# Minimap2onGPU/mm2-gb

Measured on AMD Instinct MI355X. Metric: chaining anchor-pairs/s, higher is better.
Workload: dtype int32+f32

## Files before the change

### include/mm2gb_chain.h

```cpp
#ifndef MM2GB_CHAIN_H
#define MM2GB_CHAIN_H

#include <stddef.h>
#include <stdint.h>

#ifdef __cplusplus
extern "C" {
#endif

#define MM2GB_VERSION "0.1-mi355x"

typedef struct { uint64_t x, y; } mm2gb_anchor_t;

typedef struct {
	int max_iter, max_dist_x, max_dist_y, max_skip, bw, min_cnt, min_score, is_cdna, n_seg;
	float chn_pen_gap, chn_pen_skip;
} mm2gb_misc_t;

typedef struct {
	int     num_streams;
	int     min_n;
	int64_t long_seg_buffer_size;
	int64_t max_total_n;
	int     max_read;
	int     avg_read_n;
	int     has_max_total_n, has_max_read, has_avg_read_n;
	struct { int blockdim, cut_check_anchors, anchor_per_block; } range_kernel;
	struct { int micro_batch, mid_blockdim, short_griddim, long_griddim, mid_griddim,
	             long_seg_cutoff, mid_seg_cutoff; } score_kernel;
} mm2gb_config_t;

typedef struct {
	int64_t n_anchors, n_reads;
	int64_t n_pairs;
	int64_t n_chunks;
	int64_t n_long_chunks;
	int64_t n_mid_chunks;
	int64_t n_tracked_chunks;
	int64_t n_clamped_blocks;
	float   ms_h2d, ms_prep, ms_score, ms_d2h, ms_total;
	float   ms_post;
} mm2gb_stats_t;

typedef struct mm2gb_engine mm2gb_engine_t;

const char *mm2gb_last_error(void);
const char *mm2gb_version(void);

void mm2gb_config_defaults(mm2gb_config_t *cfg);
int  mm2gb_config_parse(const char *json_text, mm2gb_config_t *cfg);
int  mm2gb_config_load(const char *path, mm2gb_config_t *cfg);

int  mm2gb_device_count(void);
int  mm2gb_device_numa_node(int device);
int  mm2gb_pin_thread_to_device(int device);
int  mm2gb_numa_cpus_for_bdf(const char *bdf, const char *sysfs_root_dir, int32_t *node_out, int32_t *cpus, int32_t max_cpus);
mm2gb_engine_t *mm2gb_engine_create(const mm2gb_config_t *cfg, const mm2gb_misc_t *misc, int device);
void mm2gb_engine_destroy(mm2gb_engine_t *eng);
int  mm2gb_engine_set_misc(mm2gb_engine_t *eng, const mm2gb_misc_t *misc);
int  mm2gb_engine_set_chain_skip(mm2gb_engine_t *eng, int keep);
int  mm2gb_engine_last_score_form(const mm2gb_engine_t *eng);
int  mm2gb_engine_band_groups(const mm2gb_engine_t *eng, int64_t *out);
int  mm2gb_engine_skip_stats(mm2gb_engine_t *eng, int64_t *out6);
int  mm2gb_engine_device(const mm2gb_engine_t *eng);
void mm2gb_engine_gang_counts(const mm2gb_engine_t *eng, int64_t *chunks, int64_t *workgroups);
int  mm2gb_has_gang_build(void);
int  mm2gb_engine_reserve(mm2gb_engine_t *eng, int64_t n_anchors, int64_t n_reads);

int mm2gb_score_host(mm2gb_engine_t *eng, int64_t n_reads, const int64_t *offsets, const mm2gb_anchor_t *anchors,
                     int32_t *f, int32_t *p, mm2gb_stats_t *stats);
int mm2gb_score_device(mm2gb_engine_t *eng, int64_t n_reads, const int64_t *d_offsets, const mm2gb_anchor_t *d_anchors,
                       int64_t n_anchors, int32_t *d_f, int32_t *d_p);
int mm2gb_engine_sync(mm2gb_engine_t *eng);
int mm2gb_engine_stats(mm2gb_engine_t *eng, mm2gb_stats_t *stats);
void *mm2gb_engine_stream(mm2gb_engine_t *eng);
float mm2gb_engine_last_kernel_ms(mm2gb_engine_t *eng);

typedef struct {
	int64_t *u_off;   uint64_t *u;
	int64_t *a_off;   mm2gb_anchor_t *a;
} mm2gb_chains_t;
int  mm2gb_chain_host(mm2gb_engine_t *eng, int64_t n_reads, const int64_t *offsets, const mm2gb_anchor_t *anchors,
                      int n_threads, mm2gb_chains_t *out, mm2gb_stats_t *stats);
void mm2gb_chains_free(mm2gb_chains_t *out);

int  mm2gb_chain_gpu(mm2gb_engine_t *eng, int64_t n_reads, const int64_t *offsets, const mm2gb_anchor_t *anchors,
                     mm2gb_chains_t *out, mm2gb_stats_t *stats);
int  mm2gb_post_device(mm2gb_engine_t *eng, int64_t n_reads, const int64_t *d_offsets, const mm2gb_anchor_t *d_anchors, int64_t n_anchors,
                       const int32_t *d_f, const int32_t *d_p, int64_t *n_chains, int64_t *n_kept, float *ms);
int  mm2gb_post_device_enqueue(mm2gb_engine_t *eng, int64_t n_reads, const int64_t *d_offsets, const mm2gb_anchor_t *d_anchors, int64_t n_anchors,
                               const int32_t *d_f, const int32_t *d_p);
int  mm2gb_post_device_totals(mm2gb_engine_t *eng, int64_t *n_chains, int64_t *n_kept, float *ms);
int  mm2gb_post_device_digest(mm2gb_engine_t *eng, int64_t n_reads, uint64_t *digest);
int  mm2gb_debug_last_fill(mm2gb_engine_t *eng, int64_t n, int32_t *f, int32_t *p);

typedef struct {
	int max_dist, max_dist_inner, bw, max_chn_skip, cap_rmq_size, min_cnt, min_sc;
	float chn_pen_gap, chn_pen_skip;
} mm2gb_rmq_param_t;
int  mm2gb_rmq_chain_gpu(mm2gb_engine_t *eng, const mm2gb_rmq_param_t *prm, int64_t n_reads, const int64_t *offsets, const mm2gb_anchor_t *anchors,
                         mm2gb_chains_t *out, int32_t *n_tied, mm2gb_stats_t *stats);
typedef struct { int64_t n_device, n_host_cost, n_host_tie; double est_device_s, est_host_s, device_s, host_s, tie_s, total_s; int32_t device_kernel , n_team ; } mm2gb_rmq_deal_t;
int  mm2gb_engine_set_rmq_kernel(mm2gb_engine_t *eng, int kind);
int  mm2gb_engine_set_rmq_team_reads(mm2gb_engine_t *eng, int n);
int  mm2gb_rmq_chain(mm2gb_engine_t *eng, const mm2gb_rmq_param_t *prm, int64_t n_reads, const int64_t *offsets, const mm2gb_anchor_t *anchors,
                     int n_threads, mm2gb_chains_t *out, int32_t *where, mm2gb_rmq_deal_t *deal);
int  mm2gb_rmq_chain_host(const mm2gb_rmq_param_t *prm, int64_t n_reads, const int64_t *offsets, const mm2gb_anchor_t *anchors, int n_threads,
                          mm2gb_chains_t *out, int32_t *n_tied);
int  mm2gb_rmq_chain_host_tied(const mm2gb_rmq_param_t *prm, int64_t n_reads, const int64_t *offsets, const mm2gb_anchor_t *anchors, int n_threads, mm2gb_chains_t *out);
mm2gb_anchor_t *mm2gb_lchain_rmq(int max_dist, int max_dist_inner, int bw, int max_chn_skip, int cap_rmq_size, int min_cnt, int min_sc,
                                 float chn_pen_gap, float chn_pen_skip, int64_t n, mm2gb_anchor_t *a, int *n_u_, uint64_t **_u, void *km);
void mm2gb_lchain_rmq_counts(int64_t *calls, int64_t *tied_calls);

typedef struct {
	int32_t id, cnt, rid, score, qs, qe, rs, re, parent, subsc, as, mlen, blen, n_sub, score0;
	uint32_t flags;
	uint32_t hash;
	float div;
} mm2gb_reg_t;
int  mm2gb_sort_seeds_gpu(mm2gb_engine_t *eng, int64_t n_reads, const int64_t *offsets, mm2gb_anchor_t *anchors);
typedef struct { uint32_t n, q_pos, span_flt, seg_tandem; } mm2gb_seed_t;
int  mm2gb_collect_seeds_gpu(mm2gb_engine_t *eng, int64_t opt_flag, int64_t n_reads, const int64_t *seed_off, const mm2gb_seed_t *seeds,
                             const int64_t *hit_off, const uint64_t *hits, const int32_t *qlen, const int32_t *q_rank,
                             int32_t n_ref, const int32_t *ref_len, const int32_t *ref_rank, int64_t *anchor_off, mm2gb_anchor_t *anchors);
int  mm2gb_gen_regs_gpu(mm2gb_engine_t *eng, int64_t n_reads, const mm2gb_chains_t *chains, const int32_t *qlen, const uint32_t *hash,
                        int is_qstrand, mm2gb_reg_t *regs);

typedef struct mm2gb_index mm2gb_index_t;
typedef struct { int32_t mid_occ, max_max_occ, occ_dist; float q_occ_frac; } mm2gb_seed_opt_t;
typedef struct {
	int32_t n_seeds, rep_len, n_mini_pos, pad_;
	int64_t n_hits;
	mm2gb_seed_t *seeds;
	uint64_t *hits;
	uint64_t *mini_pos;
} mm2gb_matches_t;
#define MM2GB_I_HPC 0x1
int  mm2gb_sketch(const char *seq, int32_t len, int w, int k, uint32_t rid, uint64_t **out_xy, int64_t *n_out);
int  mm2gb_sketch_flag(const char *seq, int32_t len, int w, int k, uint32_t rid, int flag, uint64_t **out_xy, int64_t *n_out);
mm2gb_index_t *mm2gb_index_build(int k, int w, int32_t n_seq, const char *const *seqs, const int32_t *lens, int n_threads);
mm2gb_index_t *mm2gb_index_build_flag(int k, int w, int flag, int32_t n_seq, const char *const *seqs, const int32_t *lens, int n_threads);
int  mm2gb_index_flag(const mm2gb_index_t *ix);
void mm2gb_index_destroy(mm2gb_index_t *ix);
int64_t mm2gb_index_size(const mm2gb_index_t *ix, int64_t *n_occurrences);
int32_t mm2gb_index_mid_occ(const mm2gb_index_t *ix, float mid_occ_frac, int32_t min_mid_occ, int32_t max_mid_occ);
int  mm2gb_collect_seeds_host(int64_t opt_flag, int64_t n_reads, const int64_t *seed_off, const mm2gb_seed_t *seeds, const int64_t *hit_off,
                              const uint64_t *hits, const int32_t *qlen, const int32_t *q_rank, int32_t n_ref, const int32_t *ref_len,
                              const int32_t *ref_rank, int n_threads, int64_t *anchor_off, mm2gb_anchor_t *anchors);
int  mm2gb_collect_matches(const mm2gb_index_t *ix, const char *seq, int32_t len, const mm2gb_seed_opt_t *opt, mm2gb_matches_t *out);
void mm2gb_matches_free(mm2gb_matches_t *m);

int  mm2gb_sketch_gpu(mm2gb_engine_t *eng, int w, int k, int64_t n_seqs, const int64_t *seq_off, const char *seqs,
                      const uint32_t *rid, int64_t *mini_off, uint64_t **out_xy);
int  mm2gb_sketch_gpu_flag(mm2gb_engine_t *eng, int w, int k, int flag, int64_t n_seqs, const int64_t *seq_off, const char *seqs,
                           const uint32_t *rid, int64_t *mini_off, uint64_t **out_xy);
int  mm2gb_index_to_device(mm2gb_index_t *ix, int device);
typedef struct {
	int64_t n_seeds, n_hits;
	int64_t *seed_off;
	mm2gb_seed_t *seeds;
	int64_t *hit_off;
	uint64_t *hits;
	uint64_t *mini_pos;
	int32_t *rep_len;
} mm2gb_match_batch_t;
int  mm2gb_collect_matches_gpu(mm2gb_engine_t *eng, const mm2gb_index_t *ix, const mm2gb_seed_opt_t *opt, int64_t n_reads,
                               const int64_t *seq_off, const char *seqs, mm2gb_match_batch_t *out);
void mm2gb_match_batch_free(mm2gb_match_batch_t *m);

typedef struct {
	int64_t n_keys, n_occ, n_bucket;
	int32_t bucket_shift, k, w, built_on;
	int64_t uploads;
	const uint64_t *keys;
	const int64_t  *first;
	const uint64_t *where;
	const uint32_t *bucket;
} mm2gb_index_view_t;
mm2gb_index_t *mm2gb_index_build_gpu(mm2gb_engine_t *eng, int k, int w, int32_t n_seq, const char *const *seqs, const int32_t *lens);
mm2gb_index_t *mm2gb_index_build_gpu_flag(mm2gb_engine_t *eng, int k, int w, int flag, int32_t n_seq, const char *const *seqs, const int32_t *lens);
int32_t mm2gb_index_mid_occ_gpu(mm2gb_engine_t *eng, const mm2gb_index_t *ix, float mid_occ_frac, int32_t min_mid_occ, int32_t max_mid_occ);
int  mm2gb_index_view(const mm2gb_index_t *ix, mm2gb_index_view_t *out);
int  mm2gb_index_fetch_device(const mm2gb_index_t *ix, int device, uint64_t *keys, int64_t *first, uint64_t *where, uint32_t *bucket);
int  mm2gb_index_build_split(const mm2gb_index_t *ix, double *ms5);

typedef struct {
	int64_t flag;
	int32_t seed, mid_occ, min_mid_occ, max_mid_occ, max_max_occ, occ_dist;
	float   mid_occ_frac, q_occ_frac;
	int32_t min_cnt, min_chain_score, bw, bw_long, max_gap, max_gap_ref, max_chain_iter;
	int32_t rmq_inner_dist, rmq_size_cap, rmq_rescue_size;
	float   rmq_rescue_ratio, chain_gap_scale, chain_skip_scale;
	float   mask_level; int32_t mask_len; float pri_ratio; int32_t best_n;
	int32_t host_threads;
	int32_t seeds_on_device;
	int32_t rechain_on_device;
	int32_t max_chain_skip;
	int32_t seeding_on_device;
} mm2gb_map_opt_t;
typedef struct { int64_t n_reads, n_mapped, n_anchors, n_chains, n_rechained, n_rmq_tied; double s_seed, s_anchors, s_chain, s_rechain, s_regs, s_post; } mm2gb_map_stats_t;
void mm2gb_map_opt_init(mm2gb_map_opt_t *opt);
int  mm2gb_map_reads(mm2gb_engine_t *eng, const mm2gb_index_t *ix, int k, const char *const *ref_names, const int32_t *ref_lens, int32_t n_ref,
                     const mm2gb_map_opt_t *opt, int32_t n_reads, const char *const *names, const char *const *seqs, const int32_t *lens,
                     char **paf_out, int64_t *paf_len, mm2gb_map_stats_t *stats);

int  mm2gb_map_reads_multi(mm2gb_engine_t *const *engines, int n_engines, const mm2gb_index_t *ix, int k, const char *const *ref_names, const int32_t *ref_lens,
                           int32_t n_ref, const mm2gb_map_opt_t *opt, int32_t n_reads, const char *const *names, const char *const *seqs, const int32_t *lens,
                           char **paf_out, int64_t *paf_len, mm2gb_map_stats_t *stats);
int  mm2gb_map_reads_stream(mm2gb_engine_t *const *engines, int n_engines, const mm2gb_index_t *ix, int k, const char *const *ref_names, const int32_t *ref_lens,
                            int32_t n_ref, const mm2gb_map_opt_t *opt, int32_t n_reads, const char *const *names, const char *const *seqs, const int32_t *lens,
                            int64_t chunk_bases, char **paf_out, int64_t *paf_len, mm2gb_map_stats_t *stats);
int  mm2gb_engine_release_host_scratch(mm2gb_engine_t *eng);

typedef struct mm2gb_pool mm2gb_pool_t;
mm2gb_pool_t *mm2gb_pool_create(const mm2gb_config_t *cfg, const mm2gb_misc_t *misc, int n_devices, const int *devices);
// ... 100 lines not shown
```

### mm2-gb_amd/__init__.py

```python
import ctypes as C
import os

import numpy as np

_HERE = os.path.dirname(os.path.abspath(__file__))
LIB_PATH = os.environ.get("MM2GB_LIB_PATH") or os.path.join(_HERE, "libmm2gb_chain.so")
INT32_MAX = 2**31 - 1


class Misc(C.Structure):
    _fields_ = [("max_iter", C.c_int), ("max_dist_x", C.c_int), ("max_dist_y", C.c_int), ("max_skip", C.c_int),
                ("bw", C.c_int), ("min_cnt", C.c_int), ("min_score", C.c_int), ("is_cdna", C.c_int), ("n_seg", C.c_int),
                ("chn_pen_gap", C.c_float), ("chn_pen_skip", C.c_float)]


class _RangeCfg(C.Structure):
    _fields_ = [("blockdim", C.c_int), ("cut_check_anchors", C.c_int), ("anchor_per_block", C.c_int)]


class _ScoreCfg(C.Structure):
    _fields_ = [("micro_batch", C.c_int), ("mid_blockdim", C.c_int), ("short_griddim", C.c_int), ("long_griddim", C.c_int),
                ("mid_griddim", C.c_int), ("long_seg_cutoff", C.c_int), ("mid_seg_cutoff", C.c_int)]


class Config(C.Structure):
    _fields_ = [("num_streams", C.c_int), ("min_n", C.c_int), ("long_seg_buffer_size", C.c_int64), ("max_total_n", C.c_int64),
                ("max_read", C.c_int), ("avg_read_n", C.c_int),
                ("has_max_total_n", C.c_int), ("has_max_read", C.c_int), ("has_avg_read_n", C.c_int),
                ("range_kernel", _RangeCfg), ("score_kernel", _ScoreCfg)]


class Stats(C.Structure):
    _fields_ = [("n_anchors", C.c_int64), ("n_reads", C.c_int64), ("n_pairs", C.c_int64), ("n_chunks", C.c_int64),
                ("n_long_chunks", C.c_int64), ("n_mid_chunks", C.c_int64), ("n_tracked_chunks", C.c_int64), ("n_clamped_blocks", C.c_int64),
                ("ms_h2d", C.c_float), ("ms_prep", C.c_float), ("ms_score", C.c_float), ("ms_d2h", C.c_float), ("ms_total", C.c_float),
                ("ms_post", C.c_float)]

    def as_dict(self):
        return {k: getattr(self, k) for k, _ in self._fields_}


class Chains(C.Structure):
    _fields_ = [("u_off", C.POINTER(C.c_int64)), ("u", C.POINTER(C.c_uint64)), ("a_off", C.POINTER(C.c_int64)), ("a", C.c_void_p)]


class RmqParam(C.Structure):
    _fields_ = [("max_dist", C.c_int), ("max_dist_inner", C.c_int), ("bw", C.c_int), ("max_chn_skip", C.c_int), ("cap_rmq_size", C.c_int),
                ("min_cnt", C.c_int), ("min_sc", C.c_int), ("chn_pen_gap", C.c_float), ("chn_pen_skip", C.c_float)]


READ_DONE_FN = C.CFUNCTYPE(None, C.c_void_p, C.c_int64, C.c_int, C.POINTER(C.c_uint64), C.c_int64, C.c_void_p)


class BatcherStats(C.Structure):
    _fields_ = [("reads", C.c_int64), ("anchors", C.c_int64), ("reads_per_lane", C.c_int64 * 2), ("batches", C.c_int64 * 2),
                ("batches_per_engine", C.c_int64 * 16), ("n_engines", C.c_int)]


class Mm2gbError(RuntimeError):
    pass


_lib = None

CORE_SYMBOLS = ["mm2gb_last_error", "mm2gb_version", "mm2gb_config_defaults", "mm2gb_config_parse", "mm2gb_config_load",
                "mm2gb_device_count", "mm2gb_device_numa_node", "mm2gb_pin_thread_to_device", "mm2gb_numa_cpus_for_bdf", "mm2gb_engine_create", "mm2gb_engine_destroy", "mm2gb_engine_set_misc", "mm2gb_engine_device", "mm2gb_engine_gang_counts", "mm2gb_has_gang_build",
                "mm2gb_engine_reserve", "mm2gb_score_host", "mm2gb_score_device", "mm2gb_engine_sync", "mm2gb_engine_stats",
                "mm2gb_engine_stream", "mm2gb_engine_last_kernel_ms", "mm2gb_chain_host", "mm2gb_chain_gpu", "mm2gb_post_device", "mm2gb_post_device_enqueue", "mm2gb_post_device_totals", "mm2gb_post_device_digest", "mm2gb_chains_free", "mm2gb_backtrack_host",
                "mm2gb_free", "mm2gb_lchain_dp", "mm2gb_synth_count", "mm2gb_synth_fill",
                "mm2gb_pool_create", "mm2gb_pool_destroy", "mm2gb_pool_size", "mm2gb_pool_device", "mm2gb_pool_set_misc",
                "mm2gb_pool_score_host", "mm2gb_pool_chain_host",
                "mm2gb_batcher_create", "mm2gb_batcher_add", "mm2gb_batcher_feed", "mm2gb_batcher_flush", "mm2gb_batcher_stats", "mm2gb_batcher_destroy",
                "mm2gb_plan_batches", "mm2gb_rmq_chain_gpu", "mm2gb_lchain_rmq", "mm2gb_lchain_rmq_counts",
                "mm2gb_sort_seeds_gpu", "mm2gb_gen_regs_gpu", "mm2gb_collect_seeds_gpu",
                "mm2gb_sketch", "mm2gb_index_build", "mm2gb_index_destroy", "mm2gb_index_size", "mm2gb_index_mid_occ", "mm2gb_collect_matches", "mm2gb_matches_free", "mm2gb_map_opt_init", "mm2gb_map_reads", "mm2gb_engine_release_host_scratch", "mm2gb_rmq_chain_host", "mm2gb_rmq_chain_host_tied", "mm2gb_rmq_chain", "mm2gb_engine_set_rmq_kernel", "mm2gb_engine_set_rmq_team_reads", "mm2gb_engine_set_chain_skip", "mm2gb_engine_last_score_form", "mm2gb_engine_band_groups", "mm2gb_collect_seeds_host", "mm2gb_map_reads_multi", "mm2gb_map_reads_stream",
                "mm2gb_sketch_gpu", "mm2gb_index_to_device", "mm2gb_collect_matches_gpu", "mm2gb_match_batch_free",
                "mm2gb_index_build_gpu", "mm2gb_index_mid_occ_gpu", "mm2gb_index_view", "mm2gb_index_fetch_device", "mm2gb_index_build_split",
                "mm2gb_sketch_flag", "mm2gb_sketch_gpu_flag", "mm2gb_index_build_flag", "mm2gb_index_build_gpu_flag", "mm2gb_index_flag",
                "mm2gb_align_opt_init", "mm2gb_align_regs_host", "mm2gb_align_regs_gpu", "mm2gb_align_out_free"]
BOUNDARY_SYMBOLS = ["init_stream_gpu", "chain_stream_gpu", "finish_stream_gpu", "free_stream_gpu"]


def lib():
    global _lib
    if _lib is None:
        if not os.path.exists(LIB_PATH):
            raise Mm2gbError(f"{LIB_PATH} is missing: build it with `make -C {_HERE}` (hipcc, --offload-arch=gfx950); "
                             "there is no CPU fallback")
        L = C.CDLL(LIB_PATH)
        L.mm2gb_last_error.restype = C.c_char_p
        L.mm2gb_version.restype = C.c_char_p
        L.mm2gb_config_defaults.argtypes = [C.POINTER(Config)]
        L.mm2gb_config_defaults.restype = None
        L.mm2gb_config_parse.argtypes = [C.c_char_p, C.POINTER(Config)]
        L.mm2gb_config_load.argtypes = [C.c_char_p, C.POINTER(Config)]
        L.mm2gb_engine_create.restype = C.c_void_p
        L.mm2gb_engine_create.argtypes = [C.POINTER(Config), C.POINTER(Misc), C.c_int]
        L.mm2gb_engine_destroy.argtypes = [C.c_void_p]
        L.mm2gb_engine_destroy.restype = None
        L.mm2gb_engine_set_misc.argtypes = [C.c_void_p, C.POINTER(Misc)]
        L.mm2gb_engine_device.argtypes = [C.c_void_p]
        L.mm2gb_engine_reserve.argtypes = [C.c_void_p, C.c_int64, C.c_int64]
        L.mm2gb_engine_set_chain_skip.argtypes = [C.c_void_p, C.c_int]
        L.mm2gb_engine_last_score_form.argtypes = [C.c_void_p]
        L.mm2gb_engine_band_groups.argtypes = [C.c_void_p, C.POINTER(C.c_int64)]
        L.mm2gb_score_host.argtypes = [C.c_void_p, C.c_int64, C.c_void_p, C.c_void_p, C.c_void_p, C.c_void_p, C.POINTER(Stats)]
        L.mm2gb_score_device.argtypes = [C.c_void_p, C.c_int64, C.c_void_p, C.c_void_p, C.c_int64, C.c_void_p, C.c_void_p]
        L.mm2gb_engine_sync.argtypes = [C.c_void_p]
        L.mm2gb_engine_stats.argtypes = [C.c_void_p, C.POINTER(Stats)]
        L.mm2gb_engine_stream.argtypes = [C.c_void_p]
        L.mm2gb_engine_stream.restype = C.c_void_p
        L.mm2gb_engine_last_kernel_ms.argtypes = [C.c_void_p]
        L.mm2gb_engine_last_kernel_ms.restype = C.c_float
        L.mm2gb_chain_host.argtypes = [C.c_void_p, C.c_int64, C.c_void_p, C.c_void_p, C.c_int, C.POINTER(Chains), C.POINTER(Stats)]
        L.mm2gb_chain_gpu.argtypes = [C.c_void_p, C.c_int64, C.c_void_p, C.c_void_p, C.POINTER(Chains), C.POINTER(Stats)]
        L.mm2gb_post_device_enqueue.argtypes = [C.c_void_p, C.c_int64, C.c_void_p, C.c_void_p, C.c_int64, C.c_void_p, C.c_void_p]
        L.mm2gb_post_device_totals.argtypes = [C.c_void_p, C.POINTER(C.c_int64), C.POINTER(C.c_int64), C.POINTER(C.c_float)]
        L.mm2gb_post_device_digest.argtypes = [C.c_void_p, C.c_int64, C.c_void_p]
        L.mm2gb_post_device.argtypes = [C.c_void_p, C.c_int64, C.c_void_p, C.c_void_p, C.c_int64, C.c_void_p, C.c_void_p,
                                        C.POINTER(C.c_int64), C.POINTER(C.c_int64), C.POINTER(C.c_float)]
        L.mm2gb_chains_free.argtypes = [C.POINTER(Chains)]
        L.mm2gb_chains_free.restype = None
        L.mm2gb_backtrack_host.argtypes = [C.POINTER(Misc), C.c_int64, C.c_void_p, C.c_void_p, C.c_void_p,
                                           C.POINTER(C.c_void_p), C.POINTER(C.c_void_p)]
        L.mm2gb_free.argtypes = [C.c_void_p]
        L.mm2gb_free.restype = None
        L.mm2gb_lchain_dp.restype = C.c_void_p
        L.mm2gb_lchain_dp.argtypes = [C.c_int] * 7 + [C.c_float, C.c_float, C.c_int, C.c_int, C.c_int64, C.c_void_p,
                                                      C.POINTER(C.c_int), C.POINTER(C.c_void_p), C.c_void_p]
        L.mm2gb_synth_count.restype = C.c_int64
        L.mm2gb_synth_count.argtypes = [C.c_uint64, C.c_int64, C.c_int64, C.c_int, C.c_int, C.c_void_p]
        L.mm2gb_synth_fill.argtypes = [C.c_uint64, C.c_int64, C.c_int64, C.c_int, C.c_int, C.c_void_p, C.c_void_p, C.c_int]
        L.mm2gb_pool_create.restype = C.c_void_p
        L.mm2gb_pool_create.argtypes = [C.POINTER(Config), C.POINTER(Misc), C.c_int, C.c_void_p]
        L.mm2gb_pool_destroy.argtypes = [C.c_void_p]
        L.mm2gb_pool_destroy.restype = None
        L.mm2gb_pool_size.argtypes = [C.c_void_p]
        L.mm2gb_pool_device.argtypes = [C.c_void_p, C.c_int]
        L.mm2gb_pool_set_misc.argtypes = [C.c_void_p, C.POINTER(Misc)]
        L.mm2gb_pool_score_host.argtypes = [C.c_void_p, C.c_int64, C.c_void_p, C.c_void_p, C.c_void_p, C.c_void_p, C.POINTER(Stats), C.c_void_p]
        L.mm2gb_pool_chain_host.argtypes = [C.c_void_p, C.c_int64, C.c_void_p, C.c_void_p, C.c_int, C.POINTER(Chains), C.POINTER(Stats)]
        L.mm2gb_rmq_chain_gpu.argtypes = [C.c_void_p, C.POINTER(RmqParam), C.c_int64, C.c_void_p, C.c_void_p, C.POINTER(Chains), C.c_void_p, C.POINTER(Stats)]
        L.mm2gb_lchain_rmq.restype = C.c_void_p
        L.mm2gb_lchain_rmq.argtypes = [C.c_int] * 7 + [C.c_float, C.c_float, C.c_int64, C.c_void_p, C.POINTER(C.c_int), C.POINTER(C.c_void_p), C.c_void_p]
        L.mm2gb_lchain_rmq_counts.argtypes = [C.POINTER(C.c_int64), C.POINTER(C.c_int64)]
        L.mm2gb_lchain_rmq_counts.restype = None
        L.mm2gb_sort_seeds_gpu.argtypes = [C.c_void_p, C.c_int64, C.c_void_p, C.c_void_p]
        L.mm2gb_sketch.argtypes = [C.c_char_p, C.c_int32, C.c_int, C.c_int, C.c_uint32, C.POINTER(C.c_void_p), C.POINTER(C.c_int64)]
        L.mm2gb_sketch_flag.argtypes = [C.c_char_p, C.c_int32, C.c_int, C.c_int, C.c_uint32, C.c_int, C.POINTER(C.c_void_p), C.POINTER(C.c_int64)]
        L.mm2gb_index_build_flag.restype = C.c_void_p
        L.mm2gb_index_build_flag.argtypes = [C.c_int, C.c_int, C.c_int, C.c_int32, C.POINTER(C.c_char_p), C.c_void_p, C.c_int]
        L.mm2gb_index_build_gpu_flag.restype = C.c_void_p
        L.mm2gb_index_build_gpu_flag.argtypes = [C.c_void_p, C.c_int, C.c_int, C.c_int, C.c_int32, C.POINTER(C.c_char_p), C.c_void_p]
        L.mm2gb_index_flag.argtypes = [C.c_void_p]
        L.mm2gb_sketch_gpu_flag.argtypes = [C.c_void_p, C.c_int, C.c_int, C.c_int, C.c_int64, C.c_void_p, C.c_char_p, C.c_void_p, C.c_void_p, C.POINTER(C.c_void_p)]
        L.mm2gb_index_build.restype = C.c_void_p
        L.mm2gb_index_build.argtypes = [C.c_int, C.c_int, C.c_int32, C.POINTER(C.c_char_p), C.c_void_p, C.c_int]
        L.mm2gb_index_destroy.restype = None
        L.mm2gb_index_destroy.argtypes = [C.c_void_p]
        L.mm2gb_index_size.restype = C.c_int64
        L.mm2gb_index_size.argtypes = [C.c_void_p, C.POINTER(C.c_int64)]
        L.mm2gb_index_mid_occ.restype = C.c_int32
        L.mm2gb_index_mid_occ.argtypes = [C.c_void_p, C.c_float, C.c_int32, C.c_int32]
        L.mm2gb_index_build_gpu.restype = C.c_void_p
        L.mm2gb_index_build_gpu.argtypes = [C.c_void_p, C.c_int, C.c_int, C.c_int32, C.POINTER(C.c_char_p), C.c_void_p]
        L.mm2gb_index_mid_occ_gpu.restype = C.c_int32
        L.mm2gb_index_mid_occ_gpu.argtypes = [C.c_void_p, C.c_void_p, C.c_float, C.c_int32, C.c_int32]
        L.mm2gb_index_view.argtypes = [C.c_void_p, C.c_void_p]
        L.mm2gb_index_fetch_device.argtypes = [C.c_void_p, C.c_int, C.c_void_p, C.c_void_p, C.c_void_p, C.c_void_p]
        L.mm2gb_index_build_split.argtypes = [C.c_void_p, C.c_void_p]
        L.mm2gb_collect_matches.argtypes = [C.c_void_p, C.c_char_p, C.c_int32, C.c_void_p, C.c_void_p]
        L.mm2gb_matches_free.restype = None
        L.mm2gb_matches_free.argtypes = [C.c_void_p]
        L.mm2gb_sketch_gpu.argtypes = [C.c_void_p, C.c_int, C.c_int, C.c_int64, C.c_void_p, C.c_char_p, C.c_void_p, C.c_void_p, C.POINTER(C.c_void_p)]
        L.mm2gb_index_to_device.argtypes = [C.c_void_p, C.c_int]
        L.mm2gb_collect_matches_gpu.argtypes = [C.c_void_p, C.c_void_p, C.c_void_p, C.c_int64, C.c_void_p, C.c_char_p, C.c_void_p]
        L.mm2gb_match_batch_free.restype = None
        L.mm2gb_match_batch_free.argtypes = [C.c_void_p]
        L.mm2gb_collect_seeds_gpu.argtypes = [C.c_void_p, C.c_int64, C.c_int64, C.c_void_p, C.c_void_p, C.c_void_p, C.c_void_p, C.c_void_p, C.c_void_p,
                                              C.c_int32, C.c_void_p, C.c_void_p, C.c_void_p, C.c_void_p]
        L.mm2gb_gen_regs_gpu.argtypes = [C.c_void_p, C.c_int64, C.POINTER(Chains), C.c_void_p, C.c_void_p, C.c_int, C.c_void_p]
        L.mm2gb_batcher_create.restype = C.c_void_p
        L.mm2gb_batcher_create.argtypes = [C.POINTER(Config), C.POINTER(Misc), C.c_int, C.c_void_p, C.c_int, READ_DONE_FN, C.c_void_p]
        L.mm2gb_batcher_add.argtypes = [C.c_void_p, C.c_int64, C.c_void_p, C.c_int64]
        L.mm2gb_batcher_flush.argtypes = [C.c_void_p]
        L.mm2gb_batcher_stats.argtypes = [C.c_void_p, C.POINTER(BatcherStats)]
        L.mm2gb_batcher_destroy.argtypes = [C.c_void_p]
        L.mm2gb_batcher_destroy.restype = None
        L.mm2gb_plan_batches.restype = C.c_int64
        L.mm2gb_plan_batches.argtypes = [C.c_int64, C.c_void_p, C.c_int64, C.c_int, C.c_int, C.c_void_p, C.c_void_p]
        _lib = L
    return _lib


def _check(rc):
    if rc != 0:
        raise Mm2gbError(lib().mm2gb_last_error().decode())


def default_misc(**kw):
    d = dict(max_iter=5000, max_dist_x=5000, max_dist_y=5000, max_skip=INT32_MAX, bw=500, min_cnt=3, min_score=40,
             is_cdna=0, n_seg=1, chn_pen_gap=np.float32(0.8 * 0.01 * 15), chn_pen_skip=np.float32(0.0))
    d.update(kw)
    return Misc(**d)


def default_config():
    c = Config()
    lib().mm2gb_config_defaults(C.byref(c))
    return c


def parse_config(text):
    c = Config()
    _check(lib().mm2gb_config_parse(text.encode(), C.byref(c)))
    return c


def load_config(path):
    c = Config()
    _check(lib().mm2gb_config_load(os.fsencode(path), C.byref(c)))
    return c


def device_count():
    return lib().mm2gb_device_count()


def device_numa_node(device):
    return lib().mm2gb_device_numa_node(int(device))


def pin_thread_to_device(device):
    return lib().mm2gb_pin_thread_to_device(int(device))


def numa_cpus_for_bdf(bdf, sysfs_root=""):
    L = lib()
    L.mm2gb_numa_cpus_for_bdf.restype = C.c_int
    L.mm2gb_numa_cpus_for_bdf.argtypes = [C.c_char_p, C.c_char_p, C.POINTER(C.c_int32), C.POINTER(C.c_int32), C.c_int32]
    node = C.c_int32(-1)
    buf = (C.c_int32 * 4096)()
    n = L.mm2gb_numa_cpus_for_bdf(bdf.encode(), sysfs_root.encode(), C.byref(node), buf, 4096)
    return node.value, list(buf[:min(n, 4096)])


class Engine:

    def __init__(self, misc=None, config=None, device=0, chain_skip=None):
        L = lib()
        self.misc = misc if misc is not None else default_misc()
        self.config = config if config is not None else default_config()
        self.device = int(device)
        self._h = L.mm2gb_engine_create(C.byref(self.config), C.byref(self.misc), device)
        if not self._h:
            raise Mm2gbError(L.mm2gb_last_error().decode())
        if chain_skip is not None:
            self.set_chain_skip(chain_skip)

    def close(self):
        if getattr(self, "_h", None):
            lib().mm2gb_engine_destroy(self._h)
            self._h = None

    __del__ = close

    def __enter__(self):
        return self

    def __exit__(self, *exc):
        self.close()

    def set_misc(self, misc):
        _check(lib().mm2gb_engine_set_misc(self._h, C.byref(misc)))
        self.misc = misc

    def set_chain_skip(self, keep):
        _check(lib().mm2gb_engine_set_chain_skip(self._h, 1 if keep else 0))

    def last_score_form(self):
        return int(lib().mm2gb_engine_last_score_form(self._h))

    def band_groups(self):
        out = (C.c_int64 * 2)()
        _check(lib().mm2gb_engine_band_groups(self._h, out))
        return int(out[0]), int(out[1])

    def skip_stats(self):
        L = lib()
        L.mm2gb_engine_skip_stats.argtypes = [C.c_void_p, C.c_void_p]
        out = np.zeros(6, dtype=np.int64)
        _check(L.mm2gb_engine_skip_stats(self._h, out.ctypes.data))
        keys = ("rounds", "rescan_rounds", "targets", "slowest_chunk_ticks", "slowest_chunk_anchors", "span_ticks")
        return {k: int(v) for k, v in zip(keys, out)}

    def gang_counts(self):
        c, h = C.c_int64(), C.c_int64()
        lib().mm2gb_engine_gang_counts.argtypes = [C.c_void_p, C.POINTER(C.c_int64), C.POINTER(C.c_int64)]
        lib().mm2gb_engine_gang_counts.restype = None
        lib().mm2gb_engine_gang_counts(self._h, C.byref(c), C.byref(h))
        return c.value, h.value

    def score(self, anchors, offsets):
        a = np.ascontiguousarray(anchors, dtype=np.uint64)
        off = np.ascontiguousarray(offsets, dtype=np.int64)
        n = int(off[-1])
        assert a.shape == (n, 2)
        f = np.empty(n, dtype=np.int32)
        p = np.empty(n, dtype=np.int32)
        st = Stats()
        _check(lib().mm2gb_score_host(self._h, len(off) - 1, off.ctypes.data, a.ctypes.data, f.ctypes.data, p.ctypes.data, C.byref(st)))
        return f, p, st.as_dict()

    def score_device(self, n_reads, d_offsets, d_anchors, n_anchors, d_f, d_p):
        _check(lib().mm2gb_score_device(self._h, n_reads, d_offsets, d_anchors, n_anchors, d_f, d_p))

    def sync(self):
        _check(lib().mm2gb_engine_sync(self._h))

    def stats(self):
        st = Stats()
        _check(lib().mm2gb_engine_stats(self._h, C.byref(st)))
        return st.as_dict()

    def stream(self):
        return lib().mm2gb_engine_stream(self._h)

    def chain(self, anchors, offsets, threads=1):
        a = np.ascontiguousarray(anchors, dtype=np.uint64)
        off = np.ascontiguousarray(offsets, dtype=np.int64)
        R = len(off) - 1
        out = Chains()
        st = Stats()
        _check(lib().mm2gb_chain_host(self._h, R, off.ctypes.data, a.ctypes.data, threads, C.byref(out), C.byref(st)))
        return _take_chains(out, R), st.as_dict()


def _engine_chain_gpu(self, anchors, offsets):
    a = np.ascontiguousarray(anchors, dtype=np.uint64)
    off = np.ascontiguousarray(offsets, dtype=np.int64)
    R = len(off) - 1
    out = Chains()
    st = Stats()
    _check(lib().mm2gb_chain_gpu(self._h, R, off.ctypes.data, a.ctypes.data, C.byref(out), C.byref(st)))
    return _take_chains(out, R), st.as_dict()


Engine.chain_gpu = _engine_chain_gpu


def default_rmq_param(**kw):
    d = dict(max_dist=5000, max_dist_inner=1000, bw=20000, max_chn_skip=INT32_MAX, cap_rmq_size=100000, min_cnt=3, min_sc=40,
             chn_pen_gap=np.float32(0.8 * 0.01 * 15), chn_pen_skip=np.float32(0.0))
    d.update(kw)
    return RmqParam(**d)


def _engine_rmq_chain(self, anchors, offsets, prm):
    a = np.ascontiguousarray(anchors, dtype=np.uint64)
    off = np.ascontiguousarray(offsets, dtype=np.int64)
    R = len(off) - 1
    out = Chains()
    st = Stats()
    tied = np.zeros(max(R, 1), dtype=np.int32)
    _check(lib().mm2gb_rmq_chain_gpu(self._h, C.byref(prm), R, off.ctypes.data, a.ctypes.data, C.byref(out), tied.ctypes.data, C.byref(st)))
    return _take_chains(out, R), tied[:R], st.as_dict()


Engine.rmq_chain = _engine_rmq_chain


class RmqDeal(C.Structure):
    _fields_ = [("n_device", C.c_int64), ("n_host_cost", C.c_int64), ("n_host_tie", C.c_int64), ("est_device_s", C.c_double), ("est_host_s", C.c_double),
                ("device_s", C.c_double), ("host_s", C.c_double), ("tie_s", C.c_double), ("total_s", C.c_double), ("device_kernel", C.c_int32), ("n_team", C.c_int32)]

    def as_dict(self):
        return {k: getattr(self, k) for k, _ in self._fields_}


def _engine_rmq_chain_exact(self, anchors, offsets, prm, threads=4):
    L = lib()
    L.mm2gb_rmq_chain.argtypes = [C.c_void_p, C.c_void_p, C.c_int64, C.c_void_p, C.c_void_p, C.c_int, C.c_void_p, C.c_void_p, C.c_void_p]
    a = np.ascontiguousarray(anchors, dtype=np.uint64)
    off = np.ascontiguousarray(offsets, dtype=np.int64)
    R = len(off) - 1
    out = Chains()
    where = np.zeros(max(R, 1), dtype=np.int32)
    deal = RmqDeal()
    _check(L.mm2gb_rmq_chain(self._h, C.byref(prm), R, off.ctypes.data, a.ctypes.data, int(threads), C.byref(out), where.ctypes.data, C.byref(deal)))
    return _take_chains(out, R), where[:R], deal.as_dict()


Engine.rmq_chain_exact = _engine_rmq_chain_exact


def rmq_chain_host(anchors, offsets, prm, threads=4):
    L = lib()
    L.mm2gb_rmq_chain_host.argtypes = [C.c_void_p, C.c_int64, C.c_void_p, C.c_void_p, C.c_int, C.c_void_p, C.c_void_p]
    a = np.ascontiguousarray(anchors, dtype=np.uint64)
    off = np.ascontiguousarray(offsets, dtype=np.int64)
    R = len(off) - 1
    out = Chains()
    tied = np.zeros(max(R, 1), dtype=np.int32)
    _check(L.mm2gb_rmq_chain_host(C.byref(prm), R, off.ctypes.data, a.ctypes.data, int(threads), C.byref(out), tied.ctypes.data))
    return _take_chains(out, R), tied[:R]

REG_DTYPE = np.dtype([(k, "<i4") for k in "id cnt rid score qs qe rs re parent subsc as_ mlen blen n_sub score0".split()] +
                     [("flags", "<u4"), ("hash", "<u4"), ("div", "<f4")])


def _engine_sort_seeds(self, anchors, offsets):
    a = np.ascontiguousarray(anchors, dtype=np.uint64).copy()
    off = np.ascontiguousarray(offsets, dtype=np.int64)
    _check(lib().mm2gb_sort_seeds_gpu(self._h, len(off) - 1, off.ctypes.data, a.ctypes.data))
    return a


def _engine_collect_seeds(self, flag, reads, ref_len=None, ref_rank=None):
    R = len(reads)
    seed_off = np.zeros(R + 1, np.int64)
    seed_off[1:] = np.cumsum([len(r["seeds"]) for r in reads])
    seeds = np.ascontiguousarray(np.concatenate([np.asarray(r["seeds"], np.uint32).reshape(-1, 4) for r in reads]) if R else np.zeros((0, 4), np.uint32), dtype=np.uint32)
    hit_off = np.zeros(len(seeds) + 1, np.int64)
    np.cumsum(seeds[:, 0], out=hit_off[1:])
    hits = np.ascontiguousarray(np.concatenate([np.asarray(r["hits"], np.uint64) for r in reads]) if R else np.zeros(0, np.uint64), dtype=np.uint64)
    qlen = np.ascontiguousarray([r["qlen"] for r in reads], dtype=np.int32)
    have_rank = any("q_rank" in r for r in reads)
    q_rank = np.ascontiguousarray([r.get("q_rank", 0) for r in reads], dtype=np.int32) if have_rank else None
    rl = np.ascontiguousarray(ref_len, dtype=np.int32) if ref_len is not None else None
    rr = np.ascontiguousarray(ref_rank, dtype=np.int32) if ref_rank is not None else None
    n_ref = len(rl) if rl is not None else (len(rr) if rr is not None else 0)
    a_off = np.zeros(R + 1, np.int64)
    out = np.zeros((max(len(hits), 1), 2), np.uint64)
    _check(lib().mm2gb_collect_seeds_gpu(self._h, int(flag), R, seed_off.ctypes.data, seeds.ctypes.data, hit_off.ctypes.data, hits.ctypes.data, qlen.ctypes.data,
                                         q_rank.ctypes.data if q_rank is not None else None, n_ref, rl.ctypes.data if rl is not None else None,
                                         rr.ctypes.data if rr is not None else None, a_off.ctypes.data, out.ctypes.data))
    return [out[a_off[r]:a_off[r + 1]].copy() for r in range(R)]


# ... 650 lines not shown
```

### mm2-gb_amd/csrc/chain_dev.h

```cpp
#pragma once
#include <hip/hip_runtime.h>
#include <stdint.h>

namespace mm2gb {

struct DevParams {
	int   max_dist_x, max_dist_y, bw, max_iter, n_seg, is_cdna;
	int   dq_lim;
	int   lut_last;
	int   lut_base;
	int   lut_clamp;
	int   free_sweep;
	int   band_slab;
	int   band_lag;
	float gap, skip;
};

enum : unsigned { FLAG_ANY_SEGID = 1u,
                  FLAG_NO_LUT = 2u };

constexpr int LUT_LDS_TOTAL = 31 * 2560;
constexpr int LUT_ENTRIES   = 5120;
constexpr int LUT_LDS_BASE  = LUT_LDS_TOTAL - LUT_ENTRIES * 4;
constexpr int LUT_BIAS      = (1 << 30) + (1 << 16);

constexpr int PLAN_BLOCK = 1024;
#ifndef MM2GB_PLAN_THREADS
#define MM2GB_PLAN_THREADS 256
#endif
constexpr int PLAN_THREADS = MM2GB_PLAN_THREADS;
constexpr int COST_PER_ANCHOR = 16;
constexpr int PLAN_COST_BINS = 1024;

struct GangSlot {
	int next_strip;
	int done;
	int keep[6];
	int chunk;
	int first_wg, n_wg;
	int tiles_per_wave;
	int pad_[20];
};
static_assert(sizeof(GangSlot) == 128, "one slot per 128-byte line");
constexpr int GANG_MAX_CHUNKS = 64;
constexpr int GANG_STRIP_PAIRS = 16;

struct DevBatch {
	const uint4   *raw;
	const int64_t *offsets;
	int64_t        n;
	int64_t        n_reads;
	int32_t  *st;
	int32_t  *f;
	int32_t  *p;
	int32_t  *diag;
	int32_t  *band_res;
	int32_t  *blk_firstcut;
	int64_t  *blk_pairs;
	int32_t  *blk_clamped;
	int32_t  *blk_read;
	int32_t  *blk_wmax;
	int64_t   n_blocks;
	int32_t  *chunk_start, *chunk_end;
	int64_t  *chunk_cost;
	uint8_t  *chunk_track;
	int64_t  *chunk_pp;
	int32_t  *chunk_kk, *chunk_blk;
	int64_t  *tile_sums, *tile_base;
	int32_t  *bins;
	int32_t  *order;
	int32_t  *long_list;
	int32_t  *mid_list;
	int32_t  *counters;
	int64_t  *totals;
	unsigned *flags;
	const int32_t *lut;
	int64_t  *dbg;
	GangSlot *gang_slots;
};
enum { CNT_NCHUNK = 0, CNT_CURSOR = 1, CNT_NLONG = 2, CNT_LCURSOR = 3, CNT_NTRACK = 4, CNT_NCLAMP = 5, CNT_NMID = 6, CNT_MCURSOR = 7,
       CNT_NGANG = 12,
       CNT_GANG_STRIPS = 13,
       CNT_GANG_WGS = 14,
       CNT_BAND_WAVE = 16,
       CNT_BAND_TEAM = 17,
       CNT_WORDS = 18 };

struct LaunchCfg {
	int score_grid;
	int host_mode;
	int ring_slots;
	int big_team;
	int whole_wg_pct;
	int team4_all;
	int team4_share_pct;
	int gang_max;
	int gang_pct;
	int gang_pairs;
	int64_t long_min_cost;
	int     long_min_window;
	int     wide_window;
};

void launch_window(const DevBatch &b, const DevParams &P, hipStream_t s);
void launch_plan(const DevBatch &b, const LaunchCfg &cfg, hipStream_t s);
void launch_score(const DevBatch &b, const DevParams &P, const LaunchCfg &cfg, hipStream_t s);
constexpr int SKIP_STAT_WORDS = 6;
void launch_skip_fill(const DevBatch &b, const DevParams &P, int max_skip, int32_t *mark, unsigned long long *stats, int n_cu, hipStream_t s);
void launch_build_lut(int *d_lut, const DevParams &P, hipStream_t s);
size_t score_lds_bytes(const DevParams &P, int host_mode, int ring_slots);
int  score_set_lds_limit(size_t bytes);
enum { SCORE_MODE_LUT = 0, SCORE_MODE_FAST = 1, SCORE_MODE_GENERAL = 2 };

}
```

### mm2-gb_amd/csrc/chain_kernels.hip

```cpp
#include <hip/hip_runtime.h>
#include <stdint.h>
#include <limits.h>
#include <algorithm>
#include "chain_dev.h"
#include "wave_scan.h"

namespace mm2gb {

#define WAVE 64

__device__ __forceinline__ int lane_id() { return threadIdx.x & (WAVE - 1); }
__device__ __forceinline__ int bcast(int v, int src_lane) { return __builtin_amdgcn_readlane(v, src_lane); }
__device__ __forceinline__ int first_lane(int v) { return __builtin_amdgcn_readfirstlane(v); }
__device__ __forceinline__ int wave_max_i32_dpp(int v)
{
	v = max(v, __builtin_amdgcn_update_dpp(INT_MIN, v, 0x111, 0xf, 0xf, false));
	v = max(v, __builtin_amdgcn_update_dpp(INT_MIN, v, 0x112, 0xf, 0xf, false));
	v = max(v, __builtin_amdgcn_update_dpp(INT_MIN, v, 0x114, 0xf, 0xf, false));
	v = max(v, __builtin_amdgcn_update_dpp(INT_MIN, v, 0x118, 0xf, 0xf, false));
	v = max(v, __builtin_amdgcn_update_dpp(INT_MIN, v, 0x142, 0xa, 0xf, false));
	v = max(v, __builtin_amdgcn_update_dpp(INT_MIN, v, 0x143, 0xc, 0xf, false));
	return __builtin_amdgcn_readlane(v, WAVE - 1);
}
__device__ __forceinline__ int prev_lane(int v) { return __builtin_amdgcn_update_dpp(v, v, 0x138, 0xf, 0xf, false); }
__device__ __forceinline__ int a_x(const DevBatch &b, int i) { return ((const int*)b.raw)[(size_t)i * 4]; }
__device__ __forceinline__ int a_y(const DevBatch &b, int i) { return ((const int*)b.raw)[(size_t)i * 4 + 2]; }
__device__ __forceinline__ int a_span(const DevBatch &b, int i) { return (int)(((const unsigned*)b.raw)[(size_t)i * 4 + 3] & 0xffu); }
__device__ __forceinline__ int tag_of(unsigned y_hi) { return (int)(((y_hi >> 8) & 0xff00u) | (y_hi & 0xffu)); }
__device__ __forceinline__ int a_tag(const DevBatch &b, int i) { return tag_of(((const unsigned*)b.raw)[(size_t)i * 4 + 3]); }


__device__ __forceinline__ bool in_reach(int2 v, int hi_i, unsigned x_i, unsigned dist)
{
	return v.y == hi_i && x_i <= (unsigned)v.x + dist;
}

constexpr int WIN_SAMPLE = 32;
#ifndef MM2GB_WIN_LOOKBACK
#define MM2GB_WIN_LOOKBACK 1024
#endif
constexpr int WIN_LOOKBACK = MM2GB_WIN_LOOKBACK;
constexpr int WIN_SAMPLES = WIN_LOOKBACK / WIN_SAMPLE;
constexpr int WIN_PER = PLAN_BLOCK / PLAN_THREADS;
static_assert(WIN_LOOKBACK % WIN_SAMPLE == 0 && WIN_SAMPLES <= WAVE, "the samples are one wave's lanes");
static_assert(WIN_LOOKBACK % PLAN_THREADS == 0 && 32 % WIN_PER == 0, "staging rounds; a thread's anchors share one word of read starts");

__global__ __launch_bounds__(256) void k_block_reads(DevBatch b)
{
	const int64_t blk = (int64_t)blockIdx.x * blockDim.x + threadIdx.x;
	if (blk >= b.n_blocks) return;
	const int64_t base = blk * PLAN_BLOCK;
	int64_t lo = 0, hi = b.n_reads;
	while (hi - lo > 1) {
		const int64_t mid = (lo + hi) >> 1;
		if (b.offsets[mid] <= base) lo = mid; else hi = mid;
	}
	b.blk_read[blk] = (int32_t)lo;
}

__global__ __launch_bounds__(PLAN_THREADS) void k_window(DevBatch b, DevParams P)
{
	constexpr int NW = PLAN_THREADS / WAVE;
	__shared__ int s_cut[NW];
	__shared__ unsigned long long s_pairs[NW];
	__shared__ int s_clamp[NW];
	__shared__ int s_wmax[2 * NW];
	__shared__ int2 win[WIN_LOOKBACK + PLAN_BLOCK];
	__shared__ unsigned s_starts[PLAN_BLOCK / 32];
	__shared__ unsigned s_disorder[PLAN_BLOCK / 32];
	const unsigned nb = gridDim.x, per = nb / 8, rem = nb % 8, xcd = blockIdx.x % 8, kth = blockIdx.x / 8;
	const unsigned blk = nb < 64 ? blockIdx.x : xcd * per + (xcd < rem ? xcd : rem) + kth;
	const int64_t base = (int64_t)blk * PLAN_BLOCK;
	const int base32 = (int)base, lds0 = base32 - WIN_LOOKBACK;
	const unsigned dist = (unsigned)P.max_dist_x;
	if (threadIdx.x < PLAN_BLOCK / 32) s_starts[threadIdx.x] = s_disorder[threadIdx.x] = 0;
	__syncthreads();

	const int64_t rd_first = b.blk_read[blk];
	uint4 own[WIN_PER];
#pragma unroll
	for (int m = 0; m < WIN_PER; ++m) {
		const int64_t g = base + threadIdx.x + m * PLAN_THREADS;
		own[m] = g < b.n ? b.raw[g] : make_uint4(0, 0, 0, 0);
	}
	const uint2 x0 = *(const uint2*)&b.raw[base];
	uint2 own_prev[WIN_PER];
#pragma unroll
	for (int m = 0; m < WIN_PER; ++m) {
		const int64_t g = base + threadIdx.x + m * PLAN_THREADS;
		own_prev[m] = make_uint2(0, 0);
		if (lane_id() == 0 && g > 0 && g <= b.n) own_prev[m] = *(const uint2*)&b.raw[g - 1];
	}
	const int64_t smp_pos = base - (int64_t)(lane_id() + 1) * WIN_SAMPLE;
	uint2 smp = make_uint2(0, 0);
	if (lane_id() < WIN_SAMPLES && smp_pos >= 0) smp = *(const uint2*)&b.raw[smp_pos];
	const int rs_first = (int)b.offsets[rd_first];
	for (int64_t r0 = rd_first + 1; r0 <= b.n_reads; r0 += PLAN_THREADS) {
		const int64_t r = r0 + threadIdx.x;
		if (r <= b.n_reads) {
			const int64_t v = b.offsets[r] - base;
			if (v >= 0 && v < PLAN_BLOCK) atomicOr(&s_starts[v >> 5], 1u << (v & 31));
		}
		if (b.offsets[min(r0 + PLAN_THREADS - 1, b.n_reads)] >= base + PLAN_BLOCK) break;
	}
	bool any_seg = false, big_y = false;
#pragma unroll
	for (int m = 0; m < WIN_PER; ++m) {
		const int k = threadIdx.x + m * PLAN_THREADS;
		const uint4 v = own[m];
		if (base + k < b.n) {
			const unsigned span = v.w & 0xffu;
			const unsigned seg = (v.w >> 16) & 0xffu;
			any_seg |= seg != 0;
			big_y |= v.z >= (1u << 22) || span == 0;
		}
		win[WIN_LOOKBACK + k] = make_int2((int)v.x, (int)v.y);
		const unsigned nx = (unsigned)prev_lane((int)v.x), nh = (unsigned)prev_lane((int)v.y);
		const unsigned px = lane_id() == 0 ? own_prev[m].x : nx, ph = lane_id() == 0 ? own_prev[m].y : nh;
		if (k > 0 && base + k < b.n && (ph > v.y || (ph == v.y && px > v.x))) atomicOr(&s_disorder[k >> 5], 1u << (k & 31));
	}
	if (__ballot(any_seg) != 0 && lane_id() == 0) atomicOr(b.flags, FLAG_ANY_SEGID);
	if (__ballot(big_y) != 0 && lane_id() == 0) atomicOr(b.flags, FLAG_NO_LUT);

	const int lo = (int)max((int64_t)rs_first, base - (int64_t)P.max_iter - 1);
	const bool smp_in = lane_id() < WIN_SAMPLES && smp_pos >= lo && in_reach(make_int2((int)smp.x, (int)smp.y), (int)x0.y, x0.x, dist);
	const unsigned long long smp_mask = ~__ballot(smp_in);
	const int n_in = smp_mask == 0 ? WAVE : __builtin_ctzll(smp_mask);
	const int floor_ = n_in < WIN_SAMPLES ? max(lo, base32 - (n_in + 1) * WIN_SAMPLE) : lo;
	const int ls = max(floor_, lds0);
#pragma unroll
	for (int m = 0; m < WIN_LOOKBACK / PLAN_THREADS; ++m) {
		const int j = base32 - WIN_LOOKBACK + (int)threadIdx.x + m * PLAN_THREADS;
		if (j >= ls) win[j - lds0] = *(const int2*)&b.raw[j];
	}
	__syncthreads();

	const int q0 = (int)threadIdx.x * WIN_PER;
	const int w0 = q0 >> 5;
	int start_before = -1;
	for (int u = 0; u < w0; ++u) {
		const unsigned word = s_starts[u];
		if (word != 0) start_before = u * 32 + 31 - __clz(word);
	}
	const unsigned my_word = s_starts[w0];
	const bool sorted = __ballot(lane_id() < PLAN_BLOCK / 32 && (s_disorder[lane_id()] & ~s_starts[lane_id()]) != 0) == 0;
	auto read_in_order = [&](int q, int rq) {
		const int lo = max(rq, 0);
		int hi = PLAN_BLOCK;
		for (int u = q >> 5; u < PLAN_BLOCK / 32; ++u) {
			const unsigned m = s_starts[u] & (u > q >> 5 ? 0xffffffffu : (q & 31) == 31 ? 0u : 0xffffffffu << ((q & 31) + 1));
			if (m != 0) { hi = u * 32 + __ffs(m) - 1; break; }
		}
		for (int u = lo >> 5; u <= (hi - 1) >> 5; ++u) {
			const unsigned from = u == lo >> 5 ? 0xffffffffu << (lo & 31) : 0xffffffffu;
			const unsigned to = u == (hi - 1) >> 5 ? 0xffffffffu >> (31 - ((hi - 1) & 31)) : 0xffffffffu;
			if (s_disorder[u] & ~s_starts[u] & from & to) return false;
		}
// ... 1075 lines not shown
			for (; jb < i0; jb += WAVE) {
				const int jn = jb + WAVE < i0 ? jb + WAVE + lane : jb + lane;
				const int nf = b.f[jn], nq = MODE == MODE_LUT ? a_span(b, jn) : 0;
				const int k_from = tile_lo > jb ? tile_lo - jb : 0;
				sweep_any<MODE>(b, T, jb, k_from, sf, sq, jb >= st_hi && jb + WAVE <= eq_lo, stage, P, lut, best, arg);
				sf = nf; sq = nq;
			}
		}
		in_tile<MODE, TRACK>(b, T, i0, n_here, P, lut, stage, best, arg, keep, [&](int jj) { return b.f[jj]; });
		if (T.live) {
			const int i = i0 + lane;
			b.f[i] = arg < 0 ? T.q : best;
			b.p[i] = arg < 0 ? 0 : i - arg;
		}
	}
}

struct TilePair {
	TileXY A, B;
	int n_a, n_b;
	int lo_a, hi_a, lo_b, hi_b;
	int x_first, x_last_a, x_last;
	int best_a, arg_a, best_b, arg_b;
};

__device__ __forceinline__ TileXY load_xy(const DevBatch &b, int i0, int ce, int &best)
{
	const int i = i0 + lane_id();
	const bool live = i < ce;
	const int il = live ? i : ce - 1;
	TileXY t;
	t.x = a_x(b, il); t.y = a_y(b, il);
	t.st = live ? b.st[il] : INT_MAX;
	best = a_span(b, il) + 1;
	return t;
}

__device__ __forceinline__ TilePair load_pair(const DevBatch &b, int i0, int ce)
{
	TilePair t;
	t.n_a = min(WAVE, ce - i0);
	t.n_b = max(0, min(WAVE, ce - i0 - WAVE));
	t.A = load_xy(b, i0, ce, t.best_a);
	t.B = load_xy(b, t.n_b ? i0 + WAVE : i0, ce, t.best_b);
	t.lo_a = first_lane(t.A.st); t.hi_a = bcast(t.A.st, t.n_a - 1);
	t.lo_b = t.n_b ? first_lane(t.B.st) : INT_MAX; t.hi_b = t.n_b ? bcast(t.B.st, t.n_b - 1) : INT_MAX;
	t.x_first = first_lane(t.A.x); t.x_last_a = bcast(t.A.x, t.n_a - 1);
	t.x_last = t.n_b ? bcast(t.B.x, t.n_b - 1) : t.x_last_a;
	t.arg_a = -1; t.arg_b = -1;
	return t;
}

__device__ __forceinline__ void sweep_pair_block(const DevBatch &b, TilePair &t, int jb, int eq_lo, int sf, int sq, int4 *stage, const DevParams &P)
{
	const bool nc_a = jb >= t.hi_a && jb + WAVE <= eq_lo;
	const bool use_b = t.n_b > 0 && jb + WAVE > t.lo_b;
	const bool nc_b = use_b && jb >= t.hi_b && jb + WAVE <= eq_lo;
	const int xs = a_x(b, jb + lane_id()), ys = a_y(b, jb + lane_id());
	const unsigned free_span = (unsigned)(P.dq_lim - P.bw);
	const bool free_block = P.free_sweep && (unsigned)(t.x_last - first_lane(xs)) <= free_span;
	const bool free_a = P.free_sweep && (unsigned)(t.x_last_a - first_lane(xs)) <= free_span;
	const bool single = t.n_b == 0;
	const bool far_block = free_block && nc_a && (nc_b || single) && t.x_first > bcast(xs, WAVE - 1) && __ballot(sq + P.bw > t.x_first - bcast(xs, WAVE - 1)) == 0;
	const int d0 = (first_lane(xs) - first_lane(ys)) * 4;
	stage_block_lut(xs, ys, sf, sq, stage, far_block, d0);
	if (nc_a && nc_b) sweep_staged_lut2(t.A, t.B, jb, free_block, far_block, d0, stage, P, t.best_a, t.arg_a, t.best_b, t.arg_b);
	else {
		sweep_staged_lut(t.A, jb, t.lo_a > jb ? t.lo_a - jb : 0, nc_a, nc_a && free_a, stage, P, t.best_a, t.arg_a, far_block, d0);
		if (use_b) sweep_staged_lut(t.B, jb, t.lo_b > jb ? t.lo_b - jb : 0, nc_b, nc_b && free_block, stage, P, t.best_b, t.arg_b);
	}
	__builtin_amdgcn_wave_barrier();
}

__device__ __forceinline__ void sweep_a_into_b(const DevBatch &b, TilePair &t, int cs, int i0, int f_a, int q_a, int4 *stage, const DevParams &P)
{
	if (i0 + WAVE <= t.lo_b) return;
	stage_block_lut(b, i0, f_a, q_a, stage);
	const int eq_lo = equal_x_run_start(b, cs, i0 + WAVE, first_lane(t.B.x));
	const bool no_check = i0 >= t.hi_b && i0 + WAVE <= eq_lo;
	const bool span_ab = P.free_sweep && (unsigned)(t.x_last - t.x_first) <= (unsigned)(P.dq_lim - P.bw);
	sweep_staged_lut(t.B, i0, t.lo_b > i0 ? t.lo_b - i0 : 0, no_check, no_check && span_ab, stage, P, t.best_b, t.arg_b);
	__builtin_amdgcn_wave_barrier();
}

__device__ __forceinline__ int wave_min_i32(int v) { return -wave_max_i32_dpp(-v); }

__device__ __forceinline__ void sweep_block_lut_band(int t_st, int tx4, int ty4, int idx, const int4 *stage, const DevParams &P, int &bestv)
{
	constexpr int G = 4;
	const unsigned base = (unsigned)P.lut_base, lim4 = (unsigned)P.dq_lim << 2;
	int pos = 0x7fffffff;
	asm volatile("" : "+v"(pos));
	for (int kg = 0; kg < WAVE; kg += G) {
		int4 s4[G];
		int dqm[G], drm[G], pen[G];
#pragma unroll
		for (int u = 0; u < G; ++u) s4[u] = stage[kg + u];
#pragma unroll
		for (int u = 0; u < G; ++u) {
			dqm[u] = ty4 - s4[u].w; drm[u] = tx4 - s4[u].z;
			pen[u] = *(lds_i32_ptr)(uintptr_t)lut_address(drm[u], dqm[u] & pos, base);
		}
#pragma unroll
		for (int u = 0; u < G; ++u) {
			const int dg = drm[u] < dqm[u] ? drm[u] : dqm[u];
			int v = ((s4[u].y < dg ? s4[u].y : dg) << 5) + s4[u].x;
			asm("" : "+v"(v));
			v += pen[u];
			const int j = __builtin_amdgcn_readlane(idx, kg + u);
			unsigned long long saved;
			asm volatile("s_mov_b64 %[sv], exec\n\tv_cmpx_gt_u32_e32 vcc, %[lim], %[dq]\n\tv_cmpx_ge_i32_e32 vcc, %[j], %[st]\n\tv_max_i32_e32 %[b], %[v], %[b]\n\ts_mov_b64 exec, %[sv]"
			             : [b] "+v"(bestv), [sv] "=&s"(saved) : [lim] "s"(lim4), [dq] "v"(dqm[u]), [st] "v"(t_st), [j] "s"(j), [v] "v"(v) : "vcc");
		}
	}
}

__device__ __forceinline__ int band_group(const DevBatch &b, const DevParams &P, int4 *stage, const int tgt, const int jl)
{
	const int lane = lane_id();
	const int l0 = __builtin_ctzll(__ballot(tgt >= 0));
	const int t = tgt >= 0 ? tgt : bcast(tgt, l0);
	const int x = a_x(b, t), y = a_y(b, t), st = b.st[t];
	int best = a_span(b, t) + 1, arg = -1;
	const int lo = wave_min_i32(st), hi_st = wave_max_i32_dpp(st);
	if (lo < jl) {
		const int d = x - y;
		const int dmin = wave_min_i32(d), dmax = wave_max_i32_dpp(d);
		const int gx_min = wave_min_i32(x), gx_max = wave_max_i32_dpp(x);
		const int band_lo = dmin - P.bw;
		const unsigned width = (unsigned)(dmax - dmin) + 2u * (unsigned)P.bw;
		const int tx4 = (int)(((unsigned)x - 1u) << 2), ty4 = (int)(((unsigned)y - 1u) << 2);
		const unsigned free_span = (unsigned)(P.dq_lim - P.bw);
		auto sweep = [&](const int idx) __attribute__((always_inline)) {
			const int xs = a_x(b, idx), ys = a_y(b, idx), sq = a_span(b, idx), sf = b.f[idx];
			const int sx_min = wave_min_i32(xs), sx_max = wave_max_i32_dpp(xs);
			const bool no_check = first_lane(idx) >= hi_st && gx_min > sx_max;
			const bool free_block = no_check && P.free_sweep && (unsigned)(gx_max - sx_min) <= free_span;
			const bool far_block = free_block && __ballot(sq + P.bw > gx_min - xs) == 0;
			const int d0 = (first_lane(xs) - first_lane(ys)) * 4;
			stage_block_lut(xs, ys, sf, sq, stage, far_block, d0);
			int bestv = best << 7;
			if (far_block) sweep_block_lut_free<true>(tx4, ty4, stage, (unsigned)P.lut_base, d0, bestv);
			else if (free_block) sweep_block_lut_free<false>(tx4, ty4, stage, (unsigned)P.lut_base, 0, bestv);
			else if (no_check) sweep_block_lut<false, false>(st, tx4, ty4, 0, 0, stage, P, bestv);
			else sweep_block_lut_band(st, tx4, ty4, idx, stage, P, bestv);
			const int won = bestv & 127;
			const int wj = __shfl(idx, (won - 1) & (WAVE - 1));
			arg = (unsigned)(won - 1) < (unsigned)WAVE ? wj : arg;
			best = bestv >> 7;
			__builtin_amdgcn_wave_barrier();
		};
		int sidx = 0, n_st = 0;
		int jb = lo;
		int dn = jb + lane < jl ? __hip_atomic_load(b.diag + jb + lane, __ATOMIC_RELAXED, __HIP_MEMORY_SCOPE_AGENT) : 0;
		for (; jb < jl; jb += WAVE) {
			const int j = jb + lane;
			const int dj = dn;
			dn = j + WAVE < jl ? __hip_atomic_load(b.diag + j + WAVE, __ATOMIC_RELAXED, __HIP_MEMORY_SCOPE_AGENT) : 0;
			const bool hit = j < jl && (unsigned)(dj - band_lo) <= width;
			const unsigned long long m = __ballot(hit);
			if (m == 0) continue;
			const int c = __popcll(m);
			const int rank = __builtin_amdgcn_mbcnt_hi((unsigned)(m >> 32), __builtin_amdgcn_mbcnt_lo((unsigned)m, 0u));
			const int dst = (hit ? n_st + rank : n_st + c) & (WAVE - 1);
			const int recv = __builtin_amdgcn_ds_permute(dst << 2, j);
			if (n_st + c < WAVE) {
				sidx = lane >= n_st && lane < n_st + c ? recv : sidx;
				n_st += c;
			} else {
				sweep(lane >= n_st ? recv : sidx);
				n_st += c - WAVE;
				sidx = recv;
			}
		}
		if (n_st > 0) sweep(lane < n_st ? sidx : bcast(sidx, n_st - 1));
	}
	if (tgt >= 0) { b.band_res[2 * tgt] = best; b.band_res[2 * tgt + 1] = arg; }
	return lo < jl;
}

__device__ __forceinline__ int band_slab_part(const DevBatch &b, const DevParams &P, int4 *stage, const int s0, const int n, const int jl,
                                              const int g_from, const int g_to)
{
	constexpr int R = 8;
	const int lane = lane_id();
	unsigned key[R];
	int lo = INT_MAX, hi = INT_MIN, st_lo = INT_MAX;
#pragma unroll
	for (int r = 0; r < R; ++r) {
		const int e = r * WAVE + lane;
		const int d = e < n ? a_x(b, s0 + e) - a_y(b, s0 + e) : 0;
		if (e < n) { lo = min(lo, d); hi = max(hi, d); st_lo = min(st_lo, b.st[s0 + e]); }
	}
	if (wave_min_i32(st_lo) >= jl) return 0;
	const int dmin = wave_min_i32(lo), dmax = wave_max_i32_dpp(hi);
	const unsigned range = (unsigned)(dmax - dmin);
	if (range <= 2u * (unsigned)P.bw) {
#pragma unroll
		for (int r = 0; r < R; ++r) key[r] = r * WAVE + lane < n ? (unsigned)(r * WAVE + lane) : ~0u;
	} else {
		const int sh = (range >> 22) ? 32 - __clz((int)(range >> 22)) : 0;
#pragma unroll
		for (int r = 0; r < R; ++r) {
			const int e = r * WAVE + lane;
			key[r] = e < n ? (((unsigned)(a_x(b, s0 + e) - a_y(b, s0 + e) - dmin) >> sh) << 9) | (unsigned)e : ~0u;
		}
#pragma unroll
		for (int k = 2; k <= R * WAVE; k <<= 1) {
#pragma unroll
			for (int j = k >> 1; j > 0; j >>= 1) {
				if (j >= WAVE) {
					const int jr = j / WAVE;
#pragma unroll
					for (int r = 0; r < R; ++r) {
						if (r & jr) continue;
						const bool up = ((r * WAVE) & k) == 0;
						const unsigned a = key[r], c = key[r | jr];
						key[r] = up ? min(a, c) : max(a, c);
						key[r | jr] = up ? max(a, c) : min(a, c);
					}
				} else {
#pragma unroll
					for (int r = 0; r < R; ++r) {
						const unsigned o = (unsigned)__shfl_xor((int)key[r], j);
						const bool up = ((r * WAVE + lane) & k) == 0, lower = (lane & j) == 0;
						key[r] = up == lower ? min(key[r], o) : max(key[r], o);
					}
				}
			}
		}
	}
	int swept = 0;
	for (int g = g_from; g < g_to; ++g) {
		unsigned kg = key[0];
#pragma unroll
		for (int r = 1; r < R; ++r) kg = g == r ? key[r] : kg;
		const int tgt = kg == ~0u ? -1 : s0 + (int)(kg & 511u);
		if (__ballot(tgt >= 0) == 0) break;
		swept += band_group(b, P, stage, tgt, jl);
	}
	return swept;
}
__device__ __forceinline__ bool band_fits_team(const DevParams &P, const int anchors_per_part, const int n_waves)
{
	return P.band_slab > 0 && P.band_slab / anchors_per_part <= n_waves;
}
__device__ __forceinline__ bool band_chunk(const DevBatch &b, const DevParams &P, const int ci, const int cs, const int ce)
{
	const long long len = ce - cs;
	return P.band_slab > 0 && b.band_res && 2 * (b.chunk_cost[ci] - 16 * len) > (long long)P.band_lag * len;
}

__device__ __forceinline__ void band_merge(const DevBatch &b, const int i0, const int n_here, int &best, int &arg)
{
	const int i = i0 + min(lane_id(), n_here - 1);
	const int bb = __hip_atomic_load(b.band_res + 2 * i, __ATOMIC_RELAXED, __HIP_MEMORY_SCOPE_AGENT);
	const int ba = __hip_atomic_load(b.band_res + 2 * i + 1, __ATOMIC_RELAXED, __HIP_MEMORY_SCOPE_AGENT);
	const bool take = ba >= 0 && (arg < 0 || bb > best);
	best = take ? bb : best;
	arg = take ? ba : arg;
}

__device__ __forceinline__ void band_store_diag(const DevBatch &b, const TilePair &t, const int i0)
{
	if (lane_id() < t.n_a) b.diag[i0 + lane_id()] = t.A.x - t.A.y;
	if (lane_id() < t.n_b) b.diag[i0 + WAVE + lane_id()] = t.B.x - t.B.y;
}

template <bool TRACK>
__device__ __forceinline__ void run_chunk_pairs(const DevBatch &b, const DevParams &P, const int *lut, int4 *stage, const int cs, const int ce, const bool band_on)
{
	const int lane = lane_id();
	Keep keep; keep.idx = -1; keep.x = keep.hi = keep.y = keep.tag = keep.f = 0;
	auto f_old = [&](int jj) { return b.f[jj]; };
	const bool band = band_on;
	int band_groups = 0;
	for (int i0 = cs; i0 < ce; i0 += 2 * WAVE) {
		TilePair t = load_pair(b, i0, ce);
		int jb = cs + ((t.lo_a - cs) & ~(WAVE - 1));
		const int s0 = band ? i0 - (i0 - cs) % P.band_slab : cs, jl = s0 - P.band_lag;
		const bool in_band = band && jl > cs;
		if (band) band_store_diag(b, t, i0);
		if (in_band && i0 == s0) {
			band_groups += band_slab_part(b, P, stage, s0, min(P.band_slab, ce - s0), jl, 0, P.band_slab / WAVE);
			asm volatile("s_waitcnt vmcnt(0)" ::: "memory");
		}
		if (in_band && jb < jl) jb = jl;
		if (jb < i0) {
			const int eq_lo = equal_x_run_start(b, cs, i0, first_lane(t.A.x));
			int sf = b.f[jb + lane], sq = a_span(b, jb + lane);
			for (; jb < i0; jb += WAVE) {
				const int jn = jb + WAVE < i0 ? jb + WAVE + lane : jb + lane;
				const int nf = b.f[jn], nq = a_span(b, jn);
				sweep_pair_block(b, t, jb, eq_lo, sf, sq, stage, P);
				sf = nf; sq = nq;
			}
		}
		const Target TA = load_target(b, i0, ce, TRACK);
		if (in_band && t.lo_a < jl) band_merge(b, i0, t.n_a, t.best_a, t.arg_a);
		in_tile<MODE_LUT, TRACK>(b, TA, i0, t.n_a, P, lut, stage, t.best_a, t.arg_a, keep, f_old);
		const int f_a = t.arg_a < 0 ? TA.q : t.best_a;
		if (TA.live) {
			const int i = i0 + lane;
			b.f[i] = f_a;
			b.p[i] = t.arg_a < 0 ? 0 : i - t.arg_a;
		}
		if (t.n_b == 0) break;
		sweep_a_into_b(b, t, cs, i0, f_a, TA.q, stage, P);
		const Target TB = load_target(b, i0 + WAVE, ce, TRACK);
		if (in_band && t.lo_b < jl) band_merge(b, i0 + WAVE, t.n_b, t.best_b, t.arg_b);
		in_tile<MODE_LUT, TRACK>(b, TB, i0 + WAVE, t.n_b, P, lut, stage, t.best_b, t.arg_b, keep, f_old);
		if (TB.live) {
			const int i = i0 + WAVE + lane;
			b.f[i] = t.arg_b < 0 ? TB.q : t.best_b;
			b.p[i] = t.arg_b < 0 ? 0 : i - t.arg_b;
		}
	}
	if (band_groups > 0 && lane == 0) atomicAdd(&b.counters[CNT_BAND_WAVE], band_groups);
}

struct CoopShared { int done; int keep[6]; int chunk; int bar_count; int bar_gen; int part; int band; };
#define MM2GB_AGENT __HIP_MEMORY_SCOPE_AGENT
__device__ __forceinline__ int  gload(const int *p) { return __hip_atomic_load(p, __ATOMIC_RELAXED, MM2GB_AGENT); }
__device__ __forceinline__ void gstore(int *p, int v) { __hip_atomic_store(p, v, __ATOMIC_RELAXED, MM2GB_AGENT); }
__device__ __forceinline__ void drain_stores() { asm volatile("s_waitcnt vmcnt(0)" ::: "memory"); }
constexpr int SMALL_TEAM = 4, N_SMALL_TEAMS = SCORE_THREADS / WAVE / SMALL_TEAM;
constexpr int N_TEAM_RECORDS = N_SMALL_TEAMS + 3;
constexpr int TAB_INTS = 12;

__device__ __forceinline__ void team_barrier(CoopShared *sh, int team_size)
{
	__builtin_amdgcn_fence(__ATOMIC_RELEASE, "workgroup");
	if (lane_id() == 0) {
		const int gen = __hip_atomic_load(&sh->bar_gen, __ATOMIC_RELAXED, __HIP_MEMORY_SCOPE_WORKGROUP);
		if (__hip_atomic_fetch_add(&sh->bar_count, 1, __ATOMIC_ACQ_REL, __HIP_MEMORY_SCOPE_WORKGROUP) == team_size - 1) {
			__hip_atomic_store(&sh->bar_count, 0, __ATOMIC_RELAXED, __HIP_MEMORY_SCOPE_WORKGROUP);
			__hip_atomic_fetch_add(&sh->bar_gen, 1, __ATOMIC_RELEASE, __HIP_MEMORY_SCOPE_WORKGROUP);
		} else {
			while (__hip_atomic_load(&sh->bar_gen, __ATOMIC_ACQUIRE, __HIP_MEMORY_SCOPE_WORKGROUP) == gen) __builtin_amdgcn_s_sleep(2);
		}
	}
	__builtin_amdgcn_fence(__ATOMIC_ACQUIRE, "workgroup");
}

template <class TT, class SF, class WQ>
__device__ __forceinline__ void sweep_block_by_quarters(const DevBatch &b, const TT &T, const int jb, const int k_from, const int sq, int4 *stage, const DevParams &P,
                                                        int &best, int &arg, SF &&sf_of, WQ &&wait_q)
{
	const int xs = a_x(b, jb + lane_id()), ys = a_y(b, jb + lane_id());
	const int tx4 = (int)(((unsigned)T.x - 1u) << 2), ty4 = (int)(((unsigned)T.y - 1u) << 2);
	for (int q = 0; q < 4; ++q) {
		wait_q(q);
		const int lo = max(k_from, 16 * q), hi = 16 * q + 16;
		if (lo >= hi) continue;
		stage_block_lut(xs, ys, sf_of(), sq, stage);
		int bestv = best << 7;
		sweep_block_lut_edge(T.st, tx4, ty4, jb, lo, stage, P, bestv, hi);
		const int won = bestv & 127;
		arg = (unsigned)(won - 1) < (unsigned)WAVE ? jb + won - 1 : arg;
		best = bestv >> 7;
		__builtin_amdgcn_wave_barrier();
	}
}

template <int MODE, bool TRACK>
__device__ __forceinline__ void coop_chunk(const DevBatch &b, const DevParams &P, const int *lut, int4 *stage, int *ring, const int n_slots, CoopShared *sh,
                           const int cs, const int ce, const int wave, const int n_waves, const bool band_on)
{
	const int lane = lane_id();
	const int n_tiles = (ce - cs + WAVE - 1) / WAVE;
	auto wait_done = [&](int need) {
		while (first_lane(__hip_atomic_load(&sh->done, __ATOMIC_ACQUIRE, __HIP_MEMORY_SCOPE_WORKGROUP)) < need) __builtin_amdgcn_s_sleep(MM2GB_POLL_SLEEP);
	};
	const bool band = MODE == MODE_LUT && band_on && band_fits_team(P, WAVE, n_waves);
	const int tps = band ? P.band_slab / WAVE : 1, s_first = band ? P.band_lag / P.band_slab + 1 : 0;
	int band_groups = 0;
	for (int t = wave; t < n_tiles; t += n_waves) {
		const int i0 = cs + t * WAVE;
		const Target T = load_target(b, i0, ce, TRACK);
		const int n_here = min(WAVE, ce - i0);
		int best = T.q + 1, arg = -1;
		const int tile_lo = first_lane(T.st);
		const int st_hi = bcast(T.st, n_here - 1);
		int jb = cs + ((tile_lo - cs) & ~(WAVE - 1));
		const int sl = t / tps, s0 = cs + sl * P.band_slab, jl = s0 - P.band_lag;
		const bool in_band = band && jl > cs;
		int *band_cnt = sl & 1 ? &sh->band : &sh->part;
		if (band && T.live) b.diag[i0 + lane] = T.x - T.y;
		if (in_band) {
			const int part = t - sl * tps;
			wait_done((jl - cs) / WAVE);
			band_groups += band_slab_part(b, P, stage, s0, min(P.band_slab, ce - s0), jl, part, part + 1);
			if (lane == 0) __hip_atomic_fetch_add(band_cnt, 1, __ATOMIC_RELEASE, __HIP_MEMORY_SCOPE_WORKGROUP);
			if (jb < jl) jb = jl;
		}
		const int eq_lo = MODE == MODE_LUT && jb < i0 ? equal_x_run_start(b, cs, i0, first_lane(T.x)) : i0;
		int slot = (int)((unsigned)((jb - cs) / WAVE) % (unsigned)n_slots);
		for (; jb < i0; jb += WAVE) {
			const int sq = MODE == MODE_LUT ? a_span(b, jb + lane) : 0;
			const int k = (jb - cs) / WAVE, k_from = tile_lo > jb ? tile_lo - jb : 0;
			wait_done(k + 1);
			const int sf = ring[slot * WAVE + lane];
			slot = slot + 1 == n_slots ? 0 : slot + 1;
			sweep_any<MODE>(b, T, jb, k_from, sf, sq, jb >= st_hi && jb + WAVE <= eq_lo, stage, P, lut, best, arg);
		}
		const int my_slot = (int)((unsigned)t % (unsigned)n_slots);
		wait_done(t);
		if (in_band && tile_lo < jl) {
			const int s_min = s_first + ((sl - s_first) & 1);
			const int need = tps * ((sl - s_min) / 2) + min(tps, n_tiles - sl * tps);
			while (first_lane(__hip_atomic_load(band_cnt, __ATOMIC_ACQUIRE, __HIP_MEMORY_SCOPE_WORKGROUP)) < need) __builtin_amdgcn_s_sleep(MM2GB_POLL_SLEEP);
			band_merge(b, i0, n_here, best, arg);
		}
		Keep keep;
		if (TRACK) { keep.idx = first_lane(sh->keep[0]); keep.x = first_lane(sh->keep[1]); keep.hi = first_lane(sh->keep[2]); keep.y = first_lane(sh->keep[3]); keep.tag = first_lane(sh->keep[4]); keep.f = first_lane(sh->keep[5]); }
		else { keep.idx = -1; keep.x = keep.hi = keep.y = keep.tag = keep.f = 0; }
		in_tile<MODE, TRACK>(b, T, i0, n_here, P, lut, stage, best, arg, keep,
		                     [&](int jj) { const unsigned d = (unsigned)(jj - cs); return ring[(d / WAVE) % (unsigned)n_slots * WAVE + d % WAVE]; });
		const int i = i0 + lane;
		const int fi = arg < 0 ? T.q : best;
		if (T.live) {
			ring[my_slot * WAVE + lane] = fi;
			b.f[i] = fi;
			b.p[i] = arg < 0 ? 0 : i - arg;
		}
		if (TRACK && lane == 0) { sh->keep[0] = keep.idx; sh->keep[1] = keep.x; sh->keep[2] = keep.hi; sh->keep[3] = keep.y; sh->keep[4] = keep.tag; sh->keep[5] = keep.f; }
		if (lane == 0) __hip_atomic_store(&sh->done, t + 1, __ATOMIC_RELEASE, __HIP_MEMORY_SCOPE_WORKGROUP);
	}
	if (band_groups > 0 && lane == 0) atomicAdd(&b.counters[CNT_BAND_TEAM], band_groups);
}

template <bool TRACK>
__device__ __forceinline__ void coop_chunk_pairs(const DevBatch &b, const DevParams &P, const int *lut, int4 *stage, int *ring, const int n_slots, CoopShared *sh,
                                 const int cs, const int ce, const int wave, const int n_waves, const bool band_on)
{
	const int lane = lane_id();
	const int n_tiles = (ce - cs + WAVE - 1) / WAVE;
	auto wait_done = [&](int need) {
		while (first_lane(__hip_atomic_load(&sh->done, __ATOMIC_ACQUIRE, __HIP_MEMORY_SCOPE_WORKGROUP)) < need) __builtin_amdgcn_s_sleep(MM2GB_POLL_SLEEP);
	};
	int cur = 0;
	const lds_i32_ptr ring_l = (lds_i32_ptr)(uintptr_t)(unsigned)(uintptr_t)ring;
	auto f_old = [&](int jj) {
		const unsigned d = (unsigned)(jj - cs);
		const int k = (int)(d / WAVE);
		return k >= cur - n_slots ? ring_l[(unsigned)k % (unsigned)n_slots * WAVE + d % WAVE] : b.f[jj];
	};
	const bool band = band_on && band_fits_team(P, 2 * WAVE, n_waves);
	const int pps = band ? P.band_slab / (2 * WAVE) : 1, n_pairs = (n_tiles + 1) / 2, s_first = band ? P.band_lag / P.band_slab + 1 : 0;
	int band_groups = 0;
	for (int pr = wave; 2 * pr < n_tiles; pr += n_waves) {
		const int ta = 2 * pr, i0 = cs + ta * WAVE;
		TilePair t = load_pair(b, i0, ce);
		int jb = cs + ((t.lo_a - cs) & ~(WAVE - 1));
		const int sl = pr / pps, s0 = cs + sl * P.band_slab, jl = s0 - P.band_lag;
		const bool in_band = band && jl > cs;
		int *band_cnt = sl & 1 ? &sh->band : &sh->part;
		if (band) band_store_diag(b, t, i0);
		if (in_band) {
			const int part = pr - sl * pps;
			wait_done((jl - cs) / WAVE);
			band_groups += band_slab_part(b, P, stage, s0, min(P.band_slab, ce - s0), jl, 2 * part, 2 * part + 2);
			if (lane == 0) __hip_atomic_fetch_add(band_cnt, 1, __ATOMIC_RELEASE, __HIP_MEMORY_SCOPE_WORKGROUP);
			if (jb < jl) jb = jl;
		}
		const int eq_lo = jb < i0 ? equal_x_run_start(b, cs, i0, first_lane(t.A.x)) : i0;
		int slot = (int)((unsigned)((jb - cs) / WAVE) % (unsigned)n_slots);
		const int first_in_ring = ta - n_slots;
		int nf = 0;
		if (jb < i0 && (jb - cs) / WAVE < first_in_ring) { wait_done((jb - cs) / WAVE + 1); nf = b.f[jb + lane]; }
		for (; jb < i0; jb += WAVE) {
			const int sq = a_span(b, jb + lane);
			const int k = (jb - cs) / WAVE;
			wait_done(k + 1);
			int sf;
			if (k < first_in_ring) {
				sf = nf;
				if (k + 1 < first_in_ring) { wait_done(k + 2); nf = b.f[jb + WAVE + lane]; }
			} else sf = ring[slot * WAVE + lane];
			slot = slot + 1 == n_slots ? 0 : slot + 1;
			sweep_pair_block(b, t, jb, eq_lo, sf, sq, stage, P);
		}
		const int slot_a = (int)((unsigned)ta % (unsigned)n_slots), slot_b = slot_a + 1 == n_slots ? 0 : slot_a + 1;
		wait_done(ta);
		Keep keep;
		if (TRACK) { keep.idx = first_lane(sh->keep[0]); keep.x = first_lane(sh->keep[1]); keep.hi = first_lane(sh->keep[2]); keep.y = first_lane(sh->keep[3]); keep.tag = first_lane(sh->keep[4]); keep.f = first_lane(sh->keep[5]); }
		else { keep.idx = -1; keep.x = keep.hi = keep.y = keep.tag = keep.f = 0; }
		const Target TA = load_target(b, i0, ce, TRACK);
		if (in_band && t.lo_a < jl) {
			const int s_min = s_first + ((sl - s_first) & 1);
			const int need = pps * ((sl - s_min) / 2) + min(pps, n_pairs - sl * pps);
			while (first_lane(__hip_atomic_load(band_cnt, __ATOMIC_ACQUIRE, __HIP_MEMORY_SCOPE_WORKGROUP)) < need) __builtin_amdgcn_s_sleep(MM2GB_POLL_SLEEP);
			band_merge(b, i0, t.n_a, t.best_a, t.arg_a);
		}
		cur = ta;
		in_tile<MODE_LUT, TRACK>(b, TA, i0, t.n_a, P, lut, stage, t.best_a, t.arg_a, keep, f_old);
		__builtin_amdgcn_s_setprio(MM2GB_INTILE_PRIO);
		const int f_a = t.arg_a < 0 ? TA.q : t.best_a;
		if (TA.live) {
			const int i = i0 + lane;
			ring[slot_a * WAVE + lane] = f_a;
			b.f[i] = f_a;
			b.p[i] = t.arg_a < 0 ? 0 : i - t.arg_a;
		}
		if (t.n_b > 0) {
			if (lane == 0) __hip_atomic_store(&sh->done, ta + 1, __ATOMIC_RELEASE, __HIP_MEMORY_SCOPE_WORKGROUP);
			sweep_a_into_b(b, t, cs, i0, f_a, TA.q, stage, P);
			const Target TB = load_target(b, i0 + WAVE, ce, TRACK);
			if (in_band && t.lo_b < jl) {
				const int s_min = s_first + ((sl - s_first) & 1);
				const int need = pps * ((sl - s_min) / 2) + min(pps, n_pairs - sl * pps);
				while (first_lane(__hip_atomic_load(band_cnt, __ATOMIC_ACQUIRE, __HIP_MEMORY_SCOPE_WORKGROUP)) < need) __builtin_amdgcn_s_sleep(MM2GB_POLL_SLEEP);
				band_merge(b, i0 + WAVE, t.n_b, t.best_b, t.arg_b);
			}
			cur = ta + 1;
			in_tile<MODE_LUT, TRACK>(b, TB, i0 + WAVE, t.n_b, P, lut, stage, t.best_b, t.arg_b, keep, f_old);
			__builtin_amdgcn_s_setprio(MM2GB_INTILE_PRIO);
			if (TB.live) {
				const int i = i0 + WAVE + lane;
				const int f_b = t.arg_b < 0 ? TB.q : t.best_b;
				ring[slot_b * WAVE + lane] = f_b;
				b.f[i] = f_b;
				b.p[i] = t.arg_b < 0 ? 0 : i - t.arg_b;
			}
		}
		if (TRACK && lane == 0) { sh->keep[0] = keep.idx; sh->keep[1] = keep.x; sh->keep[2] = keep.hi; sh->keep[3] = keep.y; sh->keep[4] = keep.tag; sh->keep[5] = keep.f; }
		if (lane == 0) __hip_atomic_store(&sh->done, ta + (t.n_b > 0 ? 2 : 1), __ATOMIC_RELEASE, __HIP_MEMORY_SCOPE_WORKGROUP);
		__builtin_amdgcn_s_setprio(0);
	}
	if (band_groups > 0 && lane == 0) atomicAdd(&b.counters[CNT_BAND_TEAM], band_groups);
}


template <bool TRACK>
__device__ __forceinline__ void gang_chunk_pairs(const DevBatch &b, const DevParams &P, const int *lut, int4 *stage, int *ring, const int n_slots, CoopShared *sh,
                                 GangSlot *gs, int *tab, int &seq, const int cs, const int ce, const int wave)
{
	const int lane = lane_id();
	const int n_tiles = (ce - cs + WAVE - 1) / WAVE;
	const int tpu = first_lane(gload(&gs->tiles_per_wave)) == 2 ? 2 : 1;
	const int STRIP_TILES = tpu * GANG_STRIP_PAIRS;
	int known = 0, known_global = 0;
	auto look_global = [&]() { known_global = max(known_global, first_lane(gload(&gs->done))); known = max(known, known_global); };
	auto wait_done = [&](int need) {
		if (known >= need) return;
		for (;;) {
			known = max(known, first_lane(__hip_atomic_load(&sh->done, __ATOMIC_ACQUIRE, __HIP_MEMORY_SCOPE_WORKGROUP)));
			if (known >= need) return;
			look_global();
			if (known >= need) { if (lane == 0) __hip_atomic_fetch_max(&sh->done, known, __ATOMIC_RELEASE, __HIP_MEMORY_SCOPE_WORKGROUP); return; }
			__builtin_amdgcn_s_sleep(MM2GB_GANG_POLL_SLEEP);
		}
	};
	auto wait_done_global = [&](int need) { while (known_global < need) { look_global(); if (known_global < need) __builtin_amdgcn_s_sleep(MM2GB_GANG_POLL_SLEEP); } };
	int s0 = -1, s1 = -1, s2 = -1;
	int cur = 0;
	const lds_i32_ptr ring_l = (lds_i32_ptr)(uintptr_t)(unsigned)(uintptr_t)ring;
	auto in_ring = [&](int k) { const int sk = k / STRIP_TILES; return (sk == s0 || sk == s1 || sk == s2) && k >= cur - n_slots; };
	auto f_old = [&](int jj) {
		const unsigned d = (unsigned)(jj - cs);
		const int k = (int)(d / WAVE);
		return in_ring(k) ? ring_l[(unsigned)k % (unsigned)n_slots * WAVE + d % WAVE] : gload(&b.f[jj]);
	};
	for (;; ++seq) {
		int s = 0;
		if (wave == 0) {
			if (lane == 0) {
				s = __hip_atomic_fetch_add(&gs->next_strip, 1, __ATOMIC_RELAXED, MM2GB_AGENT);
				tab[seq & 7] = s;
				__hip_atomic_store(&tab[8], seq + 1, __ATOMIC_RELEASE, __HIP_MEMORY_SCOPE_WORKGROUP);
			}
			s = first_lane(s);
		} else {
			while (first_lane(__hip_atomic_load(&tab[8], __ATOMIC_ACQUIRE, __HIP_MEMORY_SCOPE_WORKGROUP)) <= seq) __builtin_amdgcn_s_sleep(2);
			s = first_lane(tab[seq & 7]);
		}
		if (s * STRIP_TILES >= n_tiles) { ++seq; break; }
		s2 = s1; s1 = s0; s0 = s;
		const int pr = s * GANG_STRIP_PAIRS + wave;
		if (tpu * pr >= n_tiles) continue;
		const int ta = tpu * pr, i0 = cs + ta * WAVE;
		cur = ta;
		TilePair t = load_pair(b, i0, tpu == 2 ? ce : min(ce, i0 + WAVE));
		int jb = cs + ((t.lo_a - cs) & ~(WAVE - 1));
		const int eq_lo = jb < i0 ? equal_x_run_start(b, cs, i0, first_lane(t.A.x)) : i0;
		bool have = false;
		int nf = 0;
		for (; jb < i0; jb += WAVE) {
			const int sq = a_span(b, jb + lane);
			const int k = (jb - cs) / WAVE;
			if (tpu == 1 && wave > 0 && jb + WAVE == i0 && !P.lut_clamp && known <= k) {
				const int rs = (int)((unsigned)k % (unsigned)n_slots);
				sweep_block_by_quarters(b, t.A, jb, t.lo_a > jb ? t.lo_a - jb : 0, sq, stage, P, t.best_a, t.arg_a, [&]() { return ring[rs * WAVE + lane]; },
				                        [&](int q) {
					while (known <= k) {
						known = max(known, first_lane(__hip_atomic_load(&sh->done, __ATOMIC_ACQUIRE, __HIP_MEMORY_SCOPE_WORKGROUP)));
						if (known > k || first_lane(__hip_atomic_load(&sh->part, __ATOMIC_ACQUIRE, __HIP_MEMORY_SCOPE_WORKGROUP)) >= 4 * k + q + 1) break;
						__builtin_amdgcn_s_sleep(MM2GB_QUARTER_POLL_SLEEP);
					}
				});
				have = false;
				continue;
			}
			wait_done(k + 1);
			int sf;
			if (in_ring(k)) sf = ring[(unsigned)k % (unsigned)n_slots * WAVE + lane];
			else sf = have ? nf : gload(&b.f[jb + lane]);
			have = jb + WAVE < i0 && known >= k + 2 && !in_ring(k + 1);
			if (have) nf = gload(&b.f[jb + WAVE + lane]);
			sweep_pair_block(b, t, jb, eq_lo, sf, sq, stage, P);
		}
// ... 45 lines not shown
			gstore(&gs->keep[0], keep.idx + 1); gstore(&gs->keep[1], keep.x); gstore(&gs->keep[2], keep.hi); gstore(&gs->keep[3], keep.y); gstore(&gs->keep[4], keep.tag); gstore(&gs->keep[5], keep.f);
		}
		drain_stores();
		wait_done_global(ta);
		if (lane == 0) gstore(&gs->done, now_done);
		known = max(known, now_done); known_global = max(known_global, now_done);
	}
}


template <int MODE, bool GANG>
__device__ __forceinline__ int team_phase(const DevBatch &b, const DevParams &P, const int *lut, int4 *stage, int *ring, const int ring_slots, CoopShared *teams,
                          const int32_t *list, const int n_list, const int cursor, const int wave, const int team_size,
                          int first = -1, const long long min_cost = 0)
{
	const int n_teams = SCORE_THREADS / WAVE / team_size;
	const int team = wave / team_size, team_wave = wave - team * team_size;
	const int slots = ring_slots / n_teams;
	int *my_ring = ring + team * slots * WAVE;
	CoopShared *sh = &teams[team];
	while (true) {
		const bool given = first >= 0 && team == 0;
		if (team_wave == 0 && lane_id() == 0) { sh->chunk = given ? first : atomicAdd(&b.counters[cursor], 1); sh->done = 0; sh->part = 0; sh->band = 0; sh->keep[0] = -1; }
		first = -1;
		team_barrier(sh, team_size);
		const int c = first_lane(sh->chunk);
		if (c >= n_list) return -1;
		const int ci = first_lane(list[c]);
		if (min_cost > 0 && b.chunk_cost[ci] < min_cost) return c;
		if (GANG && (b.chunk_track[ci] & 8)) { team_barrier(sh, team_size); continue; }
		const int cs = first_lane(b.chunk_start[ci]), ce = first_lane(b.chunk_end[ci]);
		const bool band_on = MODE == MODE_LUT && band_chunk(b, P, ci, cs, ce);
		if (MODE == MODE_LUT && team_size < SCORE_THREADS / WAVE) {
			if (b.chunk_track[ci] & 1) coop_chunk_pairs<true>(b, P, lut, stage, my_ring, slots, sh, cs, ce, team_wave, team_size, band_on);
			else coop_chunk_pairs<false>(b, P, lut, stage, my_ring, slots, sh, cs, ce, team_wave, team_size, band_on);
		} else {
			if (b.chunk_track[ci] & 1) coop_chunk<MODE, true>(b, P, lut, stage, my_ring, slots, sh, cs, ce, team_wave, team_size, band_on);
			else coop_chunk<MODE, false>(b, P, lut, stage, my_ring, slots, sh, cs, ce, team_wave, team_size, band_on);
		}
		team_barrier(sh, team_size);
	}
}


template <int MODE, bool GANG>
__global__ __launch_bounds__(SCORE_THREADS, 8) void k_score(DevBatch b, DevParams P, int host_mode, int ring_slots, int big_team, int whole_wg_pct)
{
	extern __shared__ __attribute__((aligned(16))) int smem[];
	const unsigned fl = b.flags[0];
	const int mode = (fl & FLAG_ANY_SEGID) ? MODE_GENERAL : (host_mode == MODE_LUT && (fl & FLAG_NO_LUT)) ? MODE_FAST : host_mode;
	if (mode != MODE) return;
	int *lut = smem + (MODE == MODE_LUT ? P.lut_base / 4 : 0);
	if (MODE == MODE_LUT && ((unsigned)(uintptr_t)(__attribute__((address_space(3))) int*)smem != 0u ||
	                         (size_t)ring_slots * WAVE * 4 + SCORE_THREADS * sizeof(int4) + N_TEAM_RECORDS * sizeof(CoopShared) + TAB_INTS * 4 > (size_t)LUT_LDS_BASE ||
	                         P.lut_base < LUT_LDS_BASE || P.lut_base + 4 * (P.lut_last + 1) != LUT_LDS_TOTAL)) __builtin_trap();
	int *ring = smem;
	int4 *stage = (int4*)(ring + ring_slots * WAVE) + (threadIdx.x / WAVE) * WAVE;
	CoopShared *teams = (CoopShared*)((int4*)(ring + ring_slots * WAVE) + SCORE_THREADS);
	if (MODE == MODE_LUT) for (int k = threadIdx.x; k <= P.lut_last; k += SCORE_THREADS) lut[k] = b.lut[k];
	if (threadIdx.x < N_TEAM_RECORDS) { teams[threadIdx.x].bar_count = 0; teams[threadIdx.x].bar_gen = 0; }
	int *gang_tab = (int*)(teams + N_TEAM_RECORDS);
	if (threadIdx.x == 0) gang_tab[8] = 0;
	__syncthreads();

	const int n_long = first_lane(b.counters[CNT_NLONG]), n_mid = first_lane(b.counters[CNT_NMID]);
	const int wave = first_lane(threadIdx.x / WAVE);
	if (b.dbg && threadIdx.x == 0) b.dbg[blockIdx.x * 4 + 0] = (long long)__builtin_amdgcn_s_memrealtime();
	int gang_seq = 0;
	const int n_gang = (GANG && MODE == MODE_LUT && b.gang_slots && ring_slots > 0) ? first_lane(b.counters[CNT_NGANG]) : 0;
	if constexpr (GANG && MODE == MODE_LUT) {
	auto gang_run = [&](int e, bool late) __attribute__((always_inline)) {
		CoopShared *sh = teams + N_SMALL_TEAMS + 2;
		GangSlot *gs = b.gang_slots + e;
		const int ci = first_lane(gs->chunk);
		const int cs = first_lane(b.chunk_start[ci]), ce = first_lane(b.chunk_end[ci]);
		if (threadIdx.x == 0) {
			int go = 1;
			if (late) {
				const int next = gload(&gs->next_strip), done = gload(&gs->done), n_tiles = (ce - cs + WAVE - 1) / WAVE;
				const int st_tiles = (gload(&gs->tiles_per_wave) == 2 ? 2 : 1) * GANG_STRIP_PAIRS;
				go = next * st_tiles < n_tiles && next * st_tiles - done < 4 * st_tiles;
			}
			sh->chunk = go; sh->done = 0; sh->part = 0; sh->band = 0; sh->keep[0] = -1;
		}
		team_barrier(sh, SCORE_THREADS / WAVE);
		const int go = first_lane(sh->chunk);
		if (go) {
			if (b.chunk_track[ci] & 1) gang_chunk_pairs<true>(b, P, lut, stage, ring, ring_slots, sh, gs, gang_tab, gang_seq, cs, ce, wave);
			else gang_chunk_pairs<false>(b, P, lut, stage, ring, ring_slots, sh, gs, gang_tab, gang_seq, cs, ce, wave);
		}
		team_barrier(sh, SCORE_THREADS / WAVE);
	};
	if (n_gang > 0) {
		for (int e = 0; e < n_gang; ++e) {
			const int fw = first_lane(b.gang_slots[e].first_wg), nw = first_lane(b.gang_slots[e].n_wg);
			if ((int)blockIdx.x >= fw && (int)blockIdx.x < fw + nw) { gang_run(e, false); break; }
		}
	}
	}
	if (ring_slots > 0) {
		int first = -1;
		for (int phase = 0; phase < 3; ++phase) {
			const bool whole = phase == 0, small = phase == 2;
			if (whole && !(big_team < SCORE_THREADS / WAVE && whole_wg_pct > 0)) continue;
			const long long share = whole ? max(1ll, (long long)(b.totals[2] / gridDim.x * whole_wg_pct / 100)) : 0;
			CoopShared *records = small ? teams : whole ? teams + N_SMALL_TEAMS + 2 : teams + N_SMALL_TEAMS;
			const int got = team_phase<MODE, GANG>(b, P, lut, stage, ring, ring_slots, records, small ? b.mid_list : b.long_list, small ? n_mid : n_long,
			                                 small ? CNT_MCURSOR : CNT_LCURSOR, wave, small ? SMALL_TEAM : whole ? SCORE_THREADS / WAVE : big_team,
			                                 whole || small ? -1 : first, share);
			if (whole) first = got;
			if (phase == 1 && b.dbg && lane_id() == 0) atomicMax((unsigned long long*)&b.dbg[blockIdx.x * 4 + 1], (unsigned long long)__builtin_amdgcn_s_memrealtime());
		}
	}
	if (b.dbg && lane_id() == 0) atomicMax((unsigned long long*)&b.dbg[blockIdx.x * 4 + 2], (unsigned long long)__builtin_amdgcn_s_memrealtime());
	const int n_chunks = b.counters[CNT_NCHUNK] - n_long - n_mid;
	while (true) {
		int c = 0;
		if (lane_id() == 0) c = atomicAdd(&b.counters[CNT_CURSOR], 1);
		c = first_lane(c);
		if (c >= n_chunks) break;
		const int ci = first_lane(b.order[c]);
		const int cs = first_lane(b.chunk_start[ci]), ce = first_lane(b.chunk_end[ci]);
		if (MODE == MODE_LUT) {
			const bool band_on = band_chunk(b, P, ci, cs, ce);
			if (b.chunk_track[ci] & 1) run_chunk_pairs<true>(b, P, lut, stage, cs, ce, band_on);
			else run_chunk_pairs<false>(b, P, lut, stage, cs, ce, band_on);
		} else {
			if (b.chunk_track[ci] & 1) run_chunk<MODE, true>(b, P, lut, stage, cs, ce);
			else run_chunk<MODE, false>(b, P, lut, stage, cs, ce);
		}
	}
	if (b.dbg && lane_id() == 0) atomicMax((unsigned long long*)&b.dbg[blockIdx.x * 4 + 3], (unsigned long long)__builtin_amdgcn_s_memrealtime());
}

void launch_window(const DevBatch &b, const DevParams &P, hipStream_t s)
{
	if (b.n <= 0) return;
	hipLaunchKernelGGL(k_block_reads, dim3((unsigned)((b.n_blocks + 255) / 256)), dim3(256), 0, s, b);
	hipLaunchKernelGGL(k_window, dim3((unsigned)b.n_blocks), dim3(PLAN_THREADS), 0, s, b, P);
}

void launch_plan(const DevBatch &b, const LaunchCfg &cfg, hipStream_t s)
{
	const int n_tiles = (int)((b.n_blocks + PLANNER_THREADS - 1) / PLANNER_THREADS);
	const int chunk_grid = (int)std::min<int64_t>(1024, (b.n_blocks + 255) / 256);
	(void)hipMemsetAsync(b.bins, 0, N_LISTS * COST_BINS * sizeof(int), s);
	hipLaunchKernelGGL(plan_tile_sums, dim3(n_tiles), dim3(PLANNER_THREADS), 0, s, b);
	hipLaunchKernelGGL(plan_tile_scan, dim3(1), dim3(PLANNER_THREADS), 0, s, b, n_tiles);
	hipLaunchKernelGGL(plan_emit, dim3(n_tiles), dim3(PLANNER_THREADS), 0, s, b);
	hipLaunchKernelGGL(plan_finish, dim3(chunk_grid), dim3(256), 0, s, b, cfg);
	hipLaunchKernelGGL(plan_bins, dim3(1), dim3(64), 0, s, b);
	hipLaunchKernelGGL(plan_scatter, dim3(chunk_grid), dim3(256), 0, s, b);
	if (b.gang_slots) hipLaunchKernelGGL(plan_gangs, dim3(1), dim3(256), 0, s, b, cfg);
}

void launch_build_lut(int *d_lut, const DevParams &P, hipStream_t s)
{
	hipLaunchKernelGGL(k_build_lut, dim3((LUT_ENTRIES + 255) / 256), dim3(256), 0, s, d_lut, P);
}

size_t score_lds_bytes(const DevParams &P, int host_mode, int ring_slots)
{
	const size_t front = (size_t)ring_slots * WAVE * 4 + (size_t)SCORE_THREADS * sizeof(int4) + N_TEAM_RECORDS * sizeof(CoopShared) + TAB_INTS * 4;
	if (host_mode != MODE_LUT) return front;
	return front <= (size_t)LUT_LDS_BASE ? (size_t)LUT_LDS_TOTAL : (size_t)1 << 30;
}

int score_set_lds_limit(size_t bytes)
{
	hipError_t e = hipFuncSetAttribute((const void*)k_score<MODE_LUT, false>, hipFuncAttributeMaxDynamicSharedMemorySize, (int)bytes);
	if (e == hipSuccess) e = hipFuncSetAttribute((const void*)k_score<MODE_LUT, true>, hipFuncAttributeMaxDynamicSharedMemorySize, (int)bytes);
	if (e == hipSuccess) e = hipFuncSetAttribute((const void*)k_score<MODE_FAST, false>, hipFuncAttributeMaxDynamicSharedMemorySize, (int)bytes);
	if (e == hipSuccess) e = hipFuncSetAttribute((const void*)k_score<MODE_GENERAL, false>, hipFuncAttributeMaxDynamicSharedMemorySize, (int)bytes);
	return e == hipSuccess ? 0 : -1;
}

void launch_score(const DevBatch &b, const DevParams &P, const LaunchCfg &cfg, hipStream_t s)
{
	if (b.n <= 0) return;
	const size_t lds = score_lds_bytes(P, cfg.host_mode, cfg.ring_slots);
	const size_t lds_general = score_lds_bytes(P, MODE_GENERAL, cfg.ring_slots);
	if (cfg.host_mode == MODE_LUT) {
		if (b.gang_slots) hipLaunchKernelGGL((k_score<MODE_LUT, true>), dim3(cfg.score_grid), dim3(SCORE_THREADS), lds, s, b, P, cfg.host_mode, cfg.ring_slots, cfg.big_team, cfg.whole_wg_pct);
		else hipLaunchKernelGGL((k_score<MODE_LUT, false>), dim3(cfg.score_grid), dim3(SCORE_THREADS), lds, s, b, P, cfg.host_mode, cfg.ring_slots, cfg.big_team, cfg.whole_wg_pct);
	}
	if (cfg.host_mode == MODE_FAST || cfg.host_mode == MODE_LUT) hipLaunchKernelGGL((k_score<MODE_FAST, false>), dim3(cfg.score_grid), dim3(SCORE_THREADS), lds, s, b, P, cfg.host_mode, cfg.ring_slots, cfg.big_team, cfg.whole_wg_pct);
	hipLaunchKernelGGL((k_score<MODE_GENERAL, false>), dim3(cfg.score_grid), dim3(SCORE_THREADS), lds_general, s, b, P, cfg.host_mode, cfg.ring_slots, cfg.big_team, cfg.whole_wg_pct);
}


constexpr int SKIP_THREADS = 256;
constexpr int SKIP_WAVES_PER_CU = 32;

__device__ __forceinline__ int load_past_cache(const int32_t *p) { return __hip_atomic_load(p, __ATOMIC_RELAXED, __HIP_MEMORY_SCOPE_AGENT); }
__device__ __forceinline__ int shift_in(int v, int first)
{
	int r = prev_lane(v);
	asm volatile("v_writelane_b32 %0, %1, 0" : "+v"(r) : "s"(first_lane(first)));
	return r;
}

struct SkipCand { int x, y, t, f, p, mk; };
__device__ __forceinline__ SkipCand skip_round_load(const DevBatch &b, const int32_t *mark, int top, int st_i, int l)
{
	SkipCand c = { 0, 0, 0, 0, -1, -1 };
	const int j = top - l;
	if (j >= st_i) {
		const uint4 e = b.raw[j];
		c.x = (int)e.x; c.y = (int)e.z; c.t = tag_of(e.w);
		c.f = load_past_cache(b.f + j);
		const int pr = load_past_cache(b.p + j);
		c.p = pr ? j - pr : -1;
		c.mk = load_past_cache(mark + j);
	}
	return c;
}

__global__ __launch_bounds__(SKIP_THREADS) void k_skip_fill(DevBatch b, DevParams P, int max_skip, int32_t *mark, unsigned long long *stats)
{
	const int l = lane_id();
	const int n_chunks = b.counters[CNT_NCHUNK], n_long = b.counters[CNT_NLONG], n_mid = b.counters[CNT_NMID];
	const unsigned long long reach = (unsigned long long)P.max_dist_x;
	for (;;) {
		int item = 0;
		if (l == 0) item = atomicAdd(&b.counters[CNT_CURSOR], 1);
		item = bcast(item, 0);
		if (item >= n_chunks) break;
		const int c = item < n_long ? b.long_list[item] : item < n_long + n_mid ? b.mid_list[item - n_long] : b.order[item - n_long - n_mid];
		const int cs = b.chunk_start[c], ce = b.chunk_end[c];
		const unsigned long long t_start = stats ? __builtin_amdgcn_s_memrealtime() : 0;
		unsigned long long n_rounds = 0, n_rescan = 0;
		int64_t r = b.blk_read[cs / PLAN_BLOCK];
		while (r + 1 < b.n_reads && b.offsets[r + 1] <= cs) ++r;
		int64_t next_read = r + 1 <= b.n_reads ? b.offsets[r + 1] : INT64_MAX;
		int rx = 0, ry = 0, rt = 0, rf = 0, rp = -1;
		int max_ii = -1, mi_x = 0, mi_y = 0, mi_tag = 0, mi_f = 0;
		unsigned long long mi_x64 = 0;
		uint4 nxt = b.raw[cs];
		int nxt_st = b.st[cs];
		for (int i = cs; i < ce; ++i) {
			const uint4 ai = nxt;
			const int st_i = min(max(nxt_st, cs), i);
			if (i + 1 < ce) { nxt = b.raw[i + 1]; nxt_st = b.st[i + 1]; }
			if (i >= next_read) {
				while (r + 1 < b.n_reads && b.offsets[r + 1] <= i) ++r;
				next_read = r + 1 <= b.n_reads ? b.offsets[r + 1] : INT64_MAX;
				max_ii = -1;
			}
			const int xi = (int)ai.x, yi = (int)ai.z, ti = tag_of(ai.w), segi = ti >> 8;
			const unsigned long long xi64 = (unsigned long long)ai.y << 32 | ai.x;
			int max_f = ti & 0xff, max_j = -1, n_skip = 0, end_j = st_i - 1;
			SkipCand nx = { 0, 0, 0, 0, -1, -1 };
			if (i - 1 - WAVE >= st_i) nx = skip_round_load(b, mark, i - 1 - WAVE, st_i, l);
			unsigned long long carry = 0;
			for (int top = i - 1; top >= st_i; top -= WAVE) {
				++n_rounds;
				const bool have = top - l >= st_i;
				SkipCand cu = { rx, ry, rt, rf, rp, -1 };
				if (top != i - 1) {
					cu = nx;
					if (top - WAVE >= st_i) nx = skip_round_load(b, mark, top - WAVE, st_i, l);
				}
				int sc = 0;
				const bool ok = have && pair_score<MODE_GENERAL>(xi, yi, segi, cu.x, cu.y, cu.t, P, nullptr, sc);
				const int val = sc + cu.f;
				const int pj = cu.p;
				const int below = wave_max_below(ok ? val : INT_MIN);
				const bool better = ok && val > max(max_f, below);
				const int to = top - pj;
				const unsigned long long offered = wave_or_u64(ok && pj >= 0 && to < WAVE ? 1ull << to : 0ull);
				const bool again = ok && !better && (cu.mk == i || (((offered | carry) >> l) & 1));
				const int count = wave_skip_counts(better ? -1 : again ? 1 : 0, better ? 0 : SKIP_NONE, n_skip);
				const unsigned long long ends = __ballot(again && count > max_skip);
				const int upto = ends ? __builtin_ctzll(ends) : WAVE;
				const unsigned long long got = __ballot(better) & (upto < WAVE ? (1ull << upto) - 1 : ~0ull);
				if (got) {
					const int last = 63 - __builtin_clzll(got);
					max_f = bcast(val, last); max_j = top - last;
				}
				if (ends) { end_j = top - upto; break; }
				n_skip = bcast(count, WAVE - 1);
				carry = wave_or_u64(ok && pj >= 0 && to >= WAVE && to < 2 * WAVE ? 1ull << (to - WAVE) : 0ull);
				if (ok && pj >= 0 && to >= 2 * WAVE) __hip_atomic_store(mark + pj, i, __ATOMIC_RELAXED, __HIP_MEMORY_SCOPE_AGENT);
			}
			if (max_ii < 0 || xi64 - mi_x64 > reach) {
				int best = INT_MIN, who = -1;
				for (int top = i - 1; top >= st_i; top -= WAVE) {
					++n_rescan;
					const int j = top - l;
					int fj = rf;
					if (top != i - 1) fj = j >= st_i ? load_past_cache(b.f + j) : INT_MIN;
					else if (j < st_i) fj = INT_MIN;
					const int m = wave_max_i32_dpp(fj);
					if (m > best) { best = m; who = top - (int)__builtin_ctzll(__ballot(fj == m)); }
				}
				max_ii = who;
				if (who >= 0) {
					const uint4 e = b.raw[who];
					mi_x = (int)e.x; mi_y = (int)e.z; mi_tag = tag_of(e.w); mi_f = best;
					mi_x64 = (unsigned long long)e.y << 32 | e.x;
				}
			}
			if (max_ii >= 0 && max_ii < end_j) {
				int tmp = 0;
				if (pair_score<MODE_GENERAL>(xi, yi, segi, mi_x, mi_y, mi_tag, P, nullptr, tmp) && max_f < tmp + mi_f) { max_f = tmp + mi_f; max_j = max_ii; }
			}
// ... 23 lines not shown
```

### mm2-gb_amd/csrc/engine.h

```cpp
#pragma once
#include <hip/hip_runtime.h>
#include <stdint.h>
#include <functional>
#include <string>
#include <vector>
#include "../../include/mm2gb_chain.h"
#include "chain_dev.h"
#include "post_dev.h"
#include "seed_dev.h"

namespace mm2gb {

void set_error(const std::string &msg);
int  index_on_device(const mm2gb_index_t *ix, int device, DevIndexView *out);
void retire_device_buffer(void *ptr, size_t bytes);
int  fail(const std::string &msg);

#define MM2GB_HIP(call)                                                                                        \
	do {                                                                                                       \
		hipError_t e_ = (call);                                                                                \
		if (e_ != hipSuccess)                                                                                  \
			return ::mm2gb::fail(std::string(#call) + ": " + hipGetErrorString(e_));                           \
	} while (0)

struct DevBuf {
	void  *ptr = nullptr;
	size_t bytes = 0;
	int ensure(size_t need);
	void release();
};

void flush_retired_buffers();

struct PinnedBuf {
	void  *ptr = nullptr;
	size_t bytes = 0;
	int ensure(size_t need);
	void release();
};

struct IoSet {
	DevBuf raw, offsets, f, p;
	hipEvent_t in_start = nullptr, in_done = nullptr, comp_done = nullptr, out_start = nullptr, out_done = nullptr;
	bool used = false;
};

struct BatchSlot { hipEvent_t prep0 = nullptr, prep1 = nullptr, score1 = nullptr; };
constexpr int MAX_SLOTS = 256;

struct Engine {
	int device = 0;
	mm2gb_config_t cfg;
	mm2gb_misc_t   misc;
	DevParams      params;
	LaunchCfg      launch;
	hipStream_t    stream = nullptr;
	hipStream_t    s_in = nullptr, s_out = nullptr;
	bool           lean_streams = false;
	bool           counted_on_device = false;
	int            n_cu = 256;

	struct WorkSet {
		hipStream_t stream = nullptr;
		int64_t cap_n = 0, cap_reads = 0, cap_blocks = 0;
		DevBuf st;
		DevBuf blk_firstcut, blk_pairs, blk_clamped, blk_wmax, blk_read;
		DevBuf chunk_start, chunk_end, chunk_cost, chunk_track, order, long_list, mid_list;
		DevBuf chunk_pp, chunk_kk, chunk_blk, tile_sums, tile_base, bins;
		DevBuf counters, totals, flags;
		DevBuf gang_slots;
		DevBuf skip_mark;
		DevBuf skip_stats;
		DevBuf band_diag, band_res;
		std::vector<DevBuf*> all() { return { &st, &blk_firstcut, &blk_pairs, &blk_clamped, &blk_wmax, &blk_read, &chunk_start, &chunk_end, &chunk_cost,
		                                      &chunk_track, &order, &long_list, &mid_list, &chunk_pp, &chunk_kk, &chunk_blk, &tile_sums, &tile_base, &bins, &counters, &totals, &flags, &gang_slots, &skip_mark, &skip_stats, &band_diag, &band_res }; }
	};
	WorkSet work[2];
	DevBuf lut, dbg;
	int64_t cap_post_n = 0, cap_post_reads = 0;
	DevBuf post_dbg_tasks, post_dbg_stasks, rmq_dbg_reads, rmq_skey_in, rmq_skey, rmq_sa, rmq_srange, rmq_sort_tmp, post_z, post_fp, post_picked, post_utmp, post_heads, post_nu, post_nkept, post_misc, post_bins, post_order, post_up4, post_up16, post_sort_s, post_sort_perm, post_sort_tmp, post_cls, post_cls_cnt, post_cls_nz, post_read_nz, post_uloc, post_wtask, post_stask, rmq_tied, rmq_sum, rmq_by_y, rmq_ord, rmq_meta, rmq_win, rmq_tree, reg_out;
	DevBuf sd_seeds, sd_seed_off, sd_hit_off, sd_hits, sd_qlen, sd_q_rank, sd_ref_len, sd_ref_rank, sd_seed_read, sd_tmp, sd_n_kept, sd_a_off, sd_out;
	DevBuf sk_seqs, sk_seq_off, sk_rid, sk_mini, sk_mini_read, sk_mini_off, sk_work, sd_src_first, sd_mini_pos, sd_rep_len;
	DevBuf kw_jobs, kw_q, kw_t, kw_res, kw_slab, kw_cig, kw_img, kw_cnt, kw_off, kw_pack;
	double kw_ms[2] = { 0, 0 };
	DevBuf al_refs, al_reads, al_jobs, al_slices, al_list, al_drop;
	struct PostOut {
		DevBuf u_off, a_off, u_out, a_out;
		int64_t *h_totals = nullptr;
		hipEvent_t done = nullptr;
	} post_out[2];
	DevBuf &post_uoff = post_out[0].u_off, &post_aoff = post_out[0].a_off, &post_uout = post_out[0].u_out, &post_aout = post_out[0].a_out;
	int64_t *&h_post_totals = post_out[0].h_totals;
	hipEvent_t post0 = nullptr, post1 = nullptr;
	hipEvent_t post_fork = nullptr, post_join = nullptr;
	IoSet io[2];
	uint64_t io_seq = 0;
	PinnedBuf h_slice_off;
	std::vector<hipEvent_t> slice_in;
	PinnedBuf h_res_f, h_res_p;
	char    *h_small = nullptr;
	int32_t *h_counters = nullptr;
	int64_t *h_totals = nullptr;
	BatchSlot slots[MAX_SLOTS];
	int n_slots = 0;

	mm2gb_stats_t last = {};
	bool misc_valid = false, coop_disabled = false, debug_phases = false, one_compute_stream = false;
	int64_t team4_min_n = 0;
	int64_t gang_max_n = 0;
	int64_t last_gang_chunks = 0, last_gang_wgs = 0;
	bool rmq_tiles_last = false;
	std::function<void(const int32_t*)> rmq_tied_ready;
	hipEvent_t rmq_fill_done = nullptr;
	int  rmq_team_reads = 0;
	bool rmq_abandon_tied = false;
	bool rmq_calibrate = false;
	int  rmq_kernel = 0;
	bool lds_contract_ok = false;
	int64_t dual_stream_max_n = 16 * 1000 * 1000;
	bool chain_skip = false;
	int64_t last_band_groups[2] = { 0, 0 };
	int  last_score_form = 0;
	bool skip_stats = false;
	int  last_skip_set = 0;

	int  init(const mm2gb_config_t *cfg, const mm2gb_misc_t *misc, int device);
	void shutdown();
	int  set_misc(const mm2gb_misc_t *m);
	int  configure_score();
	int  reserve(int64_t n_anchors, int64_t n_reads, int set = 0);
	int  begin_call();
	int  enqueue_host(int64_t n_reads, const int64_t *h_offsets, const mm2gb_anchor_t *h_anchors, int64_t n, int32_t *h_f, int32_t *h_p, bool want_stats = true);
	int  enqueue(int64_t n_reads, const int64_t *d_offsets, const mm2gb_anchor_t *d_anchors, int64_t n, int32_t *d_f, int32_t *d_p, bool want_stats = true, int set = 0);
	int  score_host(int64_t n_reads, const int64_t *offsets, const mm2gb_anchor_t *anchors, int32_t *f, int32_t *p,
	                const std::function<void(int64_t, int64_t)> *slice_done);
	int  reserve_post(int64_t n_anchors, int64_t n_reads);
	int  reserve_post_out(int set, int64_t n_anchors, int64_t n_reads);
	void print_post_debug(int64_t n_reads);
	int  enqueue_post(int64_t n_reads, const int64_t *d_offsets, const mm2gb_anchor_t *d_anchors, int64_t n, const int32_t *d_f, const int32_t *d_p,
	                  const mm2gb_rmq_param_t *rmq = nullptr, int out_set = 0);
	int  enqueue_host_chains(int64_t n_reads, const int64_t *h_offsets, const mm2gb_anchor_t *h_anchors, int64_t n, int out_set, bool want_stats = false);
	int  fetch_chains(int out_set, int64_t n_reads, mm2gb_chains_t *out);
	int  chain_gpu(int64_t n_reads, const int64_t *offsets, const mm2gb_anchor_t *anchors, mm2gb_chains_t *out,
	               const mm2gb_rmq_param_t *rmq = nullptr, int32_t *n_tied = nullptr);
	int  chain_gpu_sliced(int64_t n_reads, const int64_t *offsets, const mm2gb_anchor_t *anchors, mm2gb_chains_t *out, int64_t slice);
	int  collect_seeds(int64_t opt_flag, int64_t n_reads, const int64_t *seed_off, const mm2gb_seed_t *seeds, const int64_t *hit_off, const uint64_t *hits,
	                   const int32_t *qlen, const int32_t *q_rank, int32_t n_ref, const int32_t *ref_len, const int32_t *ref_rank, int64_t *anchor_off, mm2gb_anchor_t *anchors);
	int  sketch_device(int w, int k, int flag, int64_t n_seqs, const int64_t *seq_off, const char *seqs, const uint32_t *rid, int64_t *n_mini);
	int  collect_matches_device(const DevIndexView &ix, const mm2gb_seed_opt_t &opt, int64_t n_reads, const int64_t *seq_off, const char *seqs, int64_t *n_seeds, int64_t *n_hits);
	int  collect_seeds_resident(int64_t opt_flag, int64_t n_reads, int64_t n_seeds, int64_t n_hits, int64_t *anchor_off, mm2gb_anchor_t *anchors);
	int  sort_seeds(int64_t n_reads, const int64_t *offsets, mm2gb_anchor_t *anchors);
	int  gen_regs(int64_t n_reads, const mm2gb_chains_t *chains, const int32_t *qlen, const uint32_t *hash, int is_qstrand, mm2gb_reg_t *regs);
	int  record_outputs_done(hipEvent_t ev);
	int  sync();
	int  collect_stats();
};

}

struct mm2gb_engine { mm2gb::Engine e; void *host_scratch = nullptr; void (*host_scratch_free)(void*) = nullptr; };

namespace mm2gb {
int chain_batch_on_engine(mm2gb_engine_t *eng, int64_t n_reads, const int64_t *offsets, const mm2gb_anchor_t *anchors, int n_threads, mm2gb_chains_t *out, mm2gb_stats_t *stats);
}
```

### mm2-gb_amd/csrc/engine.hip

```cpp
#include <atomic>
#include <hip/hip_runtime.h>
#include <sys/mman.h>
#include <mutex>
#include <algorithm>
#include <chrono>
#include <cstdio>
#include <cstdlib>
#include <cstring>
#include <vector>
#include <string>
#include "engine.h"
#include "host_chain.h"

namespace mm2gb {

static thread_local std::string g_err;
void set_error(const std::string &msg) { g_err = msg; }
int fail(const std::string &msg) { g_err = msg; return -1; }
const char *last_error_cstr() { return g_err.c_str(); }

static size_t grown(size_t need, size_t have)
{
	return have == 0 ? need : std::max(need, have + have / 4);
}
// ... 317 lines not shown
	hipDeviceProp_t prop;
	MM2GB_HIP(hipGetDeviceProperties(&prop, device));
	n_cu = prop.multiProcessorCount > 0 ? prop.multiProcessorCount : 256;
	cfg = *c;
	launch.score_grid = cfg.score_kernel.short_griddim > 0 ? std::max(1, cfg.score_kernel.short_griddim / 4) : n_cu * 2;
	launch.long_min_window = 128;
	launch.long_min_cost = (int64_t)std::max(1, cfg.score_kernel.mid_seg_cutoff) * std::max(64, cfg.range_kernel.blockdim) * 1024;
	launch.wide_window = 1024;
	if (const char *v = getenv("MM2GB_LONG_MIN_WINDOW")) launch.long_min_window = std::max(1, atoi(v));
	if (const char *v = getenv("MM2GB_WIDE_WINDOW")) launch.wide_window = std::max(1, atoi(v));
	if (const char *v = getenv("MM2GB_LONG_MIN_COST")) launch.long_min_cost = std::max<int64_t>(1, atoll(v));
	launch.team4_all = 0; launch.team4_share_pct = 60; team4_min_n = 250000000;
	if (const char *v = getenv("MM2GB_TEAM4_ALL")) launch.team4_all = atoi(v) != 0;
	if (const char *v = getenv("MM2GB_TEAM4_SHARE_PCT")) launch.team4_share_pct = std::max(0, atoi(v));
	if (const char *v = getenv("MM2GB_TEAM4_MIN_ANCHORS")) team4_min_n = std::max<int64_t>(0, atoll(v));
	if (const char *v = getenv("MM2GB_DEBUG_PHASES")) debug_phases = *v && *v != '0';
	if (const char *v = getenv("MM2GB_CHAIN_SKIP")) chain_skip = strcmp(v, "keep") == 0;
	{ const char *v = getenv("MM2GB_SKIP_STATS"); skip_stats = v && *v && *v != '0'; }
	launch.gang_max = 8; launch.gang_pct = 150; gang_max_n = 150000000;
	if (const char *v = getenv("MM2GB_GANG_MAX")) launch.gang_max = std::max(0, std::min(64, atoi(v)));
	if (const char *v = getenv("MM2GB_GANG_PCT")) launch.gang_pct = std::max(1, atoi(v));
	launch.gang_pairs = 0;
	if (const char *v = getenv("MM2GB_GANG_PAIRS")) launch.gang_pairs = *v && *v != '0';
	if (const char *v = getenv("MM2GB_GANG_MAX_ANCHORS")) gang_max_n = std::max<int64_t>(0, atoll(v));
	if (debug_phases && dbg.ensure((size_t)launch.score_grid * 32)) return -1;
	const char *env = getenv("MM2GB_NO_COOP");
	coop_disabled = env && *env && *env != '0';
	{
		const int before = dev >= 0 && dev < MAX_COUNTED_DEVICES ? g_engines_on_device[dev].fetch_add(1) : 0;
		counted_on_device = dev >= 0 && dev < MAX_COUNTED_DEVICES;
		const char *v = getenv("MM2GB_LEAN_STREAMS");
		lean_streams = v && *v ? *v != '0' : before > 0;
	}
	MM2GB_HIP(hipStreamCreateWithFlags(&work[0].stream, hipStreamNonBlocking));
	if (lean_streams) work[1].stream = work[0].stream; else MM2GB_HIP(hipStreamCreateWithFlags(&work[1].stream, hipStreamNonBlocking));
	stream = work[0].stream;
	{ const char *v = getenv("MM2GB_ONE_COMPUTE_STREAM"); one_compute_stream = v && *v && *v != '0'; }
	if (const char *v = getenv("MM2GB_DUAL_STREAM_MAX")) dual_stream_max_n = std::max<int64_t>(0, atoll(v));
	if (lean_streams) s_in = work[0].stream; else MM2GB_HIP(hipStreamCreateWithFlags(&s_in, hipStreamNonBlocking));
	MM2GB_HIP(hipStreamCreateWithFlags(&s_out, hipStreamNonBlocking));
	for (IoSet &s : io)
		for (hipEvent_t *e : { &s.in_start, &s.in_done, &s.comp_done, &s.out_start, &s.out_done }) MM2GB_HIP(hipEventCreate(e));
	{
		const size_t need = (size_t)MAX_SLOTS * CNT_WORDS * sizeof(int32_t) + (size_t)MAX_SLOTS * 2 * sizeof(int64_t) + 2 * 64;
		h_small = (char*)pinned_alloc(need);
		if (!h_small) return fail("mm2gb: cannot allocate the engine's page-locked read-back block");
		h_counters = (int32_t*)h_small;
		h_totals = (int64_t*)(h_small + (size_t)MAX_SLOTS * CNT_WORDS * sizeof(int32_t));
		post_out[0].h_totals = (int64_t*)((char*)h_totals + (size_t)MAX_SLOTS * 2 * sizeof(int64_t));
		post_out[1].h_totals = post_out[0].h_totals + 8;
	}
	for (WorkSet &w : work) if (w.counters.ensure(CNT_WORDS * sizeof(int32_t)) || w.totals.ensure(4 * sizeof(int64_t)) || w.flags.ensure(4 * sizeof(unsigned))) return -1;
	{
		static std::mutex probe_lock;
		static int probed[64];
		std::lock_guard<std::mutex> g(probe_lock);
		const char *v = getenv("MM2GB_LDS_PROBE");
		int &state = probed[device & 63];
		if (v && atoi(v) == 0) lds_contract_ok = false;
		else { if (!state) state = probe_lds_contract(n_cu, stream) ? 1 : 2; lds_contract_ok = state == 1; }
	}
	if (set_misc(m)) return -1;
	return 0;
}

void Engine::shutdown()
{
	if (counted_on_device) { g_engines_on_device[device].fetch_sub(1); counted_on_device = false; }
	(void)hipSetDevice(device);
	for (hipStream_t s : { s_in, work[0].stream, work[1].stream, s_out }) if (s) (void)hipStreamSynchronize(s);
	flush_retired_buffers();
	for (WorkSet &w : work) { for (DevBuf *b : w.all()) b->release(); w.cap_n = w.cap_reads = w.cap_blocks = 0; }
	lut.release(); dbg.release();
	for (IoSet &s : io) {
		s.raw.release(); s.offsets.release(); s.f.release(); s.p.release();
		for (hipEvent_t *e : { &s.in_start, &s.in_done, &s.comp_done, &s.out_start, &s.out_done }) if (*e) { (void)hipEventDestroy(*e); *e = nullptr; }
		s.used = false;
	}
	for (BatchSlot &b : slots)
		for (hipEvent_t *e : { &b.prep0, &b.prep1, &b.score1 }) if (*e) { (void)hipEventDestroy(*e); *e = nullptr; }
	h_slice_off.release(); h_res_f.release(); h_res_p.release();
	for (hipEvent_t &e : slice_in) if (e) (void)hipEventDestroy(e);
	slice_in.clear();
	for (DevBuf *b : { &post_dbg_tasks, &post_dbg_stasks, &rmq_dbg_reads, &rmq_skey_in, &rmq_skey, &rmq_sa, &rmq_srange, &rmq_sort_tmp, &post_z, &post_fp, &post_picked, &post_utmp, &post_heads, &post_nu, &post_nkept, &post_misc, &post_bins, &post_order, &post_up4, &post_up16, &post_sort_s, &post_sort_perm, &post_sort_tmp, &post_cls, &post_cls_cnt, &post_cls_nz, &post_read_nz, &post_uloc, &post_wtask, &post_stask, &rmq_tied, &rmq_sum, &rmq_by_y, &rmq_ord, &rmq_meta, &rmq_win, &rmq_tree, &reg_out,
	                   &sd_seeds, &sd_seed_off, &sd_hit_off, &sd_hits, &sd_qlen, &sd_q_rank, &sd_ref_len, &sd_ref_rank, &sd_seed_read, &sd_tmp, &sd_n_kept, &sd_a_off, &sd_out,
	                   &sk_seqs, &sk_seq_off, &sk_rid, &sk_mini, &sk_mini_read, &sk_mini_off, &sk_work, &sd_src_first, &sd_mini_pos, &sd_rep_len,
	                   &kw_jobs, &kw_q, &kw_t, &kw_res, &kw_slab, &kw_cig, &kw_img, &kw_cnt, &kw_off, &kw_pack,
	                   &al_refs, &al_reads, &al_jobs, &al_slices, &al_list, &al_drop,
	                   &post_out[0].u_off, &post_out[0].a_off, &post_out[0].u_out, &post_out[0].a_out, &post_out[1].u_off, &post_out[1].a_off, &post_out[1].u_out, &post_out[1].a_out })
		b->release();
	cap_post_n = cap_post_reads = 0;
	for (PostOut &po : post_out) {
		po.h_totals = nullptr;
		if (po.done) { (void)hipEventDestroy(po.done); po.done = nullptr; }
	}
	for (hipEvent_t *e : { &post0, &post1, &post_fork, &post_join, &rmq_fill_done }) if (*e) { (void)hipEventDestroy(*e); *e = nullptr; }
	pinned_free(h_small);
	h_small = nullptr;
	if (lean_streams) { s_in = nullptr; work[1].stream = nullptr; }
	for (hipStream_t *s : { &s_in, &work[0].stream, &work[1].stream, &s_out }) if (*s) { (void)hipStreamDestroy(*s); *s = nullptr; }
	stream = nullptr;
	h_counters = nullptr; h_totals = nullptr;
}

int Engine::reserve(int64_t n, int64_t n_reads, int set)
{
	MM2GB_HIP(hipSetDevice(device));
	if (n >= ((int64_t)1 << 31) - 2 * PLAN_BLOCK) return fail("mm2gb: a micro-batch is limited to 2^31 anchors (got " + std::to_string(n) + ")");
	WorkSet &w = work[set];
	if (n > w.cap_n || n_reads > w.cap_reads) {
		MM2GB_HIP(hipStreamSynchronize(w.stream));
		const int64_t nn = std::max<int64_t>(std::max(n, w.cap_n), 1024);
		const int64_t nb = (nn + PLAN_BLOCK - 1) / PLAN_BLOCK + 1;
		const int64_t had_reads = w.cap_reads;
		w.cap_n = w.cap_blocks = w.cap_reads = 0;
		if (w.st.ensure(nn * 4)) return -1;
		if (w.blk_firstcut.ensure(nb * 4) || w.blk_pairs.ensure(nb * 8) || w.blk_clamped.ensure(nb * 4) || w.blk_wmax.ensure(nb * 8) || w.blk_read.ensure(nb * 4)) return -1;
		if (w.chunk_start.ensure(nb * 4) || w.chunk_end.ensure(nb * 4) || w.chunk_cost.ensure(nb * 8) || w.chunk_track.ensure(nb) ||
		    w.order.ensure(nb * 4) || w.long_list.ensure(nb * 4) || w.mid_list.ensure(nb * 4) || w.chunk_pp.ensure(nb * 8) || w.chunk_kk.ensure(nb * 4) || w.chunk_blk.ensure(nb * 4) ||
		    w.tile_sums.ensure((nb / 1024 + 2) * 24) || w.tile_base.ensure((nb / 1024 + 2) * 24) || w.bins.ensure(3 * PLAN_COST_BINS * 4)) return -1;
		w.cap_n = nn; w.cap_blocks = nb; w.cap_reads = std::max(had_reads, n_reads);
	}
	return 0;
}

int Engine::begin_call()
{
	if (n_slots > 0 && sync()) return -1;
	n_slots = 0;
	last = mm2gb_stats_t();
	last_gang_chunks = last_gang_wgs = 0;
	last_band_groups[0] = last_band_groups[1] = 0;
	return 0;
}

int Engine::enqueue(int64_t n_reads, const int64_t *d_offsets, const mm2gb_anchor_t *d_anchors, int64_t n, int32_t *d_f, int32_t *d_p, bool want_stats, int set)
{
	if (n < 0 || n_reads < 0) return fail("mm2gb: negative batch size");
	if (want_stats && n_slots >= MAX_SLOTS && sync()) return -1;
	if (reserve(n, n_reads, set)) return -1;
	WorkSet &w = work[set];
	hipStream_t stream = w.stream;
	DevBuf &st = w.st, &blk_firstcut = w.blk_firstcut, &blk_pairs = w.blk_pairs, &blk_clamped = w.blk_clamped, &blk_wmax = w.blk_wmax,
	       &blk_read = w.blk_read, &chunk_start = w.chunk_start, &chunk_end = w.chunk_end, &chunk_cost = w.chunk_cost, &chunk_track = w.chunk_track, &order = w.order,
	       &long_list = w.long_list, &mid_list = w.mid_list, &chunk_pp = w.chunk_pp, &chunk_kk = w.chunk_kk, &chunk_blk = w.chunk_blk, &tile_sums = w.tile_sums,
	       &tile_base = w.tile_base, &bins = w.bins, &counters = w.counters, &totals = w.totals, &flags = w.flags;
	const int slot = want_stats ? n_slots++ : 0;
	BatchSlot &bs = slots[slot];
	if (want_stats) for (hipEvent_t *e : { &bs.prep0, &bs.prep1, &bs.score1 }) if (!*e) MM2GB_HIP(hipEventCreate(e));
	DevBatch b;
	b.raw = (const uint4*)d_anchors; b.offsets = d_offsets; b.n = n; b.n_reads = n_reads;
	b.st = (int32_t*)st.ptr;
	b.f = d_f; b.p = d_p;
	b.diag = nullptr; b.band_res = nullptr;
	b.blk_firstcut = (int32_t*)blk_firstcut.ptr; b.blk_pairs = (int64_t*)blk_pairs.ptr; b.blk_clamped = (int32_t*)blk_clamped.ptr; b.blk_wmax = (int32_t*)blk_wmax.ptr; b.blk_read = (int32_t*)blk_read.ptr;
	b.n_blocks = (n + PLAN_BLOCK - 1) / PLAN_BLOCK;
	b.chunk_start = (int32_t*)chunk_start.ptr; b.chunk_end = (int32_t*)chunk_end.ptr; b.chunk_cost = (int64_t*)chunk_cost.ptr;
	b.chunk_track = (uint8_t*)chunk_track.ptr; b.order = (int32_t*)order.ptr; b.long_list = (int32_t*)long_list.ptr; b.mid_list = (int32_t*)mid_list.ptr;
	b.chunk_pp = (int64_t*)chunk_pp.ptr; b.chunk_kk = (int32_t*)chunk_kk.ptr; b.chunk_blk = (int32_t*)chunk_blk.ptr;
	b.tile_sums = (int64_t*)tile_sums.ptr; b.tile_base = (int64_t*)tile_base.ptr; b.bins = (int32_t*)bins.ptr;
	b.counters = (int32_t*)counters.ptr; b.totals = (int64_t*)totals.ptr; b.flags = (unsigned*)flags.ptr;
	b.lut = (const int32_t*)lut.ptr;
	b.dbg = debug_phases ? (int64_t*)dbg.ptr : nullptr;
	if (debug_phases) MM2GB_HIP(hipMemsetAsync(dbg.ptr, 0, (size_t)launch.score_grid * 32, stream));
	LaunchCfg cfg_now = launch;
	if (n < team4_min_n) cfg_now.team4_share_pct = 0;
	b.gang_slots = nullptr;
	if (launch.gang_max >= 2 && launch.host_mode == SCORE_MODE_LUT && launch.ring_slots > 0 && n > 0 && n <= gang_max_n) {
		if (w.gang_slots.ensure((size_t)GANG_MAX_CHUNKS * sizeof(GangSlot))) return -1;
		b.gang_slots = (GangSlot*)w.gang_slots.ptr;
	}

	MM2GB_HIP(hipMemsetAsync(counters.ptr, 0, CNT_WORDS * sizeof(int32_t), stream));
	MM2GB_HIP(hipMemsetAsync(totals.ptr, 0, 4 * sizeof(int64_t), stream));
	MM2GB_HIP(hipMemsetAsync(flags.ptr, 0, 4 * sizeof(unsigned), stream));
	if (want_stats) MM2GB_HIP(hipEventRecord(bs.prep0, stream));
	if (n > 0) {
		launch_window(b, params, stream);
		launch_plan(b, cfg_now, stream);
	}
	if (want_stats) MM2GB_HIP(hipEventRecord(bs.prep1, stream));
	const bool walk = chain_skip && misc.max_skip < misc.max_iter;
	last_score_form = walk ? 1 : 0;
	if (n > 0 && walk) {
		if (w.skip_mark.ensure((size_t)n * sizeof(int32_t))) return -1;
		if (skip_stats && w.skip_stats.ensure(SKIP_STAT_WORDS * sizeof(unsigned long long))) return -1;
		last_skip_set = set;
		launch_skip_fill(b, params, misc.max_skip, (int32_t*)w.skip_mark.ptr, skip_stats ? (unsigned long long*)w.skip_stats.ptr : nullptr, n_cu, stream);
	} else if (n > 0) {
		if (params.band_slab > 0 && launch.host_mode == SCORE_MODE_LUT) {
			if (w.band_diag.ensure((size_t)n * sizeof(int32_t)) || w.band_res.ensure((size_t)n * 2 * sizeof(int32_t))) return -1;
			b.diag = (int32_t*)w.band_diag.ptr; b.band_res = (int32_t*)w.band_res.ptr;
		}
		launch_score(b, params, cfg_now, stream);
	}
	if (want_stats) {
		MM2GB_HIP(hipEventRecord(bs.score1, stream));
		MM2GB_HIP(hipMemcpyAsync(h_counters + (size_t)slot * CNT_WORDS, counters.ptr, CNT_WORDS * sizeof(int32_t), hipMemcpyDeviceToHost, stream));
		MM2GB_HIP(hipMemcpyAsync(h_totals + (size_t)slot * 2, totals.ptr, 2 * sizeof(int64_t), hipMemcpyDeviceToHost, stream));
		last.n_anchors += n; last.n_reads += n_reads;
	}
	MM2GB_HIP(hipGetLastError());
	return 0;
}

int Engine::reserve_post(int64_t n, int64_t n_reads)
{
	MM2GB_HIP(hipSetDevice(device));
	for (PostOut &po : post_out) {
		if (!po.h_totals) return fail("mm2gb: engine not initialised");
		if (!po.done) MM2GB_HIP(hipEventCreateWithFlags(&po.done, hipEventDisableTiming));
	}
	for (hipEvent_t *e : { &post0, &post1 }) if (!*e) MM2GB_HIP(hipEventCreate(e));
	for (hipEvent_t *e : { &post_fork, &post_join }) if (!*e) MM2GB_HIP(hipEventCreateWithFlags(e, hipEventDisableTiming));
	if (n <= cap_post_n && n_reads <= cap_post_reads) return 0;
	MM2GB_HIP(hipStreamSynchronize(stream));
	const int64_t nn = std::max<int64_t>(std::max(n, cap_post_n), 1024), nr = std::max<int64_t>(std::max(n_reads, cap_post_reads), 16);
	cap_post_n = cap_post_reads = 0;
	const size_t chains = (size_t)(nn + nr);
	if (post_sort_s.ensure((size_t)nn + 16384) || post_sort_perm.ensure((size_t)nn * 4) || post_sort_tmp.ensure((size_t)nn * 8)) return -1;
	if (post_z.ensure((size_t)nn * 8) || post_fp.ensure((size_t)nn * 8) || post_picked.ensure((size_t)nn * 4) || post_utmp.ensure(chains * 8) ||
	    post_heads.ensure(chains * 16) || post_nu.ensure((size_t)nr * 4) || post_nkept.ensure((size_t)nr * 4) || post_misc.ensure(2048) || post_bins.ensure(2 * N_SIZE_CLASSES * 4) || post_order.ensure((size_t)nr * 4) ||
	    post_up4.ensure((size_t)nn * 4) || post_up16.ensure((size_t)nn * 4)) return -1;
	if (post_cls.ensure((size_t)nn) || post_cls_cnt.ensure((size_t)nr * N_TREE_CLASSES * 4) || post_cls_nz.ensure((size_t)nr * N_TREE_CLASSES * 4) || post_read_nz.ensure((size_t)nr * 4) ||
	    post_uloc.ensure(chains * 4) || post_wtask.ensure((size_t)nr * N_TREE_CLASSES * 4 * 2)) return -1;
	if (post_stask.ensure(((size_t)nn / 64 + (size_t)nr + 64) * (16 + 16 + 4))) return -1;
	cap_post_n = nn; cap_post_reads = nr;
	return 0;
}

int Engine::reserve_post_out(int set, int64_t n, int64_t n_reads)
{
	PostOut &po = post_out[set];
	const int64_t nn = std::max<int64_t>(n, 1024), nr = std::max<int64_t>(n_reads, 16);
	const size_t need_off = (size_t)(nr + 1) * 8, need_u = (size_t)(nn + nr) * 8, need_a = (size_t)nn * 16;
	if (po.u_off.bytes >= need_off && po.a_off.bytes >= need_off && po.u_out.bytes >= need_u && po.a_out.bytes >= need_a) return 0;
	MM2GB_HIP(hipStreamSynchronize(stream));
	MM2GB_HIP(hipStreamSynchronize(s_out));
	if (po.u_off.ensure(need_off) || po.a_off.ensure(need_off) || po.u_out.ensure(need_u) || po.a_out.ensure(need_a)) return -1;
	return 0;
}

int Engine::enqueue_post(int64_t n_reads, const int64_t *d_offsets, const mm2gb_anchor_t *d_anchors, int64_t n, const int32_t *d_f, const int32_t *d_p,
                         const mm2gb_rmq_param_t *rmq, int out_set)
{
	if (out_set < 0 || out_set > 1) return fail("mm2gb: post set out of range");
	if (reserve_post(n, n_reads) || reserve_post_out(out_set, n, n_reads)) return -1;
	PostOut &po = post_out[out_set];
	PostBatch b;
	b.raw = (const uint4*)d_anchors; b.offsets = d_offsets; b.n = n; b.n_reads = n_reads; b.f = d_f; b.p = d_p;
	b.z = (unsigned long long*)post_z.ptr; b.fp = (int2*)post_fp.ptr; b.picked = (int32_t*)post_picked.ptr;
	b.up4 = (int32_t*)post_up4.ptr; b.up16 = (int32_t*)post_up16.ptr;
	b.sort_s = (unsigned char*)post_sort_s.ptr; b.sort_perm = (int32_t*)post_sort_perm.ptr; b.sort_tmp = (unsigned long long*)post_sort_tmp.ptr;
	b.u_tmp = (unsigned long long*)post_utmp.ptr; b.heads = (ulonglong2*)post_heads.ptr;
	b.n_u = (int32_t*)post_nu.ptr; b.n_kept = (int32_t*)post_nkept.ptr; b.u_off = (int64_t*)po.u_off.ptr; b.a_off = (int64_t*)po.a_off.ptr;
	b.u_out = (unsigned long long*)po.u_out.ptr; b.a_out = (uint4*)po.a_out.ptr;
	b.totals = (int64_t*)post_misc.ptr; b.cursor = (int32_t*)((char*)post_misc.ptr + 16);
	b.order = (int32_t*)post_order.ptr; b.size_bins = (int32_t*)post_bins.ptr;
	b.cls = (unsigned char*)post_cls.ptr;
	b.cls_cnt = (int32_t*)post_cls_cnt.ptr; b.cls_nz = (int32_t*)post_cls_nz.ptr; b.read_nz = (int32_t*)post_read_nz.ptr;
	b.zc = (unsigned long long*)post_sort_tmp.ptr; b.kpos = (int32_t*)post_sort_perm.ptr; b.u_loc = (int32_t*)post_uloc.ptr;
	b.wtask = (int32_t*)post_wtask.ptr; b.wtask_order = b.wtask + (size_t)std::max<int64_t>(cap_post_reads, 16) * N_TREE_CLASSES;
	{
		const size_t cap = (size_t)cap_post_n / 64 + (size_t)cap_post_reads + 64;
		b.stask[0] = (int4*)post_stask.ptr; b.stask[1] = b.stask[0] + cap;
		b.stask_order = (int32_t*)(b.stask[0] + 2 * cap);
	}
	b.walk_grid_waves = n_cu * 4 * 8;
	if (const char *v = getenv("MM2GB_WALK_WAVES")) b.walk_grid_waves = std::max(4, atoi(v));
	b.sort_pairs = 1;
	if (const char *v = getenv("MM2GB_SORT_PAIRS")) b.sort_pairs = atoi(v) != 0;
	b.dbg = debug_phases ? (long long*)((char*)post_misc.ptr + 1024) : nullptr;
	if (debug_phases) { MM2GB_HIP(hipMemsetAsync((char*)post_misc.ptr + 1024, 0, 512, stream)); MM2GB_HIP(hipMemsetAsync((char*)post_misc.ptr + 1024 + 22 * 8, 0xff, 8, stream)); }
	if (debug_phases) {
		if (post_dbg_tasks.ensure((size_t)std::max<int64_t>(n_reads, 1) * N_TREE_CLASSES * 64)) return -1;
		MM2GB_HIP(hipMemsetAsync(post_dbg_tasks.ptr, 0, (size_t)std::max<int64_t>(n_reads, 1) * N_TREE_CLASSES * 64, stream));
	}
	b.dbg_tasks = debug_phases ? (long long*)post_dbg_tasks.ptr : nullptr;
	if (debug_phases && post_dbg_stasks.ensure((size_t)262144 * 32)) return -1;
	b.dbg_stasks = debug_phases ? (long long*)post_dbg_stasks.ptr : nullptr;
	b.min_cnt = misc.min_cnt; b.min_sc = misc.min_score;
	b.max_drop = misc.is_cdna ? INT_MAX : misc.bw;
	if (rmq) { b.min_cnt = rmq->min_cnt; b.min_sc = rmq->min_sc; b.max_drop = rmq->bw; }
	b.grid_waves = n_cu * 32;
	if (const char *v = getenv("MM2GB_POST_WAVES")) b.grid_waves = std::max(4, atoi(v));
	MM2GB_HIP(hipEventRecord(post0, stream));
	launch_post(b, n_cu, stream, !lean_streams && work[1].stream && work[1].stream != stream ? work[1].stream : nullptr, post_fork, post_join);
	MM2GB_HIP(hipEventRecord(post1, stream));
	MM2GB_HIP(hipMemcpyAsync(po.h_totals, post_misc.ptr, 2 * sizeof(int64_t), hipMemcpyDeviceToHost, stream));
	MM2GB_HIP(hipEventRecord(po.done, stream));
	MM2GB_HIP(hipGetLastError());
	return 0;
}

int Engine::enqueue_host_chains(int64_t n_reads, const int64_t *h_offsets, const mm2gb_anchor_t *h_anchors, int64_t n, int out_set, bool want_stats)
{
	MM2GB_HIP(hipSetDevice(device));
	IoSet &s = io[io_seq++ & 1];
	const size_t nn = (size_t)std::max<int64_t>(n, 1);
	if (s.raw.bytes < nn * 16 || s.f.bytes < nn * 4 || s.p.bytes < nn * 4 || s.offsets.bytes < (size_t)(n_reads + 1) * 8) {
		for (hipStream_t q : { s_in, work[0].stream, work[1].stream, s_out }) MM2GB_HIP(hipStreamSynchronize(q));
		if (s.raw.ensure(nn * 16) || s.f.ensure(nn * 4) || s.p.ensure(nn * 4) || s.offsets.ensure((size_t)(n_reads + 1) * 8)) return -1;
	}
	if (s.used) MM2GB_HIP(hipStreamWaitEvent(s_in, s.comp_done, 0));
	MM2GB_HIP(hipMemcpyAsync(s.offsets.ptr, h_offsets, (size_t)(n_reads + 1) * 8, hipMemcpyHostToDevice, s_in));
	if (n > 0) MM2GB_HIP(hipMemcpyAsync(s.raw.ptr, h_anchors, (size_t)n * 16, hipMemcpyHostToDevice, s_in));
	MM2GB_HIP(hipEventRecord(s.in_done, s_in));
	MM2GB_HIP(hipStreamWaitEvent(stream, s.in_done, 0));
	if (s.used) { MM2GB_HIP(hipStreamWaitEvent(stream, s.out_done, 0)); MM2GB_HIP(hipStreamWaitEvent(stream, s.comp_done, 0)); }
	if (enqueue(n_reads, (const int64_t*)s.offsets.ptr, (const mm2gb_anchor_t*)s.raw.ptr, n, (int32_t*)s.f.ptr, (int32_t*)s.p.ptr, want_stats, 0)) return -1;
	if (enqueue_post(n_reads, (const int64_t*)s.offsets.ptr, (const mm2gb_anchor_t*)s.raw.ptr, n, (const int32_t*)s.f.ptr, (const int32_t*)s.p.ptr, nullptr, out_set)) return -1;
	MM2GB_HIP(hipEventRecord(s.comp_done, stream));
	MM2GB_HIP(hipEventRecord(s.out_done, stream));
	s.used = true;
	return 0;
}

int Engine::fetch_chains(int out_set, int64_t n_reads, mm2gb_chains_t *out)
{
	memset(out, 0, sizeof(*out));
	MM2GB_HIP(hipSetDevice(device));
	PostOut &po = post_out[out_set];
	MM2GB_HIP(hipEventSynchronize(po.done));
	const int64_t n_u = n_reads > 0 ? po.h_totals[0] : 0, n_a = n_reads > 0 ? po.h_totals[1] : 0;
	out->u_off = (int64_t*)malloc((size_t)(n_reads + 1) * 8);
	out->a_off = (int64_t*)malloc((size_t)(n_reads + 1) * 8);
	out->u = (uint64_t*)malloc((size_t)(n_u + 1) * 8);
	out->a = (mm2gb_anchor_t*)result_alloc_pinned((size_t)(n_a + 1) * 16);
	if (!out->u_off || !out->a_off || !out->u || !out->a) { free(out->u_off); free(out->a_off); free(out->u); result_release(out->a); memset(out, 0, sizeof(*out)); return fail("mm2gb: out of host memory"); }
	out->u_off[0] = out->a_off[0] = 0;
	if (n_reads > 0) {
		MM2GB_HIP(hipMemcpyAsync(out->u_off, po.u_off.ptr, (size_t)(n_reads + 1) * 8, hipMemcpyDeviceToHost, s_out));
		MM2GB_HIP(hipMemcpyAsync(out->a_off, po.a_off.ptr, (size_t)(n_reads + 1) * 8, hipMemcpyDeviceToHost, s_out));
		if (n_u > 0) MM2GB_HIP(hipMemcpyAsync(out->u, po.u_out.ptr, (size_t)n_u * 8, hipMemcpyDeviceToHost, s_out));
		if (n_a > 0) MM2GB_HIP(hipMemcpyAsync(out->a, po.a_out.ptr, (size_t)n_a * 16, hipMemcpyDeviceToHost, s_out));
		MM2GB_HIP(hipStreamSynchronize(s_out));
	}
	return 0;
}

int Engine::chain_gpu_sliced(int64_t n_reads, const int64_t *offsets, const mm2gb_anchor_t *anchors, mm2gb_chains_t *out, int64_t slice)
{
	const int64_t n = offsets[n_reads];
	if (begin_call()) return -1;
	const auto t0 = std::chrono::steady_clock::now();
	for (hipStream_t q : { s_in, work[0].stream, work[1].stream, s_out }) MM2GB_HIP(hipStreamSynchronize(q));
// ... 455 lines not shown
}

int Engine::collect_stats()
{
	if (debug_phases && n_slots > 0) {
		std::vector<int64_t> h((size_t)launch.score_grid * 4);
		if (hipMemcpy(h.data(), dbg.ptr, h.size() * 8, hipMemcpyDeviceToHost) == hipSuccess) {
			int64_t t0 = INT64_MAX, e1 = 0, e2 = 0, e3 = 0, s1 = 0, s2 = 0, s3 = 0; int n = 0;
			for (int w = 0; w < launch.score_grid; ++w) if (h[4 * w]) t0 = std::min(t0, h[4 * w]);
			for (int w = 0; w < launch.score_grid; ++w) {
				if (!h[4 * w]) continue;
				const int64_t a = h[4 * w + 1] ? h[4 * w + 1] - t0 : 0, b2 = h[4 * w + 2] - t0, c = h[4 * w + 3] - t0;
				e1 = std::max(e1, a); e2 = std::max(e2, b2); e3 = std::max(e3, c); s1 += a; s2 += b2; s3 += c; ++n;
			}
			if (n) fprintf(stderr, "[mm2gb phases] workgroups %d | end of big-team phase: mean %.2f max %.2f ms | end of 4-wave phase: mean %.2f max %.2f ms | end: mean %.2f max %.2f ms\n",
			               n, s1 / 1e5 / n, e1 / 1e5, s2 / 1e5 / n, e2 / 1e5, s3 / 1e5 / n, e3 / 1e5);
			if (n && e3 > 0) {
				int busy[8] = { 0 };
				for (int w = 0; w < launch.score_grid; ++w) if (h[4 * w]) for (int k = 0; k < 8; ++k) busy[k] += h[4 * w + 3] - t0 > e3 * k / 8;
				fprintf(stderr, "[mm2gb phases] workgroups still at work after 0/8 ... 7/8 of the kernel's time: %d %d %d %d %d %d %d %d\n", busy[0], busy[1], busy[2], busy[3], busy[4], busy[5], busy[6], busy[7]);
			}
		}
	}
	for (int k = 0; k < n_slots; ++k) {
		const int32_t *c = h_counters + (size_t)k * CNT_WORDS;
		last.n_pairs += h_totals[(size_t)k * 2];
		last.n_chunks += c[CNT_NCHUNK];
		last.n_long_chunks += c[CNT_NLONG];
		last.n_mid_chunks += c[CNT_NMID];
		last.n_tracked_chunks += c[CNT_NTRACK];
		last.n_clamped_blocks += c[CNT_NCLAMP];
		last_gang_chunks += c[CNT_NGANG]; last_gang_wgs += c[CNT_GANG_WGS];
		last_band_groups[0] += c[CNT_BAND_WAVE]; last_band_groups[1] += c[CNT_BAND_TEAM];
		float ms = 0;
		if (hipEventElapsedTime(&ms, slots[k].prep0, slots[k].prep1) == hipSuccess) last.ms_prep += ms;
		if (hipEventElapsedTime(&ms, slots[k].prep1, slots[k].score1) == hipSuccess) last.ms_score += ms;
	}
	if (n_slots > 0) last.ms_total = last.ms_prep + last.ms_score;
	n_slots = 0;
	return 0;
}

int Engine::score_host(int64_t n_reads, const int64_t *offsets, const mm2gb_anchor_t *anchors, int32_t *f, int32_t *p,
                       const std::function<void(int64_t, int64_t)> *slice_done)
{
	const int64_t base = offsets[0], n = offsets[n_reads] - base;
	for (int64_t r = 0; r < n_reads; ++r) if (offsets[r + 1] < offsets[r]) return fail("mm2gb_score_host: offsets must be non-decreasing");
	if (n > 0 && (!anchors || !f || !p)) return fail("mm2gb_score_host: null buffer");
	MM2GB_HIP(hipSetDevice(device));
	if (begin_call()) return -1;
	const auto t0 = std::chrono::steady_clock::now();
	int64_t slice = 96 * 1000 * 1000;
	if (const char *v = getenv("MM2GB_SLICE_ANCHORS")) slice = std::max<int64_t>(1, atoll(v));
	std::vector<int64_t> first(1, 0);
	if (n > slice + slice / 2) {
		int64_t tail = slice / 4;
		if (const char *v = getenv("MM2GB_SLICE_TAIL_ANCHORS")) tail = std::max<int64_t>(1, atoll(v));
		int64_t first_slice = slice;
		if (const char *v = getenv("MM2GB_SLICE_FIRST_ANCHORS")) first_slice = std::max<int64_t>(1, atoll(v));
		int64_t acc = 0;
		bool tail_cut = false;
		for (int64_t r = 0; r < n_reads; ++r) {
			acc += offsets[r + 1] - offsets[r];
			const int64_t left = offsets[n_reads] - offsets[r + 1];
			if (r + 1 >= n_reads || tail_cut) continue;
			if (left <= tail && acc > tail) { first.push_back(r + 1); acc = 0; tail_cut = true; }
			else if (acc >= (first.size() == 1 ? first_slice : slice) && left > tail + slice / 4) { first.push_back(r + 1); acc = 0; }
		}
	}
	first.push_back(n_reads);
	const size_t n_sl = first.size() - 1;
	auto drain = [&]() {
		const std::string why = last_error_cstr();
		for (hipStream_t q : { s_in, work[0].stream, work[1].stream, s_out }) (void)hipStreamSynchronize(q);
		n_slots = 0;
		set_error(why);
	};
	if (h_slice_off.ensure(((size_t)n_reads + n_sl + 1) * 8)) return -1;
	int64_t *lo = (int64_t*)h_slice_off.ptr;
	size_t w = 0;
	for (size_t k = 0; k < n_sl; ++k) {
		const int64_t r0 = first[k], r1 = first[k + 1];
		const size_t at = w;
		for (int64_t r = r0; r <= r1; ++r) lo[w++] = offsets[r] - offsets[r0];
		if (enqueue_host(r1 - r0, lo + at, anchors + offsets[r0], offsets[r1] - offsets[r0], f + (offsets[r0] - base), p + (offsets[r0] - base))) { drain(); return -1; }
		if (slice_done && k > 0) {
			if (hipEventSynchronize(io[(io_seq - 2) & 1].out_done) != hipSuccess) { drain(); return fail("mm2gb_score_host: waiting for a slice failed"); }
			(*slice_done)(first[k - 1], first[k]);
		}
	}
	if (sync()) return -1;
	if (slice_done) (*slice_done)(first[n_sl - 1], first[n_sl]);
	last.ms_total = std::chrono::duration<float, std::milli>(std::chrono::steady_clock::now() - t0).count();
	{
		const IoSet &s = io[(io_seq - 1) & 1];
		float ms = 0;
		if (hipEventElapsedTime(&ms, s.in_start, s.in_done) == hipSuccess) last.ms_h2d = ms;
		if (hipEventElapsedTime(&ms, s.out_start, s.out_done) == hipSuccess) last.ms_d2h = ms;
	}
	return 0;
}

}

using namespace mm2gb;

extern "C" {

const char *mm2gb_last_error(void) { return last_error_cstr(); }
void mm2gb_engine_gang_counts(const mm2gb_engine_t *eng, int64_t *chunks, int64_t *workgroups)
{
	if (chunks) *chunks = eng ? eng->e.last_gang_chunks : 0;
	if (workgroups) *workgroups = eng ? eng->e.last_gang_wgs : 0;
}
const char *mm2gb_version(void) { return MM2GB_VERSION; }
int mm2gb_has_gang_build(void) { return 1; }

int mm2gb_device_count(void)
{
	int n = 0;
	if (hipGetDeviceCount(&n) != hipSuccess) return 0;
	return n;
}

mm2gb_engine_t *mm2gb_engine_create(const mm2gb_config_t *cfg, const mm2gb_misc_t *misc, int device)
{
	mm2gb_config_t def;
	if (!cfg) { mm2gb_config_defaults(&def); cfg = &def; }
	if (!misc) { set_error("mm2gb_engine_create: misc is required"); return nullptr; }
	mm2gb_engine_t *eng = new mm2gb_engine_t();
	if (eng->e.init(cfg, misc, device)) { eng->e.shutdown(); delete eng; return nullptr; }
	return eng;
}

void mm2gb_engine_destroy(mm2gb_engine_t *eng)
{
	if (!eng) return;
	eng->e.shutdown();
	if (eng->host_scratch && eng->host_scratch_free) eng->host_scratch_free(eng->host_scratch);
	delete eng;
}

int mm2gb_engine_set_misc(mm2gb_engine_t *eng, const mm2gb_misc_t *misc) { return eng ? eng->e.set_misc(misc) : fail("mm2gb: null engine"); }
int mm2gb_engine_device(const mm2gb_engine_t *eng) { return eng ? eng->e.device : -1; }
int mm2gb_engine_set_rmq_team_reads(mm2gb_engine_t *eng, int n) { if (!eng || n < 0) return fail("mm2gb_engine_set_rmq_team_reads: bad argument"); eng->e.rmq_team_reads = n; return 0; }
int mm2gb_engine_set_chain_skip(mm2gb_engine_t *eng, int keep) { if (!eng || keep < 0 || keep > 1) return fail("mm2gb_engine_set_chain_skip: bad argument"); eng->e.chain_skip = keep == 1; return 0; }
int mm2gb_engine_last_score_form(const mm2gb_engine_t *eng) { return eng ? eng->e.last_score_form : -1; }
int mm2gb_engine_band_groups(const mm2gb_engine_t *eng, int64_t *out)
{
	if (!eng || !out) return fail("mm2gb_engine_band_groups: null argument");
	out[0] = eng->e.last_band_groups[0]; out[1] = eng->e.last_band_groups[1];
	return 0;
}
int mm2gb_engine_skip_stats(mm2gb_engine_t *eng, int64_t *out)
{
	if (!eng || !out) return fail("mm2gb_engine_skip_stats: null argument");
	Engine &e = eng->e;
	if (!e.skip_stats || !e.work[e.last_skip_set].skip_stats.ptr) return fail("mm2gb_engine_skip_stats: no counters (MM2GB_SKIP_STATS=1 when the engine is made, then a call that ran the walk)");
	if (e.sync()) return -1;
	unsigned long long v[SKIP_STAT_WORDS];
	MM2GB_HIP(hipMemcpy(v, e.work[e.last_skip_set].skip_stats.ptr, sizeof v, hipMemcpyDeviceToHost));
	out[0] = (int64_t)v[0]; out[1] = (int64_t)v[1]; out[2] = (int64_t)v[2];
	out[3] = (int64_t)(v[3] >> 24); out[4] = (int64_t)(v[3] & ((1u << 24) - 1)); out[5] = (int64_t)(v[5] - ~v[4]);
	return 0;
}
int mm2gb_engine_set_rmq_kernel(mm2gb_engine_t *eng, int kind) { if (!eng || kind < 0 || kind > 1) return fail("mm2gb_engine_set_rmq_kernel: bad argument"); eng->e.rmq_kernel = kind; return 0; }
int mm2gb_engine_reserve(mm2gb_engine_t *eng, int64_t n_anchors, int64_t n_reads) { return eng ? eng->e.reserve(n_anchors, n_reads) : fail("mm2gb: null engine"); }
void *mm2gb_engine_stream(mm2gb_engine_t *eng) { return eng ? (void*)eng->e.stream : nullptr; }
float mm2gb_engine_last_kernel_ms(mm2gb_engine_t *eng) { return eng ? eng->e.last.ms_prep + eng->e.last.ms_score : 0.f; }

int mm2gb_score_device(mm2gb_engine_t *eng, int64_t n_reads, const int64_t *d_offsets, const mm2gb_anchor_t *d_anchors,
                       int64_t n_anchors, int32_t *d_f, int32_t *d_p)
{
	if (!eng) return fail("mm2gb: null engine");
	Engine &e = eng->e;
	MM2GB_HIP(hipSetDevice(e.device));
	if (e.begin_call()) return -1;
	return e.enqueue(n_reads, d_offsets, d_anchors, n_anchors, d_f, d_p);
}

int mm2gb_engine_sync(mm2gb_engine_t *eng) { return eng ? eng->e.sync() : fail("mm2gb: null engine"); }

int mm2gb_chain_gpu(mm2gb_engine_t *eng, int64_t n_reads, const int64_t *offsets, const mm2gb_anchor_t *anchors, mm2gb_chains_t *out, mm2gb_stats_t *stats)
{
	if (!eng || !out) return fail("mm2gb_chain_gpu: null argument");
	if (eng->e.chain_gpu(n_reads, offsets, anchors, out)) return -1;
	if (stats) *stats = eng->e.last;
	return 0;
}

void Engine::print_post_debug(int64_t n_reads)
{
	long long t[64] = { 0 };
	if (hipMemcpy(t, (char*)post_misc.ptr + 1024, sizeof(t), hipMemcpyDeviceToHost) == hipSuccess)
		for (int lv = 0; lv < 3; ++lv)
			fprintf(stderr, "[mm2gb post-pass] sort level %d: %.1f ms; %lld radix passes over %lld elements: %lld cycles, %lld steps, refills of one line %lld, of all lines %lld\n",
			        lv, t[13 + lv] / 1e5, t[24 + 6 * lv + 5], t[24 + 6 * lv + 4], t[24 + 6 * lv + 3], t[24 + 6 * lv], t[24 + 6 * lv + 1], t[24 + 6 * lv + 2]);
	if (t[21])
		fprintf(stderr, "[mm2gb post-pass] walks: %lld tasks, first starts at 0, last ends at %.2f ms; summed %.1f ms, longest task %.2f ms; spec loads %.1f ms, long walks %.1f ms; groups %lld, open %lld, long %lld (%lld rounds)\n",
		        t[21], (t[23] - t[22]) / 1e5, t[2] / 1e5, t[5] / 1e5, t[7] / 1e5, t[8] / 1e5, t[9], t[10], t[11], t[20]);
	if (t[21])
		fprintf(stderr, "[mm2gb post-pass] wave-time summed over reads: collect %.1f ms | sort %.1f ms | chain walks %.1f ms | emit %.1f ms  (%lld reads) | longest sort task %.2f ms, walk task %.2f ms\n",
		        t[0] / 1e5, t[1] / 1e5, t[2] / 1e5, t[3] / 1e5, (long long)n_reads, t[4] / 1e5, t[5] / 1e5);
	if (t[42] > 0 && post_dbg_stasks.ptr) {
		const size_t n_t = (size_t)std::min<long long>(t[42], 262144);
		std::vector<long long> tk(n_t * 4);
		if (hipMemcpy(tk.data(), post_dbg_stasks.ptr, tk.size() * 8, hipMemcpyDeviceToHost) == hipSuccess) {
			auto ph12 = [](long long v) { return (double)((v & 511) << (2 * (v >> 9 & 7))); };
			for (int lv = 0; lv < 4; ++lv) {
				std::vector<size_t> idx;
				long long first = LLONG_MAX, last = 0, sum = 0;
				for (size_t k = 0; k < n_t; ++k) if ((int)(tk[4 * k + 2] >> 32) == lv) { idx.push_back(k); first = std::min(first, tk[4 * k]); last = std::max(last, tk[4 * k + 1]); sum += tk[4 * k + 1] - tk[4 * k]; }
				if (idx.empty()) continue;
				std::sort(idx.begin(), idx.end(), [&](size_t a, size_t b2) { return tk[4 * a + 1] - tk[4 * a] > tk[4 * b2 + 1] - tk[4 * b2]; });
				fprintf(stderr, "[mm2gb post-pass] k_post_sort_level %d: %zu tasks, %.2f ms from the first start to the last end, %.1f ms summed; the longest (elements | start | ms):", lv, idx.size(), (last - first) / 1e5, sum / 1e5);
				for (size_t k = 0; k < std::min<size_t>(idx.size(), 6); ++k) {
					const long long phv = tk[4 * idx[k] + 3];
					fprintf(stderr, "  %lld | %.2f | %.2f (histogram %.2f, set-up %.2f, walk %.2f of %lld steps, move %.2f)", tk[4 * idx[k] + 2] & 0xffffffffLL, (tk[4 * idx[k]] - first) / 1e5, (tk[4 * idx[k] + 1] - tk[4 * idx[k]]) / 1e5,
					        ph12(phv) / 1e5, ph12(phv >> 12) / 1e5, ph12(phv >> 24) / 1e5, phv >> 48 & 0xfffff, ph12(phv >> 36) / 1e5);
				}
				{
					const long long edge[4] = { 1792, 3584, 7168, LLONG_MAX };
					const char *name[4] = { "up to 1 792 elements", "up to 3 584", "up to 7 168 (resident)", "longer" };
					for (int c = 0; c < 4; ++c) {
						long long sdt = 0, sel = 0, sst = 0, sp[4] = { 0, 0, 0, 0 }; size_t nn = 0;
						for (size_t k : idx) {
							const long long len = tk[4 * k + 2] & 0xffffffffLL, dt = tk[4 * k + 1] - tk[4 * k], phv = tk[4 * k + 3];
							if (len > edge[c] || (c > 0 && len <= edge[c - 1])) continue;
							++nn; sdt += dt; sel += len; sst += phv >> 48 & 0xfffff;
							for (int q = 0; q < 4; ++q) sp[q] += ph12(phv >> (12 * q));
						}
						if (nn) fprintf(stderr, "\n    %s: %zu tasks, %lld elements, %lld steps, %.1f ms summed (histogram %.1f, set-up %.1f, walk %.1f, move %.1f)", name[c], nn, sel, sst, sdt / 1e5, sp[0] / 1e5, sp[1] / 1e5, sp[2] / 1e5, sp[3] / 1e5);
					}
				}
				fprintf(stderr, "\n    tasks in flight at 14 points of its time:");
				for (int kb = 0; kb < 14; ++kb) { const double at = first + (double)(last - first) * (kb + 0.5) / 14; int busy = 0; for (size_t k : idx) if (tk[4 * k] <= at && at < tk[4 * k + 1]) ++busy; fprintf(stderr, " %d", busy); }
				fprintf(stderr, "\n");
			}
		}
	}
	if (t[21] > 0 && post_dbg_tasks.ptr) {
		const size_t n_t = (size_t)t[21];
		std::vector<long long> tk(n_t * 8);
		if (hipMemcpy(tk.data(), post_dbg_tasks.ptr, tk.size() * 8, hipMemcpyDeviceToHost) == hipSuccess) {
			std::vector<size_t> idx(n_t);
			for (size_t k = 0; k < n_t; ++k) idx[k] = k;
			std::sort(idx.begin(), idx.end(), [&](size_t a, size_t b2) { return tk[8 * a + 1] - tk[8 * a] > tk[8 * b2 + 1] - tk[8 * b2]; });
			fprintf(stderr, "[mm2gb post-pass] k_post_walk: the longest tasks (taken as | read | class | candidates | start | ms | of which look-ahead loads | long walks | how many | rounds):\n");
			for (size_t k = 0; k < std::min<size_t>(n_t, 16); ++k) {
				const size_t q = idx[k];
				fprintf(stderr, "    %6zu | %6lld | %2lld | %7lld | %6.2f | %6.2f | %6.2f | %6.2f | %lld | %lld\n", q, tk[8 * q + 2] >> 4, tk[8 * q + 2] & 15, tk[8 * q + 3], (tk[8 * q] - t[22]) / 1e5, (tk[8 * q + 1] - tk[8 * q]) / 1e5, tk[8 * q + 4] / 1e5, tk[8 * q + 5] / 1e5, tk[8 * q + 6], tk[8 * q + 7]);
			}
			const int n_bins = 14;
			std::vector<int> busy(n_bins, 0);
			const double span = std::max(1.0, (double)(t[23] - t[22]));
			for (size_t q = 0; q < n_t; ++q) for (int k = 0; k < n_bins; ++k) { const double at = t[22] + span * (k + 0.5) / n_bins; if (tk[8 * q] <= at && at < tk[8 * q + 1]) ++busy[k]; }
			fprintf(stderr, "    tasks in flight at %d points of the kernel's time:", n_bins);
			for (int k = 0; k < n_bins; ++k) fprintf(stderr, " %d", busy[k]);
			fprintf(stderr, "\n");
		}
	}
}

int mm2gb_rmq_chain_gpu(mm2gb_engine_t *eng, const mm2gb_rmq_param_t *prm, int64_t n_reads, const int64_t *offsets, const mm2gb_anchor_t *anchors,
                        mm2gb_chains_t *out, int32_t *n_tied, mm2gb_stats_t *stats)
{
	if (!eng || !out || !prm) return fail("mm2gb_rmq_chain_gpu: null argument");
	if (prm->max_dist < 0 || prm->bw < 0 || prm->cap_rmq_size < 0) return fail("mm2gb_rmq_chain_gpu: negative parameter");
	if (eng->e.chain_gpu(n_reads, offsets, anchors, out, prm, n_tied)) return -1;
	if (stats) *stats = eng->e.last;
	return 0;
}

int mm2gb_sort_seeds_gpu(mm2gb_engine_t *eng, int64_t n_reads, const int64_t *offsets, mm2gb_anchor_t *anchors)
{
	return eng ? eng->e.sort_seeds(n_reads, offsets, anchors) : fail("mm2gb: null engine");
}

int mm2gb_collect_seeds_gpu(mm2gb_engine_t *eng, int64_t opt_flag, int64_t n_reads, const int64_t *seed_off, const mm2gb_seed_t *seeds,
                            const int64_t *hit_off, const uint64_t *hits, const int32_t *qlen, const int32_t *q_rank,
                            int32_t n_ref, const int32_t *ref_len, const int32_t *ref_rank, int64_t *anchor_off, mm2gb_anchor_t *anchors)
{
	return eng ? eng->e.collect_seeds(opt_flag, n_reads, seed_off, seeds, hit_off, hits, qlen, q_rank, n_ref, ref_len, ref_rank, anchor_off, anchors) : fail("mm2gb: null engine");
}

static int check_seq_off(const char *who, int64_t n, const int64_t *seq_off, const char *seqs)
{
	if (n < 0 || !seq_off) return fail(std::string(who) + ": null argument");
	if (seq_off[0] != 0) return fail(std::string(who) + ": seq_off[0] must be 0");
	for (int64_t r = 0; r < n; ++r) if (seq_off[r + 1] < seq_off[r]) return fail(std::string(who) + ": seq_off must be non-decreasing");
	if (seq_off[n] >= ((int64_t)1 << 31) - 1) return fail(std::string(who) + ": a batch is limited to 2^31 bases");
	if (seq_off[n] > 0 && !seqs) return fail(std::string(who) + ": null argument");
	return 0;
}

int mm2gb_sketch_gpu(mm2gb_engine_t *eng, int w, int k, int64_t n_seqs, const int64_t *seq_off, const char *seqs, const uint32_t *rid, int64_t *mini_off, uint64_t **out_xy)
{
	return mm2gb_sketch_gpu_flag(eng, w, k, 0, n_seqs, seq_off, seqs, rid, mini_off, out_xy);
}

int mm2gb_sketch_gpu_flag(mm2gb_engine_t *eng, int w, int k, int flag, int64_t n_seqs, const int64_t *seq_off, const char *seqs, const uint32_t *rid, int64_t *mini_off,
                          uint64_t **out_xy)
{
	if (!eng || !mini_off || !out_xy) return fail("mm2gb_sketch_gpu: null argument");
	if (flag & ~MM2GB_I_HPC) return fail("mm2gb_sketch_gpu: unknown flag (MM2GB_I_HPC only)");
	if (w < 1 || w > 255 || k < 1 || k > 28) return fail("mm2gb_sketch_gpu: bad arguments (0 < w < 256, 0 < k <= 28)");
// ... 152 lines not shown
```

Baseline: 7000 billion.

## Precompute banded slab sort order and diagonals in a separate pre-pass kernel

Adds a k_band_order kernel that runs before scoring. For each band slab it computes anchor diagonals, slab skip/index/sorted state and the bitonic-sorted visiting order, then writes them to device buffers. The score kernels now read the precomputed order and state instead of sorting inside the dependent chaining loop, and they drop their per-tile diagonal stores and atomic loads. This takes sort work off the critical inter-wave dependency path, at the cost of an extra launch plus extra global traffic and buffers. Host-side verification helpers are also added.

```diff
diff --git a/include/mm2gb_chain.h b/include/mm2gb_chain.h
--- a/include/mm2gb_chain.h
+++ b/include/mm2gb_chain.h
@@ -61,6 +61,10 @@
 int  mm2gb_engine_set_chain_skip(mm2gb_engine_t *eng, int keep);
 int  mm2gb_engine_last_score_form(const mm2gb_engine_t *eng);
 int  mm2gb_engine_band_groups(const mm2gb_engine_t *eng, int64_t *out);
+int  mm2gb_engine_band_order(mm2gb_engine_t *eng, int64_t n_anchors, int64_t cap_slabs, int32_t *slab_s0, int32_t *slab_n, int32_t *slab_cs,
+                             int32_t *slab_state, int64_t *n_slabs, uint16_t *order, int32_t *st);
+int  mm2gb_band_order_host(int64_t n, const int32_t *x, const int32_t *y, const int32_t *st, int slab, int lag, int bw,
+                           int32_t *slab_s0, int32_t *slab_n, int32_t *slab_state, uint16_t *order, int64_t *n_slabs);
 int  mm2gb_engine_skip_stats(mm2gb_engine_t *eng, int64_t *out6);
 int  mm2gb_engine_device(const mm2gb_engine_t *eng);
 void mm2gb_engine_gang_counts(const mm2gb_engine_t *eng, int64_t *chunks, int64_t *workgroups);
diff --git a/mm2-gb_amd/__init__.py b/mm2-gb_amd/__init__.py
--- a/mm2-gb_amd/__init__.py
+++ b/mm2-gb_amd/__init__.py
@@ -73,7 +73,7 @@
                 "mm2gb_batcher_create", "mm2gb_batcher_add", "mm2gb_batcher_feed", "mm2gb_batcher_flush", "mm2gb_batcher_stats", "mm2gb_batcher_destroy",
                 "mm2gb_plan_batches", "mm2gb_rmq_chain_gpu", "mm2gb_lchain_rmq", "mm2gb_lchain_rmq_counts",
                 "mm2gb_sort_seeds_gpu", "mm2gb_gen_regs_gpu", "mm2gb_collect_seeds_gpu",
-                "mm2gb_sketch", "mm2gb_index_build", "mm2gb_index_destroy", "mm2gb_index_size", "mm2gb_index_mid_occ", "mm2gb_collect_matches", "mm2gb_matches_free", "mm2gb_map_opt_init", "mm2gb_map_reads", "mm2gb_engine_release_host_scratch", "mm2gb_rmq_chain_host", "mm2gb_rmq_chain_host_tied", "mm2gb_rmq_chain", "mm2gb_engine_set_rmq_kernel", "mm2gb_engine_set_rmq_team_reads", "mm2gb_engine_set_chain_skip", "mm2gb_engine_last_score_form", "mm2gb_engine_band_groups", "mm2gb_collect_seeds_host", "mm2gb_map_reads_multi", "mm2gb_map_reads_stream",
+                "mm2gb_sketch", "mm2gb_index_build", "mm2gb_index_destroy", "mm2gb_index_size", "mm2gb_index_mid_occ", "mm2gb_collect_matches", "mm2gb_matches_free", "mm2gb_map_opt_init", "mm2gb_map_reads", "mm2gb_engine_release_host_scratch", "mm2gb_rmq_chain_host", "mm2gb_rmq_chain_host_tied", "mm2gb_rmq_chain", "mm2gb_engine_set_rmq_kernel", "mm2gb_engine_set_rmq_team_reads", "mm2gb_engine_set_chain_skip", "mm2gb_engine_last_score_form", "mm2gb_engine_band_groups", "mm2gb_engine_band_order", "mm2gb_band_order_host", "mm2gb_collect_seeds_host", "mm2gb_map_reads_multi", "mm2gb_map_reads_stream",
                 "mm2gb_sketch_gpu", "mm2gb_index_to_device", "mm2gb_collect_matches_gpu", "mm2gb_match_batch_free",
                 "mm2gb_index_build_gpu", "mm2gb_index_mid_occ_gpu", "mm2gb_index_view", "mm2gb_index_fetch_device", "mm2gb_index_build_split",
                 "mm2gb_sketch_flag", "mm2gb_sketch_gpu_flag", "mm2gb_index_build_flag", "mm2gb_index_build_gpu_flag", "mm2gb_index_flag",
@@ -245,6 +245,23 @@
     return node.value, list(buf[:min(n, 4096)])
 
 
+def band_order_host(x, y, st, slab, lag, bw):
+    L = lib()
+    L.mm2gb_band_order_host.argtypes = [C.c_int64] + [C.c_void_p] * 3 + [C.c_int] * 3 + [C.c_void_p] * 4 + [C.POINTER(C.c_int64)]
+    x, y, st = (np.ascontiguousarray(v, dtype=np.int32) for v in (x, y, st))
+    n = len(x)
+    if len(y) != n or len(st) != n:
+        raise ValueError("band_order_host: x, y and st must have one entry per anchor")
+    cap = n // int(slab) + 1 if int(slab) > 0 else 1
+    s0, cnt, state = (np.zeros(cap, dtype=np.int32) for _ in range(3))
+    order = np.zeros(max(n, 1), dtype=np.uint16)
+    ns = C.c_int64(0)
+    _check(L.mm2gb_band_order_host(n, x.ctypes.data, y.ctypes.data, st.ctypes.data, int(slab), int(lag), int(bw),
+                                   s0.ctypes.data, cnt.ctypes.data, state.ctypes.data, order.ctypes.data, C.byref(ns)))
+    k = int(ns.value)
+    return s0[:k], cnt[:k], state[:k], order[:n]
+
+
 class Engine:
 
     def __init__(self, misc=None, config=None, device=0, chain_skip=None):
@@ -285,6 +302,19 @@
         out = (C.c_int64 * 2)()
         _check(lib().mm2gb_engine_band_groups(self._h, out))
         return int(out[0]), int(out[1])
+
+    def band_order(self, n_anchors):
+        L = lib()
+        L.mm2gb_engine_band_order.argtypes = [C.c_void_p, C.c_int64, C.c_int64] + [C.c_void_p] * 4 + [C.POINTER(C.c_int64), C.c_void_p, C.c_void_p]
+        n = int(n_anchors)
+        cap = n // 128 + 1
+        s0, cnt, cs, state = (np.zeros(cap, dtype=np.int32) for _ in range(4))
+        order, st = np.zeros(n, dtype=np.uint16), np.zeros(n, dtype=np.int32)
+        ns = C.c_int64(0)
+        _check(L.mm2gb_engine_band_order(self._h, n, cap, s0.ctypes.data, cnt.ctypes.data, cs.ctypes.data, state.ctypes.data, C.byref(ns),
+                                         order.ctypes.data, st.ctypes.data))
+        k = min(int(ns.value), cap)
+        return {"s0": s0[:k], "n": cnt[:k], "cs": cs[:k], "state": state[:k], "order": order, "st": st}
 
     def skip_stats(self):
         L = lib()
diff --git a/mm2-gb_amd/csrc/band_order.h b/mm2-gb_amd/csrc/band_order.h
--- /dev/null
+++ b/mm2-gb_amd/csrc/band_order.h
@@ -0,0 +1,22 @@
+#pragma once
+#include <hip/hip_runtime.h>
+#include <stdint.h>
+
+namespace mm2gb {
+
+enum : int32_t { BAND_SLAB_SKIP = 0,
+                 BAND_SLAB_INDEX = 1,
+                 BAND_SLAB_SORTED = 2 };
+constexpr int BAND_MAX_SLAB = 512;
+
+__host__ __device__ inline bool band_slab_skipped(int st_min, int jl) { return st_min >= jl; }
+__host__ __device__ inline bool band_slab_in_index_order(unsigned range, int bw) { return range <= 2u * (unsigned)bw; }
+__host__ __device__ inline int band_key_shift(unsigned range)
+{
+	int sh = 0;
+	for (unsigned v = range >> 22; v; v >>= 1) ++sh;
+	return sh;
+}
+__host__ __device__ inline unsigned band_key(int d, int dmin, int sh, int e) { return (((unsigned)(d - dmin) >> sh) << 9) | (unsigned)e; }
+
+}
diff --git a/mm2-gb_amd/csrc/band_order_host.cpp b/mm2-gb_amd/csrc/band_order_host.cpp
--- /dev/null
+++ b/mm2-gb_amd/csrc/band_order_host.cpp
@@ -0,0 +1,43 @@
+#include <algorithm>
+#include <limits.h>
+#include <vector>
+#include "band_order.h"
+#include "engine.h"
+
+extern "C" int mm2gb_band_order_host(int64_t n, const int32_t *x, const int32_t *y, const int32_t *st, int slab, int lag, int bw,
+                                     int32_t *slab_s0, int32_t *slab_n, int32_t *slab_state, uint16_t *order, int64_t *n_slabs)
+{
+	using namespace mm2gb;
+	if (n < 0 || n > INT_MAX || (n > 0 && (!x || !y || !st || !order)) || !slab_s0 || !slab_n || !slab_state || !n_slabs) return fail("mm2gb_band_order_host: bad argument");
+	if ((slab != 128 && slab != 256 && slab != 512) || lag < 0 || lag > slab || lag % 64 != 0 || bw < 0) return fail("mm2gb_band_order_host: slab must be 128, 256 or 512, lag a multiple of 64 up to the slab");
+	int64_t ns = 0;
+	std::fill(order, order + n, (uint16_t)0);
+	std::vector<unsigned> key;
+	for (int64_t s0 = 0; s0 < n; s0 += slab) {
+		const int jl = (int)s0 - lag, len = (int)std::min<int64_t>(slab, n - s0);
+		if (jl <= 0) continue;
+		int dmin = INT_MAX, dmax = INT_MIN, st_min = INT_MAX;
+		for (int e = 0; e < len; ++e) {
+			const int d = (int)((unsigned)x[s0 + e] - (unsigned)y[s0 + e]);
+			dmin = std::min(dmin, d); dmax = std::max(dmax, d); st_min = std::min(st_min, st[s0 + e]);
+		}
+		const unsigned range = (unsigned)dmax - (unsigned)dmin;
+		int state = BAND_SLAB_SKIP;
+		key.resize(len);
+		for (int e = 0; e < len; ++e) key[e] = (unsigned)e;
+		if (!band_slab_skipped(st_min, jl)) {
+			state = BAND_SLAB_INDEX;
+			if (!band_slab_in_index_order(range, bw)) {
+				state = BAND_SLAB_SORTED;
+				const int sh = band_key_shift(range);
+				for (int e = 0; e < len; ++e) key[e] = band_key((int)((unsigned)x[s0 + e] - (unsigned)y[s0 + e]), dmin, sh, e);
+				std::sort(key.begin(), key.end());
+			}
+		}
+		for (int e = 0; e < len; ++e) order[s0 + e] = (uint16_t)(key[e] & (unsigned)(BAND_MAX_SLAB - 1));
+		slab_s0[ns] = (int32_t)s0; slab_n[ns] = len; slab_state[ns] = state;
+		++ns;
+	}
+	*n_slabs = ns;
+	return 0;
+}
diff --git a/mm2-gb_amd/csrc/chain_dev.h b/mm2-gb_amd/csrc/chain_dev.h
--- a/mm2-gb_amd/csrc/chain_dev.h
+++ b/mm2-gb_amd/csrc/chain_dev.h
@@ -54,6 +54,8 @@
 	int32_t  *f;
 	int32_t  *p;
 	int32_t  *diag;
+	uint16_t *band_order;
+	int32_t  *band_state;
 	int32_t  *band_res;
 	int32_t  *blk_firstcut;
 	int64_t  *blk_pairs;
@@ -104,6 +106,7 @@
 
 void launch_window(const DevBatch &b, const DevParams &P, hipStream_t s);
 void launch_plan(const DevBatch &b, const LaunchCfg &cfg, hipStream_t s);
+void launch_band_order(const DevBatch &b, const DevParams &P, const LaunchCfg &cfg, hipStream_t s);
 void launch_score(const DevBatch &b, const DevParams &P, const LaunchCfg &cfg, hipStream_t s);
 constexpr int SKIP_STAT_WORDS = 6;
 void launch_skip_fill(const DevBatch &b, const DevParams &P, int max_skip, int32_t *mark, unsigned long long *stats, int n_cu, hipStream_t s);
diff --git a/mm2-gb_amd/csrc/chain_kernels.hip b/mm2-gb_amd/csrc/chain_kernels.hip
--- a/mm2-gb_amd/csrc/chain_kernels.hip
+++ b/mm2-gb_amd/csrc/chain_kernels.hip
@@ -3,6 +3,7 @@
 #include <limits.h>
 #include <algorithm>
 #include "chain_dev.h"
+#include "band_order.h"
 #include "wave_scan.h"
 
 namespace mm2gb {
@@ -1384,11 +1385,11 @@
 		};
 		int sidx = 0, n_st = 0;
 		int jb = lo;
-		int dn = jb + lane < jl ? __hip_atomic_load(b.diag + jb + lane, __ATOMIC_RELAXED, __HIP_MEMORY_SCOPE_AGENT) : 0;
+		int dn = jb + lane < jl ? b.diag[jb + lane] : 0;
 		for (; jb < jl; jb += WAVE) {
 			const int j = jb + lane;
 			const int dj = dn;
-			dn = j + WAVE < jl ? __hip_atomic_load(b.diag + j + WAVE, __ATOMIC_RELAXED, __HIP_MEMORY_SCOPE_AGENT) : 0;
+			dn = j + WAVE < jl ? b.diag[j + WAVE] : 0;
 			const bool hit = j < jl && (unsigned)(dj - band_lo) <= width;
 			const unsigned long long m = __ballot(hit);
 			if (m == 0) continue;
@@ -1414,61 +1415,11 @@
 __device__ __forceinline__ int band_slab_part(const DevBatch &b, const DevParams &P, int4 *stage, const int s0, const int n, const int jl,
                                               const int g_from, const int g_to)
 {
-	constexpr int R = 8;
-	const int lane = lane_id();
-	unsigned key[R];
-	int lo = INT_MAX, hi = INT_MIN, st_lo = INT_MAX;
-#pragma unroll
-	for (int r = 0; r < R; ++r) {
-		const int e = r * WAVE + lane;
-		const int d = e < n ? a_x(b, s0 + e) - a_y(b, s0 + e) : 0;
-		if (e < n) { lo = min(lo, d); hi = max(hi, d); st_lo = min(st_lo, b.st[s0 + e]); }
-	}
-	if (wave_min_i32(st_lo) >= jl) return 0;
-	const int dmin = wave_min_i32(lo), dmax = wave_max_i32_dpp(hi);
-	const unsigned range = (unsigned)(dmax - dmin);
-	if (range <= 2u * (unsigned)P.bw) {
-#pragma unroll
-		for (int r = 0; r < R; ++r) key[r] = r * WAVE + lane < n ? (unsigned)(r * WAVE + lane) : ~0u;
-	} else {
-		const int sh = (range >> 22) ? 32 - __clz((int)(range >> 22)) : 0;
-#pragma unroll
-		for (int r = 0; r < R; ++r) {
-			const int e = r * WAVE + lane;
-			key[r] = e < n ? (((unsigned)(a_x(b, s0 + e) - a_y(b, s0 + e) - dmin) >> sh) << 9) | (unsigned)e : ~0u;
-		}
-#pragma unroll
-		for (int k = 2; k <= R * WAVE; k <<= 1) {
-#pragma unroll
-			for (int j = k >> 1; j > 0; j >>= 1) {
-				if (j >= WAVE) {
-					const int jr = j / WAVE;
-#pragma unroll
-					for (int r = 0; r < R; ++r) {
-						if (r & jr) continue;
-						const bool up = ((r * WAVE) & k) == 0;
-						const unsigned a = key[r], c = key[r | jr];
-						key[r] = up ? min(a, c) : max(a, c);
-						key[r | jr] = up ? max(a, c) : min(a, c);
-					}
-				} else {
-#pragma unroll
-					for (int r = 0; r < R; ++r) {
-						const unsigned o = (unsigned)__shfl_xor((int)key[r], j);
-						const bool up = ((r * WAVE + lane) & k) == 0, lower = (lane & j) == 0;
-						key[r] = up == lower ? min(key[r], o) : max(key[r], o);
-					}
-				}
-			}
-		}
-	}
+	if (first_lane(b.band_state[s0 >> 6]) == BAND_SLAB_SKIP) return 0;
 	int swept = 0;
-	for (int g = g_from; g < g_to; ++g) {
-		unsigned kg = key[0];
-#pragma unroll
-		for (int r = 1; r < R; ++r) kg = g == r ? key[r] : kg;
-		const int tgt = kg == ~0u ? -1 : s0 + (int)(kg & 511u);
-		if (__ballot(tgt >= 0) == 0) break;
+	for (int g = g_from; g < g_to && g * WAVE < n; ++g) {
+		const int e = g * WAVE + lane_id();
+		const int tgt = e < n ? s0 + (int)b.band_order[s0 + e] : -1;
 		swept += band_group(b, P, stage, tgt, jl);
 	}
 	return swept;
@@ -1493,10 +1444,95 @@
 	arg = take ? ba : arg;
 }
 
-__device__ __forceinline__ void band_store_diag(const DevBatch &b, const TilePair &t, const int i0)
-{
-	if (lane_id() < t.n_a) b.diag[i0 + lane_id()] = t.A.x - t.A.y;
-	if (lane_id() < t.n_b) b.diag[i0 + WAVE + lane_id()] = t.B.x - t.B.y;
+constexpr int BAND_ORDER_THREADS = 256;
+constexpr int BAND_ORDER_WINDOW = 512;
+
+__device__ __forceinline__ void band_order_slab(const DevBatch &b, const DevParams &P, const int s0, const int n, const int jl, const bool has_sources)
+{
+	constexpr int R = BAND_MAX_SLAB / WAVE;
+	const int lane = lane_id();
+	int d[R];
+	int lo = INT_MAX, hi = INT_MIN, st_lo = INT_MAX;
+#pragma unroll
+	for (int r = 0; r < R; ++r) {
+		const int e = r * WAVE + lane;
+		d[r] = 0;
+		if (e < n) {
+			const uint4 a = b.raw[s0 + e];
+			d[r] = (int)a.x - (int)a.z;
+			b.diag[s0 + e] = d[r];
+			lo = min(lo, d[r]); hi = max(hi, d[r]);
+			if (has_sources) st_lo = min(st_lo, b.st[s0 + e]);
+		}
+	}
+	if (!has_sources) return;
+	unsigned key[R];
+#pragma unroll
+	for (int r = 0; r < R; ++r) key[r] = r * WAVE + lane < n ? (unsigned)(r * WAVE + lane) : ~0u;
+	int state = BAND_SLAB_SKIP;
+	const int dmin = wave_min_i32(lo), dmax = wave_max_i32_dpp(hi);
+	const unsigned range = (unsigned)(dmax - dmin);
+	if (!band_slab_skipped(wave_min_i32(st_lo), jl)) {
+		state = BAND_SLAB_INDEX;
+		if (!band_slab_in_index_order(range, P.bw)) {
+			state = BAND_SLAB_SORTED;
+			const int sh = band_key_shift(range);
+#pragma unroll
+			for (int r = 0; r < R; ++r) key[r] = r * WAVE + lane < n ? band_key(d[r], dmin, sh, r * WAVE + lane) : ~0u;
+#pragma unroll
+			for (int k = 2; k <= R * WAVE; k <<= 1) {
+#pragma unroll
+				for (int j = k >> 1; j > 0; j >>= 1) {
+					if (j >= WAVE) {
+						const int jr = j / WAVE;
+#pragma unroll
+						for (int r = 0; r < R; ++r) {
+							if (r & jr) continue;
+							const bool up = ((r * WAVE) & k) == 0;
+							const unsigned a = key[r], c = key[r | jr];
+							key[r] = up ? min(a, c) : max(a, c);
+							key[r | jr] = up ? max(a, c) : min(a, c);
+						}
+					} else {
+#pragma unroll
+						for (int r = 0; r < R; ++r) {
+							const unsigned o = (unsigned)__shfl_xor((int)key[r], j);
+							const bool up = ((r * WAVE + lane) & k) == 0, lower = (lane & j) == 0;
+							key[r] = up == lower ? min(key[r], o) : max(key[r], o);
+						}
+					}
+				}
+			}
+		}
+	}
+#pragma unroll
+	for (int r = 0; r < R; ++r) if (r * WAVE + lane < n) b.band_order[s0 + r * WAVE + lane] = (uint16_t)(key[r] & (unsigned)(BAND_MAX_SLAB - 1));
+	if (lane == 0) b.band_state[s0 >> 6] = state;
+}
+
+__global__ __launch_bounds__(BAND_ORDER_THREADS) void k_band_order(DevBatch b, DevParams P, int host_mode)
+{
+	if (host_mode != MODE_LUT || (b.flags[0] & (FLAG_ANY_SEGID | FLAG_NO_LUT))) return;
+	const int n_chunks = first_lane(b.counters[CNT_NCHUNK]);
+	const long long a0 = ((long long)blockIdx.x * (BAND_ORDER_THREADS / WAVE) + threadIdx.x / WAVE) * BAND_ORDER_WINDOW;
+	if (a0 >= b.n || n_chunks <= 0) return;
+	const int a = first_lane((int)a0), a1 = first_lane((int)min((long long)b.n, a0 + BAND_ORDER_WINDOW));
+	int c_lo = 0, c_hi = n_chunks;
+	while (c_hi - c_lo > 1) {
+		const int mid = (c_lo + c_hi) >> 1;
+		if (first_lane(b.chunk_start[mid]) <= a) c_lo = mid; else c_hi = mid;
+	}
+	for (int ci = c_lo; ci < n_chunks; ++ci) {
+		const int cs = first_lane(b.chunk_start[ci]), ce = first_lane(b.chunk_end[ci]);
+		if (cs >= a1) break;
+		if (!band_chunk(b, P, ci, cs, ce)) continue;
+		const int end = min(a1, ce);
+		const long long k0 = cs >= a ? 0 : ((long long)a - cs + P.band_slab - 1) / P.band_slab;
+		for (long long s = cs + k0 * P.band_slab; s < end; s += P.band_slab) {
+			const int s0 = (int)s;
+			band_order_slab(b, P, s0, min(P.band_slab, ce - s0), s0 - P.band_lag, s0 - P.band_lag > cs);
+		}
+	}
 }
 
 template <bool TRACK>
@@ -1512,7 +1548,6 @@
 		int jb = cs + ((t.lo_a - cs) & ~(WAVE - 1));
 		const int s0 = band ? i0 - (i0 - cs) % P.band_slab : cs, jl = s0 - P.band_lag;
 		const bool in_band = band && jl > cs;
-		if (band) band_store_diag(b, t, i0);
 		if (in_band && i0 == s0) {
 			band_groups += band_slab_part(b, P, stage, s0, min(P.band_slab, ce - s0), jl, 0, P.band_slab / WAVE);
 			asm volatile("s_waitcnt vmcnt(0)" ::: "memory");
@@ -1618,7 +1653,6 @@
 		const int sl = t / tps, s0 = cs + sl * P.band_slab, jl = s0 - P.band_lag;
 		const bool in_band = band && jl > cs;
 		int *band_cnt = sl & 1 ? &sh->band : &sh->part;
-		if (band && T.live) b.diag[i0 + lane] = T.x - T.y;
 		if (in_band) {
 			const int part = t - sl * tps;
 			wait_done((jl - cs) / WAVE);
@@ -1688,7 +1722,6 @@
 		const int sl = pr / pps, s0 = cs + sl * P.band_slab, jl = s0 - P.band_lag;
 		const bool in_band = band && jl > cs;
 		int *band_cnt = sl & 1 ? &sh->band : &sh->part;
-		if (band) band_store_diag(b, t, i0);
 		if (in_band) {
 			const int part = pr - sl * pps;
 			wait_done((jl - cs) / WAVE);
@@ -2040,6 +2073,13 @@
 	hipLaunchKernelGGL(plan_bins, dim3(1), dim3(64), 0, s, b);
 	hipLaunchKernelGGL(plan_scatter, dim3(chunk_grid), dim3(256), 0, s, b);
 	if (b.gang_slots) hipLaunchKernelGGL(plan_gangs, dim3(1), dim3(256), 0, s, b, cfg);
+}
+
+void launch_band_order(const DevBatch &b, const DevParams &P, const LaunchCfg &cfg, hipStream_t s)
+{
+	if (b.n <= 0 || P.band_slab <= 0 || cfg.host_mode != MODE_LUT || !b.band_res || !b.band_order || !b.band_state || !b.diag) return;
+	const int64_t waves = (b.n + BAND_ORDER_WINDOW - 1) / BAND_ORDER_WINDOW, per_wg = BAND_ORDER_THREADS / WAVE;
+	hipLaunchKernelGGL(k_band_order, dim3((unsigned)((waves + per_wg - 1) / per_wg)), dim3(BAND_ORDER_THREADS), 0, s, b, P, cfg.host_mode);
 }
 
 void launch_build_lut(int *d_lut, const DevParams &P, hipStream_t s)
diff --git a/mm2-gb_amd/csrc/engine.h b/mm2-gb_amd/csrc/engine.h
--- a/mm2-gb_amd/csrc/engine.h
+++ b/mm2-gb_amd/csrc/engine.h
@@ -72,8 +72,9 @@
 		DevBuf skip_mark;
 		DevBuf skip_stats;
 		DevBuf band_diag, band_res;
+		DevBuf band_order, band_state;
 		std::vector<DevBuf*> all() { return { &st, &blk_firstcut, &blk_pairs, &blk_clamped, &blk_wmax, &blk_read, &chunk_start, &chunk_end, &chunk_cost,
-		                                      &chunk_track, &order, &long_list, &mid_list, &chunk_pp, &chunk_kk, &chunk_blk, &tile_sums, &tile_base, &bins, &counters, &totals, &flags, &gang_slots, &skip_mark, &skip_stats, &band_diag, &band_res }; }
+		                                      &chunk_track, &order, &long_list, &mid_list, &chunk_pp, &chunk_kk, &chunk_blk, &tile_sums, &tile_base, &bins, &counters, &totals, &flags, &gang_slots, &skip_mark, &skip_stats, &band_diag, &band_res, &band_order, &band_state }; }
 	};
 	WorkSet work[2];
 	DevBuf lut, dbg;
@@ -123,6 +124,8 @@
 	int  last_score_form = 0;
 	bool skip_stats = false;
 	int  last_skip_set = 0;
+	int  last_band_set = -1;
+	int64_t last_band_n = 0;
 
 	int  init(const mm2gb_config_t *cfg, const mm2gb_misc_t *misc, int device);
 	void shutdown();
diff --git a/mm2-gb_amd/csrc/engine.hip b/mm2-gb_amd/csrc/engine.hip
--- a/mm2-gb_amd/csrc/engine.hip
+++ b/mm2-gb_amd/csrc/engine.hip
@@ -493,7 +493,7 @@
 	b.raw = (const uint4*)d_anchors; b.offsets = d_offsets; b.n = n; b.n_reads = n_reads;
 	b.st = (int32_t*)st.ptr;
 	b.f = d_f; b.p = d_p;
-	b.diag = nullptr; b.band_res = nullptr;
+	b.diag = nullptr; b.band_res = nullptr; b.band_order = nullptr; b.band_state = nullptr;
 	b.blk_firstcut = (int32_t*)blk_firstcut.ptr; b.blk_pairs = (int64_t*)blk_pairs.ptr; b.blk_clamped = (int32_t*)blk_clamped.ptr; b.blk_wmax = (int32_t*)blk_wmax.ptr; b.blk_read = (int32_t*)blk_read.ptr;
 	b.n_blocks = (n + PLAN_BLOCK - 1) / PLAN_BLOCK;
 	b.chunk_start = (int32_t*)chunk_start.ptr; b.chunk_end = (int32_t*)chunk_end.ptr; b.chunk_cost = (int64_t*)chunk_cost.ptr;
@@ -516,23 +516,28 @@
 	MM2GB_HIP(hipMemsetAsync(totals.ptr, 0, 4 * sizeof(int64_t), stream));
 	MM2GB_HIP(hipMemsetAsync(flags.ptr, 0, 4 * sizeof(unsigned), stream));
 	if (want_stats) MM2GB_HIP(hipEventRecord(bs.prep0, stream));
+	const bool walk = chain_skip && misc.max_skip < misc.max_iter;
+	last_score_form = walk ? 1 : 0;
+	last_band_set = -1;
 	if (n > 0) {
 		launch_window(b, params, stream);
 		launch_plan(b, cfg_now, stream);
+		if (!walk && params.band_slab > 0 && launch.host_mode == SCORE_MODE_LUT) {
+			if (w.band_diag.ensure((size_t)n * sizeof(int32_t)) || w.band_res.ensure((size_t)n * 2 * sizeof(int32_t)) ||
+			    w.band_order.ensure((size_t)n * sizeof(uint16_t)) || w.band_state.ensure(((size_t)n / 64 + 1) * sizeof(int32_t))) return -1;
+			b.diag = (int32_t*)w.band_diag.ptr; b.band_res = (int32_t*)w.band_res.ptr;
+			b.band_order = (uint16_t*)w.band_order.ptr; b.band_state = (int32_t*)w.band_state.ptr;
+			launch_band_order(b, params, cfg_now, stream);
+			last_band_set = set; last_band_n = n;
+		}
 	}
 	if (want_stats) MM2GB_HIP(hipEventRecord(bs.prep1, stream));
-	const bool walk = chain_skip && misc.max_skip < misc.max_iter;
-	last_score_form = walk ? 1 : 0;
 	if (n > 0 && walk) {
 		if (w.skip_mark.ensure((size_t)n * sizeof(int32_t))) return -1;
 		if (skip_stats && w.skip_stats.ensure(SKIP_STAT_WORDS * sizeof(unsigned long long))) return -1;
 		last_skip_set = set;
 		launch_skip_fill(b, params, misc.max_skip, (int32_t*)w.skip_mark.ptr, skip_stats ? (unsigned long long*)w.skip_stats.ptr : nullptr, n_cu, stream);
 	} else if (n > 0) {
-		if (params.band_slab > 0 && launch.host_mode == SCORE_MODE_LUT) {
-			if (w.band_diag.ensure((size_t)n * sizeof(int32_t)) || w.band_res.ensure((size_t)n * 2 * sizeof(int32_t))) return -1;
-			b.diag = (int32_t*)w.band_diag.ptr; b.band_res = (int32_t*)w.band_res.ptr;
-		}
 		launch_score(b, params, cfg_now, stream);
 	}
 	if (want_stats) {
@@ -1294,6 +1299,51 @@
 	out[0] = eng->e.last_band_groups[0]; out[1] = eng->e.last_band_groups[1];
 	return 0;
 }
+int mm2gb_engine_band_order(mm2gb_engine_t *eng, int64_t n_anchors, int64_t cap_slabs, int32_t *slab_s0, int32_t *slab_n, int32_t *slab_cs,
+                            int32_t *slab_state, int64_t *n_slabs, uint16_t *order, int32_t *st)
+{
+	if (!eng || !n_slabs || cap_slabs < 0 || (cap_slabs > 0 && (!slab_s0 || !slab_n || !slab_cs || !slab_state))) return fail("mm2gb_engine_band_order: bad argument");
+	Engine &e = eng->e;
+	if (e.sync()) return -1;
+	*n_slabs = 0;
+	if (e.last_band_set < 0) return 0;
+	const Engine::WorkSet &w = e.work[e.last_band_set];
+	const int64_t n = e.last_band_n;
+	if (n_anchors != n) return fail("mm2gb_engine_band_order: the last micro-batch had another number of anchors");
+	MM2GB_HIP(hipSetDevice(e.device));
+	MM2GB_HIP(hipStreamSynchronize(w.stream));
+	int32_t cnt[CNT_WORDS];
+	unsigned flags = 0;
+	MM2GB_HIP(hipMemcpy(cnt, w.counters.ptr, sizeof cnt, hipMemcpyDeviceToHost));
+	MM2GB_HIP(hipMemcpy(&flags, w.flags.ptr, sizeof flags, hipMemcpyDeviceToHost));
+	if (st) MM2GB_HIP(hipMemcpy(st, w.st.ptr, (size_t)n * sizeof(int32_t), hipMemcpyDeviceToHost));
+	if (flags & (FLAG_ANY_SEGID | FLAG_NO_LUT)) return 0;
+	if (order) MM2GB_HIP(hipMemcpy(order, w.band_order.ptr, (size_t)n * sizeof(uint16_t), hipMemcpyDeviceToHost));
+	const int n_chunks = cnt[CNT_NCHUNK];
+	std::vector<int32_t> cs(n_chunks), ce(n_chunks), state((size_t)n / 64 + 1);
+	std::vector<int64_t> cost(n_chunks);
+	if (n_chunks > 0) {
+		MM2GB_HIP(hipMemcpy(cs.data(), w.chunk_start.ptr, (size_t)n_chunks * 4, hipMemcpyDeviceToHost));
+		MM2GB_HIP(hipMemcpy(ce.data(), w.chunk_end.ptr, (size_t)n_chunks * 4, hipMemcpyDeviceToHost));
+		MM2GB_HIP(hipMemcpy(cost.data(), w.chunk_cost.ptr, (size_t)n_chunks * 8, hipMemcpyDeviceToHost));
+	}
+	MM2GB_HIP(hipMemcpy(state.data(), w.band_state.ptr, state.size() * 4, hipMemcpyDeviceToHost));
+	const int slab = e.params.band_slab, lag = e.params.band_lag;
+	int64_t ns = 0;
+	for (int c = 0; c < n_chunks; ++c) {
+		const int64_t len = ce[c] - cs[c];
+		if (!(2 * (cost[c] - 16 * len) > (int64_t)lag * len)) continue;
+		for (int64_t s0 = cs[c]; s0 < ce[c]; s0 += slab) {
+			if (s0 - lag <= cs[c]) continue;
+			if (ns < cap_slabs) {
+				slab_s0[ns] = (int32_t)s0; slab_n[ns] = (int32_t)std::min<int64_t>(slab, ce[c] - s0); slab_cs[ns] = cs[c]; slab_state[ns] = state[(size_t)s0 >> 6];
+			}
+			++ns;
+		}
+	}
+	*n_slabs = ns;
+	return 0;
+}
 int mm2gb_engine_skip_stats(mm2gb_engine_t *eng, int64_t *out)
 {
 	if (!eng || !out) return fail("mm2gb_engine_skip_stats: null argument");
```

Result: faster. 7227 billion (median of 6 runs) (+3.2%).
